# YoungSeng/QPGesture

Measured on AMD Instinct MI355X. Metric: matched gesture frames/sec (GestureKNN), higher is better.
Workload: dtype split-f16 products / f64 block sums + f64 re-evaluation; 1 GPU; 1 x 24 s clip (M=6 windows, Q=48 steps, 1440 frames each) per job vs speaker-10-class DB N_db=2048 windows (53248 candidates), shipped mode wavlm_feat(f32-bounded/f64-exact)+text(f32)+phase; n_db=2048, windows_per_clip=6, clips=1, clips_per_gpu=1, feature_dtype=f32, audio_precision=mixed, encode_batch=0, clips_in_flight=1, parallelism=single GPU, unsharded DB

## Files before the change

include/qpg.h:

```cpp
#ifndef QPG_H
#define QPG_H

#include <stddef.h>
#include <stdint.h>

#ifdef __cplusplus
extern "C" {
#endif

#define QPG_OK 0
#define QPG_EINVAL (-1)
#define QPG_EHIP (-2)
#define QPG_EUNSUP (-3)

typedef struct qpg_ctx qpg_ctx;

int qpg_version(void);
const char* qpg_build_id(void);
int qpg_ctx_create(int device, qpg_ctx** out);
int qpg_dev_kernarg(void);
int qpg_ctx_destroy(qpg_ctx* ctx);
#define QPG_OPT_GATE_DEDUP_FROM_CHAINS 0
#define QPG_OPT_TAKES_STAGES 1
#define QPG_OPT_COUNT 4
int qpg_ctx_set_option(qpg_ctx* ctx, int option, int value);
int qpg_ctx_get_option(qpg_ctx* ctx, int option, int* value);
int qpg_last_error(char* buf, size_t n);
int qpg_signal_i32(qpg_ctx*, void* stream, int32_t* dst, int32_t value);
int qpg_doorbell_wait(qpg_ctx*, void* stream, int32_t* counter, const int32_t* go, int32_t timeout_ms);


int qpg_wavlm_resample_f32(qpg_ctx*, void* stream, const float* x, int64_t N, int Tin, int F, int Tout, float* out);

int qpg_frame_norm2_f64(qpg_ctx*, void* stream, const float* x, int64_t rows, int F, double* out);

int qpg_audio_cand_norm2(qpg_ctx*, void* stream, const double* fn2, int N, int T, const int32_t* cand_t,
                         int G, int n_taps, int tap_stride, double* cn2);

int qpg_l2_normalize_rows_f32(qpg_ctx*, void* stream, const float* x, int64_t rows, int D, float* out);
int qpg_text_pack_queries_f32(qpg_ctx*, void* stream, const float* x, int M, int R, int D, const int32_t* q_win,
                              const int32_t* q_row, int Q, float* out);


int qpg_audio_pack_queries(qpg_ctx*, void* stream, const float* qbase, int M, int T, int F,
                           const int32_t* q_win, const int32_t* q_t, int Q, int n_taps, int tap_stride,
                           float* q32, double* qn2);

int qpg_audio_cosine_f64(qpg_ctx*, void* stream, const float* base, int N, int T, int F,
                         const int32_t* cand_t, int G, int n_taps, int tap_stride, const double* cn2,
                         const float* q32, const double* qn2, int Q, double* D, int64_t ldD);
int qpg_audio_cosine_f64_h(qpg_ctx*, void* stream, const void* base_f16, int N, int T, int F,
                           const int32_t* cand_t, int G, int n_taps, int tap_stride, const double* cn2,
                           const float* q32, const double* qn2, int Q, double* D, int64_t ldD);

#define QPG_AUDIO_MX_ERR 2.05e-6
int qpg_audio_cosine_mx(qpg_ctx*, void* stream, const float* base, int N, int T, int F, const int32_t* cand_t, int G,
                        int n_taps, int tap_stride, const double* cn2, const float* q32, const double* qn2, int Q,
                        void* D, int d_is_f32, int64_t ldD, int32_t* stats);

int qpg_audio_cosine_mx_h(qpg_ctx*, void* stream, const void* base_f16, int N, int T, int F, const int32_t* cand_t, int G,
                          int n_taps, int tap_stride, const double* cn2, const float* q32, const double* qn2, int Q,
                          void* D, int d_is_f32, int64_t ldD, int32_t* stats);

#define QPG_AUDIO_HL_ERR 1.3e-6
int qpg_audio_hl_supported(int T, int F, int G, int n_taps, int tap_stride, int cand_step);
int qpg_audio_pack_queries_hl(qpg_ctx*, void* stream, const float* qbase, int M, int T, int F, const int32_t* q_win,
                              const int32_t* q_t, int Q, int n_taps, int tap_stride, float* q32, double* qn2, void* image,
                              int64_t image_bytes);
int64_t qpg_audio_hl_db_bytes(int N, int F);
int64_t qpg_audio_hl_query_bytes(int Q, int F);
int qpg_audio_hl_pack_db(qpg_ctx*, void* stream, const float* base, int N, int T, int F, int G, int n_taps, int tap_stride,
                         int cand_step, void* image, int64_t image_bytes);
int qpg_audio_hl_pack_queries(qpg_ctx*, void* stream, const float* q32, int Q, int F, void* image, int64_t image_bytes);
int qpg_clip_pack_hl(qpg_ctx*, void* stream, const float* qbase, int M, int T, int F, const int32_t* q_win,
                     const int32_t* q_t, int Q, int n_taps, int tap_stride, float* q32, double* qn2, void* image,
                     int64_t image_bytes, const float* text_ctx, int Mt, int R, int Dt, const int32_t* tq_win,
                     const int32_t* tq_row, int Qt, float* qn_out, void* cols_image, int64_t cols_bytes);
int qpg_audio_cosine_hl(qpg_ctx*, void* stream, const void* db_image, int N, int F, int G, const double* cn2,
                        const void* q_image, const double* qn2, int Q, void* D, int d_is_f32, int64_t ldD, int32_t* stats);
int qpg_audio_hl1_supported(int T, int F, int G, int n_taps, int tap_stride, int cand_step);
int64_t qpg_audio_hl1_db_bytes(int N, int F);
int qpg_audio_hl1_pack_db(qpg_ctx*, void* stream, const void* base_f16, int N, int T, int F, int G, int n_taps,
                          int tap_stride, int cand_step, void* image, int64_t image_bytes);
int qpg_audio_cosine_hl1(qpg_ctx*, void* stream, const void* db_image, int N, int F, int G, const double* cn2,
                         const void* q_image, const double* qn2, int Q, void* D, int d_is_f32, int64_t ldD, int32_t* stats);
int qpg_probe_mfma_f16_tile(qpg_ctx*, void* stream, const void* a, const void* b, const float* c, int tiles, float* out);

int qpg_text_pack_candidates_f32(qpg_ctx*, void* stream, const float* x, int N, int R, int Dm,
                                 const int32_t* cand_r, int G, float* xt);

int qpg_text_cosine_f32(qpg_ctx*, void* stream, const float* xt, int64_t C, int Dm, const float* qn, int Q,
                        float* D, int64_t ldD);

int64_t qpg_text_percode_ws_bytes(int64_t C, int Q, int K, int tiles_per_chunk);
int qpg_text_percode_f32(qpg_ctx*, void* stream, const float* xt, int64_t C, int Dm, const int16_t* cand_code, int K,
                         const float* qn, int Q, int tiles_per_chunk, int32_t idx_base, float absent, void* ws,
                         int64_t ws_bytes, float* out_dist, int32_t* out_idx, int16_t* out_rank, int32_t* out_nn);
int qpg_text_pack_candidates_f16(qpg_ctx*, void* stream, const float* x, int N, int R, int Dm, const int32_t* cand_r,
                                 int G, void* xh, float* nrm);
int qpg_text_percode_f16(qpg_ctx*, void* stream, const void* xh, const float* nrm, int64_t C, int Dm,
                         const int16_t* cand_code, int K, const float* qn, int Q, int32_t idx_base, float absent,
                         void* ws, int64_t ws_bytes, float* out_dist, int32_t* out_idx, int16_t* out_rank,
                         int32_t* out_nn);

int64_t qpg_hl_rows_bytes(int64_t R, int D);
int64_t qpg_hl_cols_bytes(int Q, int D);
int qpg_hl_pack_rows(qpg_ctx*, void* stream, const float* xs, int64_t R, int D, void* image, int64_t image_bytes);
int qpg_hl_pack_cols(qpg_ctx*, void* stream, const float* qn, int Q, int D, void* image, int64_t image_bytes);
int qpg_hl_prepare_queries(qpg_ctx*, void* stream, const float* q, int Q, int D, float* qn_out, void* cols_image,
                           int64_t image_bytes, float* qperm_out);
int qpg_hl_gemm_distance(qpg_ctx*, void* stream, const void* rows_image, int64_t R, int D, const void* cols_image, int Q,
                         float* Dm, int64_t ldD, float* tile_min, int64_t ldT);
int qpg_hl_gemm_tilemin(qpg_ctx*, void* stream, const void* rows_image, int64_t R, int D, const void* cols_image, int Q,
                        float band, float* tile_min, uint16_t* tile_mask, int64_t ldT);
int qpg_hl_gemm_tilemin_h(qpg_ctx*, void* stream, const void* rows_image, int64_t R, int D, const void* cols_image, int Q,
                          float band, float* tile_min_t, uint16_t* tile_mask_t, int64_t ldQ);
int qpg_perm32_rows_f32(qpg_ctx*, void* stream, const float* x, int64_t R, int D, float* y);
int qpg_percode_select_bycode_f32(qpg_ctx*, void* stream, const float* tile_min_t, const uint16_t* tile_mask_t, int64_t ldQ,
                                  int Q, int64_t R, const int16_t* row_code, const int32_t* row_index,
                                  const int32_t* zero_row, const int32_t* code_tile, int K, float band,
                                  const float* qn_perm, const float* xs_perm, int D, float absent, float* out_dist,
                                  int32_t* out_idx, int16_t* out_rank, int32_t* out_nn, int32_t* stats, int32_t idx_base);
int qpg_percode_select_sorted_f32(qpg_ctx*, void* stream, const float* Dm, int64_t ldD, const float* tile_min,
                                  const uint16_t* tile_mask , int64_t ldT,
                                  int Q, int64_t R, const int16_t* row_code, const int32_t* row_index,
                                  const int32_t* zero_row, const int32_t* code_tile, int K, float band, const float* qn,
                                  const float* xs, int D, float absent, float* out_dist, int32_t* out_idx,
                                  int16_t* out_rank, int32_t* out_nn, int32_t* stats, int32_t idx_base, int q_block,
                                  int64_t block_stride);

int qpg_wavvq_lev_f32(qpg_ctx*, void* stream, const int32_t* sym_db, int N, int T, const int32_t* cand_t, int G,
                      const int32_t* tap_off, int n_taps, const int32_t* sym_q, int Mq, int Tq,
                      const int32_t* q_win, const int32_t* q_t, int Q, float* D, int64_t ldD);

int qpg_percode_select_f64(qpg_ctx*, void* stream, const double* D, int64_t ldD, int Q, const int16_t* cand_code,
                           int64_t C, int K, double absent, int32_t idx_base, double* out_dist, int32_t* out_idx,
                           int16_t* out_rank, int q_block, int64_t block_stride);
int qpg_percode_select_f32(qpg_ctx*, void* stream, const float* D, int64_t ldD, int Q, const int16_t* cand_code,
                           int64_t C, int K, float absent, int32_t idx_base, float* out_dist, int32_t* out_idx,
                           int16_t* out_rank, int q_block, int64_t block_stride);

int qpg_percode_select_guarded_f64(qpg_ctx*, void* stream, const double* D, int64_t ldD, int Q, const int16_t* cand_code,
                                   int64_t C, int K, double absent, int32_t idx_base, double* out_dist, int32_t* out_idx,
                                   int16_t* out_rank, int q_block, int64_t block_stride, const float* base, int T, int F,
                                   const int32_t* cand_t, int G, int n_taps, int tap_stride, const float* q32, double eps,
                                   int32_t* stats, int base_is_f16);

int64_t qpg_percode_select_exact_ws_bytes(int Q, int64_t C, int K);
int qpg_percode_select_exact_f64(qpg_ctx*, void* stream, const double* D, int64_t ldD, int Q, const int16_t* cand_code,
                                 int64_t C, int K, double absent, int32_t idx_base, double* out_dist, int32_t* out_idx,
                                 int16_t* out_rank, int q_block, int64_t block_stride, const float* base, int T, int F,
                                 const int32_t* cand_t, int G, int n_taps, int tap_stride, const float* q32, double eps,
                                 int32_t* stats, int base_is_f16, void* ws, int64_t ws_bytes);

int qpg_percode_select_mixed_f64(qpg_ctx*, void* stream, const void* D, int d_is_f32, int64_t ldD, int Q, const int16_t* cand_code,
                                 int64_t C, int K, double absent, int32_t idx_base, double* out_dist, int32_t* out_idx,
                                 int16_t* out_rank, int q_block, int64_t block_stride, const float* base, int T, int F,
                                 const int32_t* cand_t, int G, int n_taps, int tap_stride, const float* q32,
                                 const double* qn2, const double* cn2, double eps1, double eps2, int32_t* stats,
                                 void* ws, int64_t ws_bytes, int base_is_f16);
int64_t qpg_percode_select_mixed_ws_bytes(int Q, int K);
int64_t qpg_percode_select_mixed_ws_stride(int K);
int qpg_percode_select_mixed_f64_cut(qpg_ctx*, void* stream, const void* D, int d_is_f32, int64_t ldD, int Q,
                                     const int16_t* cand_code, int64_t C, int K, double absent, int32_t idx_base,
                                     double* out_dist, int32_t* out_idx, int16_t* out_rank, int q_block, int64_t block_stride,
                                     const float* base, int T, int F, const int32_t* cand_t, int G, int n_taps,
                                     int tap_stride, const float* q32, const double* qn2, const double* cn2, double eps1,
                                     double eps2, int32_t* stats, void* ws, int64_t ws_bytes, int base_is_f16,
                                     const int16_t* pos_rank_t, const int16_t* freq_rank, int top_n, int probe);

int64_t qpg_merge_mixed_ws_bytes(int Q, int K, int fl_cap);
int qpg_merge_mixed_phase1_f64(qpg_ctx*, void* stream, const void* recv, int W, int64_t src_stride, int64_t dist_off,
                               int64_t idx_off, int Q, int K, double absent, double eps1, int R, void* req,
                               int64_t req_stride, void* ws, int64_t ws_bytes, int32_t* stats, int fl_cap,
                               int64_t flag_off);
int qpg_shard_refine_f64(qpg_ctx*, void* stream, const void* req_recv, int W, int64_t req_stride, int R, int q_stride,
                         int64_t cand_base, const float* base, int base_is_f16, int T, int F, const int32_t* cand_t, int G,
                         int n_taps, int tap_stride, const float* q32, const double* qn2, const double* cn2, void* resp,
                         int64_t resp_stride, int reference_arithmetic, int32_t* stats, int Rq);
int qpg_flags_stamp(qpg_ctx*, void* stream, void* buf, int nblk, int64_t stride, int64_t off, const int32_t* stats);
int qpg_flags_gather(qpg_ctx*, void* stream, const void* buf, int nblk, int64_t stride, int64_t off, int32_t* stats);
int qpg_merge_mixed_phase2_f64(qpg_ctx*, void* stream, const void* recv, int W, int64_t src_stride, int64_t idx_off, int Q,
                               int K, double absent, const void* ws, int64_t ws_bytes, const void* resp_recv,
                               int64_t resp_stride, double* out_dist, int32_t* out_idx, int16_t* out_rank, int32_t* stats,
                               int fl_cap, double eps2);

int qpg_merge_select_f64(qpg_ctx*, void* stream, const void* recv, int W, int64_t src_stride, int64_t dist_off,
                         int64_t idx_off, int Q, int K, double absent, double* out_dist, int32_t* out_idx,
                         int16_t* out_rank, double eps2, int32_t* stats);
int qpg_merge_select_f32(qpg_ctx*, void* stream, const void* recv, int W, int64_t src_stride, int64_t dist_off,
                         int64_t idx_off, int Q, int K, float absent, float* out_dist, int32_t* out_idx,
                         int16_t* out_rank);

int qpg_rank_rows_f64(qpg_ctx*, void* stream, const double* d, int Q, int K, int16_t* out);
int qpg_rank_rows_f32(qpg_ctx*, void* stream, const float* d, int Q, int K, int16_t* out);


int qpg_l2_table_f32(qpg_ctx*, void* stream, const float* sig, int K, int Dm, float* out);

#define QPG_MODE_AUD_TXT 0
#define QPG_MODE_AUD 1
#define QPG_MODE_TXT 2
#define QPG_MODE_SERIAL_WALK 0x100
#define QPG_MODE_PREFUSED 0x200

int qpg_match_steps(qpg_ctx*, void* stream, const int16_t* aud_rank, const int32_t* aud_idx,
                    const int16_t* txt_rank, const int32_t* txt_idx, const int16_t* pos_rank,
                    const int16_t* freq_rank, const int32_t* code, int code_ld, const int32_t* aud_cidx,
                    const int32_t* aud_pslot, int Ga, const int32_t* txt_cidx, const int32_t* txt_pslot, int Gt,
                    const float* phase, int Tp, int mode, int M, int steps, int K, int seed_code,
                    const float* seed_phase, int32_t* gate_tables, int32_t* out_codes, float* out_phase,
                    int32_t* out_vote, int32_t* out_status, const int32_t* guard_flags);
int qpg_match_steps_batch(qpg_ctx*, void* stream, const int16_t* aud_rank, const int32_t* aud_idx, const int16_t* txt_rank,
                          const int32_t* txt_idx, const int16_t* pos_rank, const int16_t* freq_rank, const int32_t* code,
                          int code_ld, const int32_t* aud_cidx, const int32_t* aud_pslot, int Ga, const int32_t* txt_cidx,
                          const int32_t* txt_pslot, int Gt, const float* phase, int Tp, int mode, int M, int steps, int K,
                          int n_chains, const int32_t* seed_codes, const float* seed_phase, int32_t* gate_tables,
                          int32_t* out_codes, float* out_phase, int32_t* out_vote, int32_t* out_status,
                          int64_t status_stride, const int32_t* guard_flags);
#define QPG_TAKES_MAX 65536
size_t qpg_match_steps_takes_ws_bytes(int n_takes, int M, int steps);
int qpg_match_steps_takes(qpg_ctx*, void* stream, const int16_t* aud_rank, const int32_t* aud_idx, const int16_t* txt_rank,
                          const int32_t* txt_idx, const int16_t* pos_rank, const int16_t* freq_rank, const int32_t* code,
                          int code_ld, const int32_t* aud_cidx, const int32_t* aud_pslot, int Ga, const int32_t* txt_cidx,
                          const int32_t* txt_pslot, int Gt, const float* phase, int Tp, int mode, int M, int steps, int K,
                          int n_takes, const int32_t* seed_codes, const float* seed_phase, int32_t* gate_tables,
                          int32_t* out_codes, float* out_phase, int32_t* out_vote, int32_t* out_status,
                          int64_t status_stride, const int32_t* guard_flags, void* workspace, size_t workspace_bytes);
int qpg_fuse_best_ranked(qpg_ctx*, void* stream, const int16_t* rank, const int32_t* idx, const int16_t* pos_rank,
                         const int16_t* freq_rank, int Q, int K, int32_t* T);

typedef struct qpg_comm qpg_comm;
int qpg_comm_unique_id(void* id, int64_t id_bytes);
int qpg_comm_create(qpg_ctx*, const void* id, int64_t id_bytes, int rank, int world, qpg_comm** out);
int qpg_comm_destroy(qpg_comm*);
int qpg_comm_allgather(qpg_ctx*, void* stream, qpg_comm*, const void* send, void* recv, int64_t bytes);
int qpg_comm_alltoall(qpg_ctx*, void* stream, qpg_comm*, const void* send, void* recv, int64_t bytes);
int qpg_comm_allreduce_max_i32(qpg_ctx*, void* stream, qpg_comm*, int32_t* buf, int64_t count);
int qpg_allreduce_min_u64(qpg_ctx*, void* stream, qpg_comm*, uint64_t* buf, int64_t count);
int qpg_pack_min_u64(qpg_ctx*, void* stream, const float* dist, const int32_t* idx, int64_t n, uint64_t* packed);
int qpg_unpack_min_u64(qpg_ctx*, void* stream, const uint64_t* packed, int64_t n, float absent, float* dist, int32_t* idx);


int qpg_conv1d_f32(qpg_ctx*, void* stream, const float* x, int B, int T_in, int Cin, const float* w,
                   const float* bias, int taps, int Cin_pad, int Cout, int Cout_pad, int in_stride, int in_offset,
                   int dil, int T_out, int out_stride, int out_offset, int T_y, const float* residual, int relu_in,
                   int relu_out, float* y, float* ws, int64_t ws_floats);

int qpg_convt_f32(qpg_ctx*, void* stream, const float* x, int B, int T_in, int Cx, const float* wt, const float* bias,
                  int taps, int Cin_pad, int Cout, int Cout_pad, int in_stride, int in_offset, int dil, int T_out,
                  int out_stride, int out_offset, int T_y, const float* residual, int relu_in, int relu_out, float* y);
int qpg_convt_pair_f32(qpg_ctx*, void* stream, const float* x, int B, int T_in, int Cx, const float* wt0,
                       const float* bias0, int in_offset0, int out_offset0, const float* wt1, const float* bias1,
                       int in_offset1, int out_offset1, int taps, int Cin_pad, int Cout, int Cout_pad, int in_stride,
                       int dil, int T_out, int out_stride, int T_y, float* y);
int qpg_tpack_f32(qpg_ctx*, void* stream, const float* w, int taps, int Cin_pad, int Cout_pad, int nb, float* out);
int qpg_pad_channels_f32(qpg_ctx*, void* stream, const float* x, int64_t R, int C, int Cp, float* y);
int qpg_resblock_f32(qpg_ctx*, void* stream, const float* x, int B, int T, int dil, const float* wpack,
                     const float* b1, const float* b2, float* y, float* hidden);

int qpg_vq_argmin_f32(qpg_ctx*, void* stream, const float* z, const float* dot, const float* kk, int64_t R, int E,
                      int K, int64_t* ids, float* dmin, float* dsecond);

int qpg_vq_gather_f32(qpg_ctx*, void* stream, const float* k, const int64_t* ids, int64_t R, int E, int K, float* out,
                      int32_t* status);

#define QPG_CONV16_WEXP_FROM_IMAGE 0x7fff
int64_t qpg_conv16_image_bytes(int taps, int Cin, int Cout);
int qpg_conv16_pack_weights(qpg_ctx*, void* stream, const float* w, int taps, int Cin, int Cin_pad_w, int Cout, int Cout_pad_w,
                            void* image, int64_t image_bytes);
int qpg_conv16_f32(qpg_ctx*, void* stream, const float* x, int B, int T_in, int Cx, int Cin, const void* image, int w_exp,
                   const float* bias, int taps, int Cout, int in_stride, int in_offset, int dil, int T_out, int out_stride,
                   int out_offset, int T_y, const float* residual, int relu_in, int relu_out, float* y, int32_t* status);

#define QPG_VQ_MAX_DOWN 4
#define QPG_VQ_MAX_DEPTH 4
typedef struct {
  const float* w;
  const float* b;
  int32_t taps, cin, cin_pad, cout, cout_pad;
  const float* wt;
} qpg_conv_desc;
typedef struct {
  int32_t in_dim, width, emb, bins, down_t, depth, growth, reverse_dec;
  qpg_conv_desc enc_down[QPG_VQ_MAX_DOWN];
  qpg_conv_desc enc_res[QPG_VQ_MAX_DOWN][QPG_VQ_MAX_DEPTH][2];
  qpg_conv_desc enc_out;
  qpg_conv_desc dec_in;
  qpg_conv_desc dec_res[QPG_VQ_MAX_DOWN][QPG_VQ_MAX_DEPTH][2];
  qpg_conv_desc dec_up_even[QPG_VQ_MAX_DOWN];
  qpg_conv_desc dec_up_odd[QPG_VQ_MAX_DOWN];
  qpg_conv_desc dec_out;
  qpg_conv_desc kT;
  const float* k;
  const float* kk;
  const float* enc_res_pack[QPG_VQ_MAX_DOWN][QPG_VQ_MAX_DEPTH];
  const float* dec_res_pack[QPG_VQ_MAX_DOWN][QPG_VQ_MAX_DEPTH];
} qpg_vq_model;

int64_t qpg_vq_workspace_floats(const qpg_vq_model* m, int B, int T);
int qpg_vq_encode_f32(qpg_ctx*, void* stream, const qpg_vq_model* m, const float* x, int B, int T, float* ws,
                      int64_t ws_floats, int64_t* ids, float* latent, float* margin);
int qpg_vq_decode_f32(qpg_ctx*, void* stream, const qpg_vq_model* m, const int64_t* ids, int B, int L, float* ws,
                      int64_t ws_floats, float* out, int32_t* status);

int qpg_pose_to_euler_f64(qpg_ctx*, void* stream, const float* poses, int64_t T, int J, const double* mean,
                          const double* stdc, const double* sg_mid, const double* sg_head, const double* sg_tail, int W,
                          double* euler, int32_t* status);

#define QPG_PAE_CHANNELS 135
#define QPG_PAE_MID 15
#define QPG_PAE_EMBED 8
#define QPG_PAE_TIME 240
#define QPG_PAE_HALO 120
#define QPG_PAE_WS_STRIDE 136
#define QPG_PAE_MAX_CHUNK (1 << 22)
#define QPG_PAE_OFF_W1 0
#define QPG_PAE_OFF_BN1 522240
#define QPG_PAE_OFF_W2 522288
#define QPG_PAE_OFF_BN2 583728
#define QPG_PAE_OFF_FC 583776
#define QPG_PAE_OFF_FCBN 587616
#define QPG_PAE_OFF_FREQ 587664
#define QPG_PAE_OFF_TPI 587784
#define QPG_PAE_PARAM_FLOATS 587792
int qpg_pae_phase_f32(qpg_ctx*, void* stream, const float* params, const double* pose, const double* mean,
                      const double* stdc, const int64_t* clip_off, int n_clips, int64_t n_total, int64_t frame0,
                      int64_t n_frames, float* ws, int64_t ws_floats, float* out, float* v_out, float* latent_out);

#define QPG_PAET_OFF_TPI 0
#define QPG_PAET_OFF_ARGS 1
#define QPG_PAET_OFF_FREQS 241
#define QPG_PAET_TRAINABLE 361
#define QPG_PAET_OFF_CONV1_W 361
#define QPG_PAET_OFF_CONV1_B 486361
#define QPG_PAET_OFF_BN1 486376
#define QPG_PAET_OFF_CONV2_W 486406
#define QPG_PAET_OFF_CONV2_B 515206
#define QPG_PAET_OFF_BN2 515214
#define QPG_PAET_OFF_FC 515230
#define QPG_PAET_OFF_FCBN 519086
#define QPG_PAET_OFF_DECONV1_W 519118
#define QPG_PAET_OFF_DECONV1_B 547918
#define QPG_PAET_OFF_BN3 547933
#define QPG_PAET_OFF_DECONV2_W 547963
#define QPG_PAET_OFF_DECONV2_B 1033963
#define QPG_PAET_PARAM_FLOATS 1034098
#define QPG_PAET_ST_BN1 0
#define QPG_PAET_ST_BN2 30
#define QPG_PAET_ST_FCBN 46
#define QPG_PAET_ST_BN3 78
#define QPG_PAET_STATS_FLOATS 108
#define QPG_PAET_MAX_BATCH 65536
#define QPG_PAET_SLABS 16
int qpg_pae_train_ws_floats(qpg_ctx*, void* stream, int batch, int64_t* floats);
int qpg_pae_train_forward_f32(qpg_ctx*, void* stream, const float* params, float* stats, const float* poses,
                              int64_t n_frames, const int64_t* starts, int batch, int train, float* ws,
                              int64_t ws_floats, double* loss);
int qpg_pae_train_backward_f32(qpg_ctx*, void* stream, const float* params, int batch, float* ws, int64_t ws_floats,
                               float* grads);
int qpg_pae_adamw_f32(qpg_ctx*, void* stream, float* p, const float* g, float* m, float* v, int64_t n, double lr,
                      double weight_decay, double beta1, double beta2, double eps, int64_t step);

int64_t qpg_vq_reduce_ws_bytes(void);

int qpg_vq_loss_f32(qpg_ctx*, void* stream, const float* x_out, const float* x_target, int B, int T, int C,
                    const float* commit_loss, float w_commit, float w_reg, float w_vel, float w_acc, void* ws,
                    int64_t ws_bytes, float* out6);
int qpg_vq_loss_grad_f32(qpg_ctx*, void* stream, const float* x_out, const float* x_target, int B, int T, int C,
                         float w_reg, float w_vel, float w_acc, float upstream, float* d_x_out);

int qpg_vq_latent_stats_f32(qpg_ctx*, void* stream, const float* z, const float* zq, const float* dmin, int64_t R,
                            int E, void* ws, int64_t ws_bytes, float* out3);
int qpg_vq_commit_grad_f32(qpg_ctx*, void* stream, const float* z, const float* zq, int64_t R, int E, float scale,
                           const float* d_zq, float* d_z);

int64_t qpg_vq_code_sums_ws_bytes(int64_t R, int E, int K);
int qpg_vq_code_sums_f32(qpg_ctx*, void* stream, const float* z, const int64_t* ids, int64_t R, int E, int K,
                         float* batch_sum, float* batch_elem, void* ws, int64_t ws_bytes);
int qpg_vq_ema_update_f32(qpg_ctx*, void* stream, float* k, float* k_sum, float* k_elem, const float* batch_sum,
                          const float* batch_elem, const float* k_rand, float mu, float threshold, int K, int E,
                          float* kT, int ldkT, float* kk, void* ws, int64_t ws_bytes, float* out4);
int qpg_vq_code_norms_f32(qpg_ctx*, void* stream, const float* k, int K, int E, float* kk);
// ... 26 lines not shown
```

qpgesture_amd/code_knn.py:

```python
import ctypes
from collections import namedtuple
from typing import NamedTuple, Optional

import numpy as np
import torch

from . import _lib
from .parallel import allreduce_max_, allreduce_min_index, exchange_bytes, shard_rows
from .sorted_rows import SortedRows

from .constant import (ABSENT_DIST, NUM_AUDIO_FEAT_FRAMES, STEP_SZ, WAVVQ_GROUP_SIZE, codebook_size, num_frames,
                       num_frames_code)

MODE_AUD_TXT, MODE_AUD, MODE_TXT = _lib.QPG_MODE_AUD_TXT, _lib.QPG_MODE_AUD, _lib.QPG_MODE_TXT
AUDIO_MX_ERR = _lib.QPG_AUDIO_MX_ERR
AUDIO_MX_BAND = 2.1 * AUDIO_MX_ERR
AUDIO_HL_ERR = _lib.QPG_AUDIO_HL_ERR
AUDIO_HL_BAND = 2.1 * AUDIO_HL_ERR

FLAG_LIST_OVERFLOW, FLAG_SMALL_NORMS, FLAG_REQUEST_OVERFLOW, FLAG_CROSS_SHARD_TIE = 1, 2, 4, 8
FLAG_TEXT_OVERFLOW = 16


_PIN_SENTINEL = -1234567
# ... 599 lines not shown
        D = torch.empty((Q, max(C, 1)), dtype=torch.float32, device=dev)
        taps = (ctypes.c_int32 * len(db.vq_taps))(*db.vq_taps)
        _lib.call("qpg_wavvq_lev_f32", dev, db.vq_sym, db.n_local, db.Tv, db.vq_t, db.Gv, taps, len(db.vq_taps),
                  sym_q, sym_q.shape[0], sym_q.shape[1], _i32(q_win, dev), _i32(q_t, dev), Q, D, D.stride(0))
        dist, idx, rank = self._select_plain(D, db.vq_cand_code, C, db.Gv, out, want_rank and db.world == 1)
        self._last_D_aud = D
        return self._finish(dist, idx, rank, want_rank, reduce)

    def _reduce_min(self, dist, idx):
        if self.db.world == 1:
            return dist, idx
        return allreduce_min_index(dist, idx)

    def guard_stats(self):
        v = self._guard_stats.cpu().numpy()
        return int(v[0]), bool(v[1])

    def mixed_stats(self):
        v = self._guard_stats.cpu().numpy()
        return {"tier1_pairs": int(v[2]), "tier2_pairs": int(v[0]), "flags": int(v[1])}

    def tier1_list_lengths(self):
        ws, Q = self._mix_ws, self._last_mix_Q
        if ws is None or not Q:
            return np.zeros((0,), np.int64)
        K = self.db.K
        stride = int(_lib.load().qpg_percode_select_mixed_ws_stride(K))
        w = ws[:Q * stride].view(Q, stride)[:, 24 * K:24 * K + 4].contiguous().view(torch.int32)
        return w.cpu().numpy().reshape(-1).astype(np.int64)

    def clear_flags(self):
        self._guard_stats[1:2].zero_()

    @staticmethod
    def numpy_ranks(dist, idx=None, integer=False):
        d = dist.detach().cpu().numpy()
        present = None if idx is None else (idx.detach().cpu().numpy() >= 0)
        out = np.empty(d.shape, np.int16)
        for r_, row in enumerate(d):
            full = present is not None and bool(present[r_].all())
            if full and integer:
                arr = np.array([int(x) for x in row])
            elif full:
                arr = np.array(list(row))
            else:
                arr = np.array(list(row.astype(np.float64)))
            out[r_] = arr.argsort().argsort()
        return torch.from_numpy(out).to(dist.device)

    def rank_rows(self, dist):
        out = torch.empty(dist.shape, dtype=torch.int16, device=dist.device)
        name = "qpg_rank_rows_f64" if dist.dtype == torch.float64 else "qpg_rank_rows_f32"
        _lib.call(name, self.db.device, dist.contiguous(), dist.shape[0], dist.shape[1], out)
        return out

    def _unpack(self, dist, idx, G, ks, cidx):
        d = dist[0].cpu().numpy()
        ix = idx[0].cpu().numpy()
        code = self.db.code_host
        dists, pays, aux = [], [], []
        for c in range(self.db.K):
            if ix[c] < 0:
                dists.append(ABSENT_DIST)
                pays.append([])
                aux.append([])
            else:
                j, g = divmod(int(ix[c]), G)
                dists.append(d[c])
                pays.append(code[j, cidx[g]:cidx[g] + STEP_SZ])
                aux.append([j, ks[g]])
        return dists, pays, aux

    def search_audio_cands(self, clip_input, mode="wavlm_feat"):
        db = self.db
        if mode == "wavvq_feat":
            v = np.asarray(clip_input).reshape(11, 2).astype(np.int64)
            track = np.zeros((1, db.Tv, 2), np.int64)
            t0 = -min(db.vq_taps)
            for i, off in enumerate(db.vq_taps):
                track[0, t0 + off] = v[i]
            dist, idx = self.sweep_audio_wavvq(track, [0], [t0])
            return self._unpack(dist, idx, db.Gv, db.vq_k, db.vq_cidx_host)
        if mode != "wavlm_feat":
            raise NotImplementedError(mode)
        q = torch.as_tensor(np.asarray(clip_input, np.float32).reshape(1, NUM_AUDIO_FEAT_FRAMES, db.F),
                            device=db.device).contiguous()
        dist, idx = self.sweep_audio(q, [0], [0], tap_stride=1)
        return self._unpack(dist, idx, db.Ga, db.aud_k, db.aud_cidx_host)

    def search_text_cands(self, clip_input, mode="wavvq_feat"):
        db = self.db
        q = torch.as_tensor(np.asarray(clip_input, np.float32).reshape(1, db.Dt), device=db.device).contiguous()
        dist, idx = self.sweep_text(q)
        return self._unpack(dist, idx, db.Gt, db.txt_k, db.txt_rows_host)

    def n_steps(self):
        return len(self.query_positions())

    def _query_index(self, M):
        if M not in self._qcache:
            pos, dev = self.query_positions(), self.db.device
            qw = np.repeat(np.arange(M), len(pos))
            qt = np.tile(np.array([int(i) for i in pos]), M)
            rows_ = [int(i / self.n_db_frm * 30) for i in pos] * M
            self._qcache[M] = (_i32(qw, dev), _i32(qt, dev), _i32(np.asarray(rows_), dev))
        return self._qcache[M]

    def _fork_side(self):
        dev = self.db.device
        if self._side_stream is None:
            self._side_stream = torch.cuda.Stream(dev)
            self._side_gate, self._side_done = torch.cuda.Event(), torch.cuda.Event()
            self._sweep_event = torch.cuda.Event()
        if dev.index is None or dev.index == torch.cuda.current_device():
            self._side_gate.record()
        else:
            self._side_gate.record(torch.cuda.current_stream(dev))
        self._side_stream.wait_event(self._side_gate)
        return self._side_stream

    def _clip_pack(self, test_interp, test_context, q_win, q_t, q_row, Q):
        db, dev = self.db, self.db.device
        q32 = torch.empty((Q, NUM_AUDIO_FEAT_FRAMES * db.F), dtype=torch.float32, device=dev)
        qn2 = torch.empty((Q,), dtype=torch.float64, device=dev)
        qi = self._hl_qimage = _grown(self._hl_qimage, int(_lib.load().qpg_audio_hl_query_bytes(Q, db.F)), dev)
        qn = torch.empty((Q, db.Dt), dtype=torch.float32, device=dev)
        cols = db.txt_sorted.cols_buffer(Q, self._txt_scratch)
        tc, ti = test_context.contiguous(), test_interp.contiguous()
        _lib.call("qpg_clip_pack_hl", dev, ti, ti.shape[0], db.T, db.F, q_win, q_t, Q, NUM_AUDIO_FEAT_FRAMES,
                  db.tap_stride, q32, qn2, qi, qi.numel(), tc, tc.shape[0], tc.shape[1], db.Dt, q_win, q_row, Q, qn, cols,
                  cols.numel())
        return q32, qn2, qn

    def sweep_tables(self, test_interp, test_context, n_windows, mode=MODE_AUD_TXT, owner_blocks=False, for_walk=False,
                     after_sweep=None):
        db, dev = self.db, self.db.device
        M, steps = n_windows, self.n_steps()
        if test_interp.shape[0] < M or (mode != MODE_AUD and test_context.shape[0] < M):
            raise IndexError("n_windows=%d but the test arrays hold %d audio / %d context windows"
                             % (M, test_interp.shape[0], test_context.shape[0]))
        want = (db.Tv, 2) if self.use_wavvq else (db.T, db.F)
        if tuple(test_interp.shape[1:]) != want:
            raise ValueError("test audio windows have shape %s, database expects %s"
                             % (tuple(test_interp.shape[1:]), want))
        q_win, q_t, q_row = self._query_index(M)
        Q = M * steps
        key = (self._knobs(), self._facts(), M, steps, mode, for_walk, owner_blocks)
        plan = self._plans.get(key)
        if plan is None:
            plan = self._plans[key] = plan_step(*key)
        sharded = plan.sharded
        T = dict(aud_d=None, aud_idx=None, aud_rank=None, txt_d=None, txt_idx=None, txt_rank=None)
        gtab = torch.empty((3, max(M, 1) * steps, db.K), dtype=torch.int32, device=dev) if plan.split_fuse else None
        lay = self._layout(Q, owner_blocks, mode) if sharded else None
        side = self._fork_side() if plan.overlap else None
        packed = None
        if plan.clip_pack:
            packed = self._clip_pack(test_interp, test_context, q_win, q_t, q_row, Q)
            self._side_gate.record(torch.cuda.current_stream(dev))
            side.wait_event(self._side_gate)

        def keep(p_, g, r):
            T[p_ + "_d"], T[p_ + "_idx"], T[p_ + "_rank"] = r[0], r[1], (None if sharded else r[2])
            if gtab is not None:
                _lib.call("qpg_fuse_best_ranked", dev, r[2], r[1], db.pos_rank, db.freq_rank, Q, db.K, gtab[g])

        def text_pack():
            tc = test_context.contiguous()
            qn = torch.empty((Q, db.Dt), dtype=torch.float32, device=dev)
            _lib.call("qpg_text_pack_queries_f32", dev, tc, tc.shape[0], tc.shape[1], db.Dt, q_win, q_row, Q, qn)
            return qn

        def text_side(qn=None):
            if packed is not None:
                qn = packed[2]
            elif qn is None:
                qn = text_pack()
            keep("txt", 1, self.sweep_text(qn, want_rank=not sharded, reduce=not sharded, normalised=True,
                                           out=lay.views("txt") if sharded else None, cols_packed=packed is not None,
                                           kind=plan.text))

        if plan.order == "text_first":
            with torch.cuda.stream(side):
                text_side()
        aud = None
        if mode != MODE_TXT:
            out = lay.views("aud") if sharded else None
            if self.use_wavvq:
                r = self.sweep_audio_wavvq(test_interp, q_win, q_t, want_rank=not sharded, reduce=not sharded, out=out)
            else:
                aud = self._sweep_audio(plan.audio, test_interp, q_win, q_t, out=out, prepacked=packed,
                                        sweep_event=self._sweep_event if plan.order == "text_after_sweep" else None,
                                        after_sweep=after_sweep)
                r = self._finish(aud.dist, aud.idx, aud.rank, not sharded, not sharded)
            keep("aud", 0, r)
        if plan.order == "text_after_sweep":
            with torch.cuda.stream(side):
                qn_early = None if packed is not None else text_pack()
                side.wait_event(self._sweep_event)
                text_side(qn_early)
        elif plan.order == "audio_first":
            with torch.cuda.stream(side):
                text_side()
        if plan.overlap:
            self._side_done.record(side)
            torch.cuda.current_stream(dev).wait_event(self._side_done)
        elif mode != MODE_AUD:
            text_side()
        if sharded:
            self._merge_shards(lay, owner_blocks, T, aud)
        if self.host_ranks:
            for p_ in ("aud", "txt"):
                if T[p_ + "_d"] is not None:
                    T[p_ + "_rank"] = self.numpy_ranks(T[p_ + "_d"], T[p_ + "_idx"],
                                                       integer=(p_ == "aud" and self.use_wavvq))
        if gtab is not None:
            T["gate_tables"] = gtab
        return T

    def _layout(self, Q, owner_blocks, mode):
        parts = tuple(p_ for p_, off in (("aud", MODE_TXT), ("txt", MODE_AUD)) if mode != off)
        key = (Q, self.db.world if owner_blocks else 1, parts, not self.use_wavvq)
        if key not in self._layouts:
            self._layouts[key] = ExchangeLayout(key[0], self.db.K, key[1], parts, key[3], self.db.device)
        return self._layouts[key]

    def _merge_shards(self, lay, owner_blocks, T, aud):
        db, dev = self.db, self.db.device
        _lib.call("qpg_flags_stamp", dev, lay.send, lay.nblk, lay.block_bytes, lay.off["flags"], self._guard_stats)
        recv = exchange_bytes(lay.send, db.world, owner_blocks)
        src_stride = lay.block_bytes if owner_blocks else lay.send.numel()
        gathered = False
        for p_ in lay.parts:
            d = torch.empty((lay.Qb, db.K), dtype=lay.dtype[p_], device=dev)
            ix = torch.empty((lay.Qb, db.K), dtype=torch.int32, device=dev)
            rk = torch.empty((lay.Qb, db.K), dtype=torch.int16, device=dev)
            wavlm_aud = p_ == "aud" and aud is not None
            if wavlm_aud and aud.plan.path in ("mixed", "exact"):
                self._merge_mixed(recv, src_stride, lay, owner_blocks, d, ix, rk, aud.q32, aud.qn2, aud.plan)
                gathered = True
            elif lay.dtype[p_] == torch.float64:
                guard = wavlm_aud and self.tie_eps > 0
                _lib.call("qpg_merge_select_f64", dev, recv, db.world, src_stride, lay.off[p_ + "_d"],
                          lay.off[p_ + "_i"], lay.Qb, db.K, float(ABSENT_DIST), d, ix, rk,
                          float(self.tie_eps) if guard else 0.0, self._guard_stats if guard else None)
            else:
                _lib.call("qpg_merge_select_f32", dev, recv, db.world, src_stride,
                          lay.off[p_ + "_d"], lay.off[p_ + "_i"], lay.Qb, db.K, float(ABSENT_DIST), d, ix, rk)
            T[p_ + "_d"], T[p_ + "_idx"], T[p_ + "_rank"] = d, ix, rk
        if not gathered:
            _lib.call("qpg_flags_gather", dev, recv, db.world, src_stride, lay.off["flags"], self._guard_stats)
        if owner_blocks:
            allreduce_max_(self._guard_stats[1:2], force=self.force_sharded)

    def _merge_mixed(self, recv, src_stride, lay, owner_blocks, d, ix, rk, q32, qn2, plan):
        db, dev = self.db, self.db.device
        W, Qb, K = db.world, lay.Qb, db.K
        exact = plan.path == "exact"
        if exact:
            Rq, fl_cap, band = K, K * W, float(self.tie_eps)
        else:
            Rq = int(self.mixed_requests) if self.mixed_requests else max(64, 512 // W)
            fl_cap, band = 1024, plan.band
        R = Qb * Rq
        req_stride = resp_stride = 8 + 8 * R
        key = (exact, W, R)
        bufs = self._mm_cache.get(key)
        need_ws = int(_lib.load().qpg_merge_mixed_ws_bytes(Qb, K, fl_cap))
        if bufs is None or bufs[2].numel() < need_ws:
            bufs = self._mm_cache[key] = (torch.empty((W * req_stride,), dtype=torch.uint8, device=dev),
                                          torch.empty((W * resp_stride,), dtype=torch.uint8, device=dev),
                                          torch.empty((need_ws,), dtype=torch.uint8, device=dev))
        req, resp, ws = bufs
        _lib.call("qpg_merge_mixed_phase1_f64", dev, recv, W, src_stride, lay.off["aud_d"], lay.off["aud_i"], Qb, K,
                  float(ABSENT_DIST), band, R, req, req_stride, ws, ws.numel(), self._guard_stats, fl_cap,
                  lay.off["flags"])
        half = int(db.feature_dtype == "f16")
        refine = (db.idx_base * db.Ga, db.base, half, db.T, db.F, db.aud_t, db.Ga, NUM_AUDIO_FEAT_FRAMES, db.tap_stride,
                  q32, qn2, db.cn2, resp, resp_stride, int(exact), self._guard_stats, Rq)
        if owner_blocks:
            req_recv = exchange_bytes(req, W, True)
            _lib.call("qpg_shard_refine_f64", dev, req_recv, W, req_stride, R, Qb, *refine)
            resp_recv = exchange_bytes(resp, W, True)
        else:
            mine = req[db.rank * req_stride:(db.rank + 1) * req_stride]
            _lib.call("qpg_shard_refine_f64", dev, mine, 1, req_stride, R, 0, *refine)
            resp_recv = exchange_bytes(resp[:resp_stride], W, False)
        _lib.call("qpg_merge_mixed_phase2_f64", dev, recv, W, src_stride, lay.off["aud_i"], Qb, K, float(ABSENT_DIST), ws,
                  ws.numel(), resp_recv, resp_stride, d, ix, rk, self._guard_stats, fl_cap,
                  0.0 if exact else float(self.tie_eps))

    def _seed_phase_tensor(self, seed_phase):
        if isinstance(seed_phase, torch.Tensor):
            return seed_phase.to(self.db.device, torch.float32).contiguous()
        return torch.as_tensor(np.asarray(seed_phase, np.float32), device=self.db.device).contiguous()

    def _launch_walk(self, T, q0, Qt, rows, mode, prefusable, M, steps, seed, sp, outs, chains=None):
        db, dev = self.db, self.db.device
        gate = T.get("gate_tables")
        prefused = prefusable and gate is not None and mode == MODE_AUD_TXT and gate.shape[1] == Qt
        if not prefused:
            gate = torch.empty((3, rows, db.K), dtype=torch.int32, device=dev)
        mode_w = mode | (_lib.QPG_MODE_PREFUSED if prefused else 0)
        if chains is None and self.serial_walk:
            mode_w |= _lib.QPG_MODE_SERIAL_WALK
        a_cidx, a_pslot, a_G = self._audio_grid()
        tabs = [None if T[k] is None else T[k][q0:q0 + Qt] for k in ("aud_rank", "aud_idx", "txt_rank", "txt_idx")]
        head = (*tabs, db.pos_rank, db.freq_rank, db.code, db.code.shape[1], a_cidx, a_pslot, a_G, db.txt_cidx,
                db.txt_pslot, db.Gt, db.phase, db.Tp, mode_w, M, steps, db.K)
        guard = self._guard_stats[1:2]
        if chains is None:
            _lib.call("qpg_match_steps", dev, *head, seed, sp, gate, *outs, guard)
        else:
            _lib.call("qpg_match_steps_batch", dev, *head, chains, seed, sp, gate, *outs, 2, guard)
        return gate

    def walk(self, T, n_windows, window_offset=0, mode=MODE_AUD_TXT, seed_code=None, seed_phase=None, sync=True,
             seed_ptrs=None, out_pin=None, n_chains=1):
# ... 165 lines not shown
```

qpgesture_amd/csrc/qpg_common.h:

```cpp
#pragma once
#include <hip/hip_runtime.h>
#include <stdint.h>
#include <stdio.h>
#include <string.h>

#include "../../include/qpg.h"

struct qpg_ctx {
  int device;
  int n_cu;
  float* zeros;
  bool select_lds_raised;
  int opt[QPG_OPT_COUNT];
};

#ifdef QPG_DEBUG_HOOKS
#define QPG_HOOK_VAR(type, name, value) static type name = value
#else
#define QPG_HOOK_VAR(type, name, value) static constexpr type name = value
#endif

void qpg_set_error(const char* fmt, ...);

#define QPG_REQUIRE(cond, ...)      \
  do {                              \
    if (!(cond)) {                  \
      qpg_set_error(__VA_ARGS__);   \
      return QPG_EINVAL;            \
    }                               \
  } while (0)

#define QPG_LAUNCH_CHECK(name)                                                \
  do {                                                                        \
    hipError_t e_ = hipGetLastError();                                        \
    if (e_ != hipSuccess) {                                                   \
      qpg_set_error("%s: launch failed: %s", name, hipGetErrorString(e_));    \
      return QPG_EHIP;                                                        \
    }                                                                         \
  } while (0)

static inline hipStream_t qpg_stream(void* s) { return reinterpret_cast<hipStream_t>(s); }

typedef double f64x4 __attribute__((ext_vector_type(4)));
typedef float f32x4 __attribute__((ext_vector_type(4)));
typedef float f32x16 __attribute__((ext_vector_type(16)));

#pragma clang fp contract(off)
__device__ __forceinline__ float f_mul(float a, float b) { return a * b; }
__device__ __forceinline__ float f_add(float a, float b) { return a + b; }
__device__ __forceinline__ float f_sub(float a, float b) { return a - b; }
__device__ __forceinline__ float f_div(float a, float b) { return a / b; }
__device__ __forceinline__ float f_sqrt(float a) { return __builtin_sqrtf(a); }
__device__ __forceinline__ double f_mul(double a, double b) { return a * b; }
__device__ __forceinline__ double f_add(double a, double b) { return a + b; }
__device__ __forceinline__ double f_sub(double a, double b) { return a - b; }
__device__ __forceinline__ double f_div(double a, double b) { return a / b; }

__device__ __forceinline__ double cosine_from_dot(double dot, double qn2, double cn2) {
  const double tiny = 10.0 * 2.220446049250313e-16;
  double nq = sqrt(qn2), nc = sqrt(cn2);
  bool zq = nq < tiny, zc = nc < tiny;
  if (zq || zc) {
    double a = zq ? qn2 : 1.0, b = zc ? cn2 : 1.0;
    double cross = dot / ((zq ? 1.0 : nq) * (zc ? 1.0 : nc));
    return 0.5 * (a + b - 2.0 * cross);
  }
  return 1.0 - dot / (nq * nc);
}


__host__ __device__ __forceinline__ int rank_sort_pow2(int K) {
  int p = 2;
  while (p < K) p <<= 1;
  return p;
}
__device__ __forceinline__ unsigned long long rank_sort_key(double d) {
  const long long b = __double_as_longlong(d + 0.0);
  return b < 0 ? ~(unsigned long long)b : ((unsigned long long)b | 0x8000000000000000ull);
}
__device__ __forceinline__ unsigned long long rank_sort_key(float d) {
  const unsigned int b = __float_as_uint(d + 0.0f);
  return (unsigned long long)((b >> 31) ? ~b : (b | 0x80000000u));
}
template <int PJ>
__device__ __forceinline__ int lane_xor(int x) {
  if (PJ == 1) return __builtin_amdgcn_update_dpp(x, x, 0xB1, 0xf, 0xf, false);
  if (PJ == 2) return __builtin_amdgcn_update_dpp(x, x, 0x4E, 0xf, 0xf, false);
  if (PJ == 4) {
    const int t = __builtin_amdgcn_update_dpp(x, x, 0x104, 0xf, 0x5, false);
    return __builtin_amdgcn_update_dpp(t, x, 0x114, 0xf, 0xa, false);
  }
  if (PJ == 8) return __builtin_amdgcn_update_dpp(x, x, 0x128, 0xf, 0xf, false);
  if (PJ == 16) {
    const auto r = __builtin_amdgcn_permlane16_swap(x, x, false, false);
    return (threadIdx.x & 16) ? r[0] : r[1];
  }
  const auto r = __builtin_amdgcn_permlane32_swap(x, x, false, false);
  return (threadIdx.x & 32) ? r[0] : r[1];
}
template <int PJ>
__device__ __forceinline__ void lane_xor_pair(unsigned long long k0, unsigned long long k1, int c0, int c1,
                                              unsigned long long& p0, unsigned long long& p1, int& q0, int& q1) {
  const unsigned int a0 = (unsigned int)lane_xor<PJ>((int)(unsigned int)k0);
  const unsigned int a1 = (unsigned int)lane_xor<PJ>((int)(unsigned int)(k0 >> 32));
  const unsigned int a2 = (unsigned int)lane_xor<PJ>((int)(unsigned int)k1);
  const unsigned int a3 = (unsigned int)lane_xor<PJ>((int)(unsigned int)(k1 >> 32));
  q0 = lane_xor<PJ>(c0);
  q1 = lane_xor<PJ>(c1);
  p0 = ((unsigned long long)a1 << 32) | a0;
  p1 = ((unsigned long long)a3 << 32) | a2;
}

struct RankPair {
  unsigned long long k0, k1;
  int c0, c1;
};
__device__ __forceinline__ bool rank_gt(unsigned long long ka, int ca, unsigned long long kb, int cb) {
  return ka > kb || (ka == kb && ca > cb);
}
template <int J>
__device__ __forceinline__ void bitonic_chain(RankPair& e, int i0, int k, unsigned long long* skey, int* scode) {
  if constexpr (J == 0) {
    return;
  } else {
    if (J < k) {
      const bool up = (i0 & k) == 0;
      if constexpr (J == 1) {
        if (rank_gt(e.k0, e.c0, e.k1, e.c1) == up) {
          const unsigned long long tk = e.k0; e.k0 = e.k1; e.k1 = tk;
          const int tc = e.c0; e.c0 = e.c1; e.c1 = tc;
        }
      } else {
        unsigned long long p0, p1;
        int q0, q1;
        if constexpr (J / 2 < 64) {
          lane_xor_pair<J / 2>(e.k0, e.k1, e.c0, e.c1, p0, p1, q0, q1);
        } else {
          __syncthreads();
          skey[i0] = e.k0; skey[i0 + 1] = e.k1; scode[i0] = e.c0; scode[i0 + 1] = e.c1;
          __syncthreads();
          const int o0 = i0 ^ J;
          p0 = skey[o0]; p1 = skey[o0 + 1]; q0 = scode[o0]; q1 = scode[o0 + 1];
        }
        const bool keep_min = ((i0 & J) == 0) == up;
        if (rank_gt(e.k0, e.c0, p0, q0) == keep_min) { e.k0 = p0; e.c0 = q0; }
        if (rank_gt(e.k1, e.c1, p1, q1) == keep_min) { e.k1 = p1; e.c1 = q1; }
      }
    }
    bitonic_chain<J / 2>(e, i0, k, skey, scode);
  }
}
template <int KP, typename T, typename F>
__device__ __forceinline__ void block_sorted_ranks_unrolled(const T* v, int K, unsigned long long* skey, int* scode,
                                                            F&& emit) {
  const int tid = threadIdx.x;
  if ((tid & ~63) * 2 >= KP) {
    for (int k = 256; k <= KP; k <<= 1)
      for (int j = k >> 1; j >= 128; j >>= 1) {
        __syncthreads();
        __syncthreads();
      }
    return;
  }
  const int i0 = 2 * tid;
  RankPair e;
  e.k0 = i0 < K ? rank_sort_key(v[i0]) : ~0ull;
  e.k1 = i0 + 1 < K ? rank_sort_key(v[i0 + 1]) : ~0ull;
// ... 44 lines not shown
```

qpgesture_amd/csrc/qpg_core.hip:

```cpp
#include <stdarg.h>

#include "qpg_common.h"
#include <stdlib.h>

static thread_local char g_err[512] = "";

void qpg_set_error(const char* fmt, ...) {
  va_list ap;
  va_start(ap, fmt);
  vsnprintf(g_err, sizeof(g_err), fmt, ap);
  va_end(ap);
}

extern "C" int qpg_version(void) { return 109; }

#ifndef QPG_BUILD_ID
#define QPG_BUILD_ID "unstamped"
#endif
static const char g_build_id[] = "QPG_BUILD_ID=" QPG_BUILD_ID;
extern "C" const char* qpg_build_id(void) { return g_build_id + 13; }

extern "C" int qpg_dev_kernarg(void) {
  const char* e = getenv("HIP_FORCE_DEV_KERNARG");
  return (e && e[0] == '1') ? 1 : 0;
}

extern "C" int qpg_last_error(char* buf, size_t n) {
  if (!buf || n == 0) return QPG_EINVAL;
  strncpy(buf, g_err, n - 1);
  buf[n - 1] = 0;
  return QPG_OK;
}

extern "C" int qpg_ctx_create(int device, qpg_ctx** out) {
  QPG_REQUIRE(out != nullptr, "qpg_ctx_create: out is null");
  int n = 0;
  if (hipGetDeviceCount(&n) != hipSuccess || device < 0 || device >= n) {
    qpg_set_error("qpg_ctx_create: no HIP device %d (count %d)", device, n);
    return QPG_EHIP;
  }
  hipDeviceProp_t p;
  if (hipGetDeviceProperties(&p, device) != hipSuccess) {
    qpg_set_error("qpg_ctx_create: hipGetDeviceProperties failed");
    return QPG_EHIP;
  }
  qpg_ctx* c = new qpg_ctx;
  c->device = device;
  c->n_cu = p.multiProcessorCount;
  c->zeros = nullptr;
  c->select_lds_raised = false;
  for (int i = 0; i < QPG_OPT_COUNT; ++i) c->opt[i] = 0;
  c->opt[QPG_OPT_GATE_DEDUP_FROM_CHAINS] = 1;
  c->opt[QPG_OPT_TAKES_STAGES] = 7;
  int prev = 0;
  (void)hipGetDevice(&prev);
  const bool ok = hipSetDevice(device) == hipSuccess && hipMalloc(reinterpret_cast<void**>(&c->zeros), 4096) == hipSuccess &&
                  hipMemset(c->zeros, 0, 4096) == hipSuccess;
  (void)hipSetDevice(prev);
  if (!ok) {
    qpg_set_error("qpg_ctx_create: could not allocate the context's zero page on device %d", device);
    delete c;
    return QPG_EHIP;
  }
  *out = c;
  return QPG_OK;
}

extern "C" int qpg_ctx_set_option(qpg_ctx* ctx, int option, int value) {
  QPG_REQUIRE(ctx != nullptr, "qpg_ctx_set_option: null context");
  QPG_REQUIRE(option >= 0 && option < QPG_OPT_COUNT, "qpg_ctx_set_option: unknown option %d", option);
  if (option == QPG_OPT_GATE_DEDUP_FROM_CHAINS) QPG_REQUIRE(value >= 0, "qpg_ctx_set_option: gate_dedup_from_chains >= 0");
  ctx->opt[option] = value;
  return QPG_OK;
}

extern "C" int qpg_ctx_get_option(qpg_ctx* ctx, int option, int* value) {
  QPG_REQUIRE(ctx != nullptr && value != nullptr, "qpg_ctx_get_option: null pointer");
  QPG_REQUIRE(option >= 0 && option < QPG_OPT_COUNT, "qpg_ctx_get_option: unknown option %d", option);
  *value = ctx->opt[option];
  return QPG_OK;
}

extern "C" int qpg_ctx_destroy(qpg_ctx* ctx) {
  if (ctx && ctx->zeros) (void)hipFree(ctx->zeros);
  delete ctx;
  return QPG_OK;
}

__global__ void signal_i32_kernel(int32_t* dst, int32_t value) {
  __hip_atomic_store(dst, value, __ATOMIC_RELEASE, __HIP_MEMORY_SCOPE_SYSTEM);
}

extern "C" int qpg_signal_i32(qpg_ctx* ctx, void* stream, int32_t* dst, int32_t value) {
  QPG_REQUIRE(ctx && dst && (reinterpret_cast<uintptr_t>(dst) % 4) == 0, "qpg_signal_i32: null or misaligned destination");
  hipLaunchKernelGGL(signal_i32_kernel, dim3(1), dim3(1), 0, qpg_stream(stream), dst, value);
  QPG_LAUNCH_CHECK("signal_i32_kernel");
  return QPG_OK;
}

__global__ void doorbell_wait_kernel(int32_t* __restrict__ counter, const int32_t* __restrict__ go, int32_t timeout_ms) {
  const int32_t seq = atomicAdd(counter, 1) + 1;
  const long long t0 = wall_clock64();
  const long long limit = (long long)timeout_ms * 100000ll;
  while (__hip_atomic_load(go, __ATOMIC_RELAXED, __HIP_MEMORY_SCOPE_SYSTEM) - seq < 0) {
    if (wall_clock64() - t0 > limit) break;
    __builtin_amdgcn_s_sleep(16);
  }
  __atomic_thread_fence(__ATOMIC_ACQUIRE);
}

extern "C" int qpg_doorbell_wait(qpg_ctx* ctx, void* stream, int32_t* counter, const int32_t* go, int32_t timeout_ms) {
  QPG_REQUIRE(ctx && counter && go && timeout_ms > 0 && timeout_ms <= 60000, "qpg_doorbell_wait: bad argument (timeout 1..60000 ms)");
  hipLaunchKernelGGL(doorbell_wait_kernel, dim3(1), dim3(1), 0, qpg_stream(stream), counter, go, timeout_ms);
  QPG_LAUNCH_CHECK("doorbell_wait_kernel");
  return QPG_OK;
}

__global__ __launch_bounds__(256) void frame_norm2_kernel(const float* __restrict__ x, int64_t rows, int F,
                                                          double* __restrict__ out) {
  const int lane = threadIdx.x & 63;
  const int64_t row = (int64_t)blockIdx.x * 4 + (threadIdx.x >> 6);
  if (row >= rows) return;
  const float* p = x + row * F;
  double s = 0.0;
  if ((F & 3) == 0) {
    for (int e = lane * 4; e < F; e += 256) {
      f32x4 v = *reinterpret_cast<const f32x4*>(p + e);
      s += (double)v.x * v.x + (double)v.y * v.y + (double)v.z * v.z + (double)v.w * v.w;
    }
  } else {
    for (int e = lane; e < F; e += 64) s += (double)p[e] * p[e];
  }
  for (int o = 32; o > 0; o >>= 1) s += __shfl_down(s, o, 64);
  if (lane == 0) out[row] = s;
}

extern "C" int qpg_frame_norm2_f64(qpg_ctx* ctx, void* stream, const float* x, int64_t rows, int F, double* out) {
  QPG_REQUIRE(ctx && x && out && rows >= 0 && F > 0, "qpg_frame_norm2_f64: bad argument");
  if (rows == 0) return QPG_OK;
  hipLaunchKernelGGL(frame_norm2_kernel, dim3((unsigned)((rows + 3) / 4)), dim3(256), 0, qpg_stream(stream), x, rows,
                     F, out);
  QPG_LAUNCH_CHECK("frame_norm2_kernel");
  return QPG_OK;
}

__global__ void audio_cand_norm2_kernel(const double* __restrict__ fn2, int N, int T, const int32_t* __restrict__ cand_t,
                                        int G, int n_taps, int tap_stride, double* __restrict__ cn2) {
  int64_t i = (int64_t)blockIdx.x * blockDim.x + threadIdx.x;
  if (i >= (int64_t)N * G) return;
  int j = (int)(i / G), g = (int)(i % G);
  int t0 = cand_t[g];
  double s = 0.0;
  for (int k = 0; k < n_taps; ++k) {
    int t = t0 + k * tap_stride;
    if (t < T) s += fn2[(int64_t)j * T + t];
  }
  cn2[i] = s;
}

extern "C" int qpg_audio_cand_norm2(qpg_ctx* ctx, void* stream, const double* fn2, int N, int T,
                                    const int32_t* cand_t, int G, int n_taps, int tap_stride, double* cn2) {
  QPG_REQUIRE(ctx && fn2 && cand_t && cn2 && N >= 0 && T > 0 && G > 0 && n_taps > 0 && tap_stride > 0,
              "qpg_audio_cand_norm2: bad argument");
  int64_t n = (int64_t)N * G;
  if (n == 0) return QPG_OK;
  hipLaunchKernelGGL(audio_cand_norm2_kernel, dim3((unsigned)((n + 255) / 256)), dim3(256), 0, qpg_stream(stream),
                     fn2, N, T, cand_t, G, n_taps, tap_stride, cn2);
  QPG_LAUNCH_CHECK("audio_cand_norm2_kernel");
  return QPG_OK;
}

template <bool GATHER>
__global__ __launch_bounds__(256) void l2_normalize_rows_kernel(const float* __restrict__ x, int64_t rows, int D,
                                                                float* __restrict__ out,
                                                                const int32_t* __restrict__ win,
                                                                const int32_t* __restrict__ row, int R) {
  const int64_t t = (int64_t)blockIdx.x * blockDim.x + threadIdx.x;
  int64_t r = t >> 2;
  const int l = (int)(t & 3);
  const bool live = r < rows;
  if (!live) r = rows - 1;
  const float* p = GATHER ? x + ((int64_t)win[r] * R + row[r]) * D : x + r * D;
  float a = 0.f;
  const int nfull = D >> 4;
  int g = 0;
  for (; g + 8 <= nfull; g += 8) {
    float v[32];
#pragma unroll
    for (int j = 0; j < 32; ++j) v[j] = p[(g + (j >> 2)) * 16 + (j & 3) * 4 + l];
#pragma unroll
    for (int j = 0; j < 8; ++j) {
#pragma unroll
      for (int u = 3; u >= 0; --u) a = f_add(f_mul(v[j * 4 + u], v[j * 4 + u]), a);
    }
  }
  for (; g < nfull; ++g) {
#pragma unroll
    for (int u = 3; u >= 0; --u) {
      const float v = p[g * 16 + u * 4 + l];
      a = f_add(f_mul(v, v), a);
    }
  }
  for (int i = nfull * 16; i < D; i += 4) {
    const float v = (i + l < D) ? p[i + l] : 0.f;
    a = f_add(f_mul(v, v), a);
  }
  const float o1 = __shfl_xor(a, 1, 64);
  const float pair = f_add(a, o1);
  const float o2 = __shfl_xor(pair, 2, 64);
  float n = f_sqrt(f_add(pair, o2));
  if (n < 10.f * 1.1920928955078125e-07f) n = 1.f;
  if (live) {
    float* o = out + r * D;
    int e = l;
    for (; e + 28 < D; e += 32) {
      float v[8];
#pragma unroll
      for (int j = 0; j < 8; ++j) v[j] = p[e + 4 * j];
#pragma unroll
      for (int j = 0; j < 8; ++j) o[e + 4 * j] = f_div(v[j], n);
    }
    for (; e < D; e += 4) o[e] = f_div(p[e], n);
  }
}

extern "C" int qpg_l2_normalize_rows_f32(qpg_ctx* ctx, void* stream, const float* x, int64_t rows, int D, float* out) {
// ... 47 lines not shown
```

qpgesture_amd/csrc/qpg_select.hip:

```cpp
#include "qpg_common.h"

__device__ __forceinline__ unsigned long long order_key(double d) {
  unsigned long long b = (unsigned long long)__double_as_longlong(d);
  return (b >> 63) ? ~b : (b | 0x8000000000000000ull);
}
__device__ __forceinline__ double key_value(unsigned long long k, double) {
  unsigned long long b = (k >> 63) ? (k & 0x7fffffffffffffffull) : ~k;
  return __longlong_as_double((long long)b);
}
__device__ __forceinline__ unsigned int order_key(float d) {
  unsigned int b = __float_as_uint(d);
  return (b >> 31) ? ~b : (b | 0x80000000u);
}
__device__ __forceinline__ float key_value(unsigned int k, float) {
  unsigned int b = (k >> 31) ? (k & 0x7fffffffu) : ~k;
  return __uint_as_float(b);
}

template <typename T, typename KeyT, bool PACKED>
__global__ __launch_bounds__(1024) void percode_select_kernel(const T* __restrict__ D, int64_t ldD,
                                                              const int16_t* __restrict__ cand_code, int64_t C, int K,
                                                              T absent, int32_t idx_base, T* __restrict__ out_dist,
                                                              int32_t* __restrict__ out_idx,
                                                              int16_t* __restrict__ out_rank, int q_block,
                                                              int64_t block_stride) {
  extern __shared__ __attribute__((aligned(16))) unsigned char smem[];
  unsigned long long* best = reinterpret_cast<unsigned long long*>(smem);
  unsigned int* besti = reinterpret_cast<unsigned int*>(smem + 8 * (size_t)K);
  T* v = reinterpret_cast<T*>(smem + 12 * (size_t)rank_sort_pow2(K));
  constexpr int VEC = 16 / sizeof(T);
  typedef T vecT __attribute__((ext_vector_type(VEC)));
  typedef int16_t vecC __attribute__((ext_vector_type(VEC)));
  const int q = blockIdx.x;
  if (q_block > 0) {
    const int64_t shift = (int64_t)(q / q_block) * block_stride;
    const int64_t rowoff = (int64_t)(q % q_block) * K - (int64_t)q * K;
    out_dist = reinterpret_cast<T*>(reinterpret_cast<unsigned char*>(out_dist) + shift) + rowoff;
    out_idx = reinterpret_cast<int32_t*>(reinterpret_cast<unsigned char*>(out_idx) + shift) + rowoff;
  }
  const T* row = D + (int64_t)q * ldD;
  for (int k = threadIdx.x; k < K; k += blockDim.x) {
    best[k] = ~0ull;
    besti[k] = 0xffffffffu;
  }
  __syncthreads();
  const bool vec_ok = (ldD % VEC) == 0 && (reinterpret_cast<uintptr_t>(D) % 16) == 0 &&
                      (reinterpret_cast<uintptr_t>(cand_code) % (2 * VEC)) == 0;
  const int64_t Cv = vec_ok ? (C / VEC) * VEC : 0;
  for (int64_t c = (int64_t)threadIdx.x * VEC; c < Cv; c += (int64_t)blockDim.x * VEC) {
    const vecT d = *reinterpret_cast<const vecT*>(row + c);
    const vecC cd = *reinterpret_cast<const vecC*>(cand_code + c);
#pragma unroll
    for (int e = 0; e < VEC; ++e) {
      if ((unsigned)cd[e] >= (unsigned)K) continue;
      const unsigned long long key = PACKED ? (((unsigned long long)order_key(d[e]) << 32) | (unsigned int)(c + e + idx_base))
                                            : (unsigned long long)order_key(d[e]);
      atomicMin(&best[cd[e]], key);
    }
  }
  for (int64_t c = Cv + threadIdx.x; c < C; c += blockDim.x) {
    const int cd = cand_code[c];
    if ((unsigned)cd >= (unsigned)K) continue;
    const unsigned long long key = PACKED ? (((unsigned long long)order_key(row[c]) << 32) | (unsigned int)(c + idx_base))
                                          : (unsigned long long)order_key(row[c]);
    atomicMin(&best[cd], key);
  }
  __syncthreads();
  if (!PACKED) {
    for (int64_t c = (int64_t)threadIdx.x * VEC; c < Cv; c += (int64_t)blockDim.x * VEC) {
      const vecT d = *reinterpret_cast<const vecT*>(row + c);
      const vecC cd = *reinterpret_cast<const vecC*>(cand_code + c);
#pragma unroll
      for (int e = 0; e < VEC; ++e)
        if ((unsigned)cd[e] < (unsigned)K && (unsigned long long)order_key(d[e]) == best[cd[e]])
          atomicMin(&besti[cd[e]], (unsigned int)(c + e + idx_base));
    }
    for (int64_t c = Cv + threadIdx.x; c < C; c += blockDim.x) {
      const int cd = cand_code[c];
      if ((unsigned)cd < (unsigned)K && (unsigned long long)order_key(row[c]) == best[cd])
        atomicMin(&besti[cd], (unsigned int)(c + idx_base));
    }
    __syncthreads();
  }
  for (int k = threadIdx.x; k < K; k += blockDim.x) {
    const unsigned long long kv = best[k];
    const bool have = kv != ~0ull;
    T d;
    int32_t ix;
    if (PACKED) {
      d = have ? key_value((KeyT)(kv >> 32), T(0)) : absent;
      ix = have ? (int32_t)(kv & 0xffffffffu) : -1;
    } else {
      d = have ? key_value((KeyT)kv, T(0)) : absent;
      ix = have ? (int32_t)besti[k] : -1;
    }
    v[k] = d;
    out_dist[(int64_t)q * K + k] = d;
    out_idx[(int64_t)q * K + k] = ix;
  }
  if (!out_rank) return;
  __syncthreads();
  const int Kp = rank_sort_pow2(K);
  block_sorted_ranks(v, K, best, reinterpret_cast<int*>(best + Kp),
                     [&](int k, int r) { out_rank[(int64_t)q * K + k] = (int16_t)r; });
}

template <typename T, typename F>
__device__ __forceinline__ void block_stable_ranks(const T* v, int K, int* cnt, F&& emit) {
  const int tid = threadIdx.x;
  if (K <= 512 && K >= 64 && (int)blockDim.x >= 256) {
    __shared__ unsigned long long rank_skey[512];
    __shared__ int rank_scode[512];
    block_sorted_ranks(v, K, rank_skey, rank_scode, emit);
    return;
  }
  const int P = (int)blockDim.x >= 2 * K ? (int)blockDim.x / K : 1;
  if (P == 1) {
    for (int k = tid; k < K; k += blockDim.x) {
      const T x = v[k];
      int r = 0;
#pragma unroll 8
      for (int o = 0; o < K; ++o) {
        const T y = v[o];
        r += (y < x) || (y == x && o < k);
      }
      emit(k, r);
    }
    return;
  }
  for (int k = tid; k < K; k += blockDim.x) cnt[k] = 0;
  __syncthreads();
  if (tid < P * K) {
    const int k = tid % K, part = tid / K;
    const int o0 = (int)((int64_t)part * K / P), o1 = (int)((int64_t)(part + 1) * K / P);
    const T x = v[k];
    int r = 0;
#pragma unroll 8
    for (int o = o0; o < o1; ++o) {
      const T y = v[o];
      r += (y < x) || (y == x && o < k);
    }
    atomicAdd(&cnt[k], r);
  }
  __syncthreads();
  for (int k = tid; k < K; k += blockDim.x) emit(k, cnt[k]);
}

struct GuardArgs {
  const float* base;
  int half;
  const float* q32;
  const int32_t* cand_t;
  int T, F, G, n_taps, tap_stride;
// ... 349 lines not shown
#define SEL_STAMP(i)                                                                          \
  do {                                                                                        \
    __syncthreads();                                                                          \
    if (blockIdx.x == 0 && blockIdx.y == 0 && threadIdx.x == 0) {                             \
      qpg_select_prof_buf[phase][i] = wall_clock64();                                         \
      qpg_select_prof_buf[3 + phase][i] = clock64();                                          \
    }                                                                                         \
  } while (0)
extern "C" int qpg_debug_select_prof(long long* out) {
  return hipMemcpyFromSymbol(out, HIP_SYMBOL(qpg_select_prof_buf), sizeof(long long) * 96) == hipSuccess ? 0 : -1;
}
#else
#define SEL_STAMP(i)
#endif

template <int NPER>
__global__ __launch_bounds__(256) void select_refine_kernel(GuardArgs A, int K, const double* __restrict__ cn2,
                                                            const double* __restrict__ qn2, unsigned char* __restrict__ ws,
                                                            int fast) {
  const int q = blockIdx.x, lane = threadIdx.x & 63;
  const int g = blockIdx.y * 4 + (threadIdx.x >> 6), ng = gridDim.y * 4;
  unsigned char* wq = mix_query_base(ws, q, K);
  const int* w_n = reinterpret_cast<const int*>(wq + 24 * (size_t)K);
  const int* w_lc = w_n + 4;
  double* w_ld = reinterpret_cast<double*>(const_cast<int*>(w_lc) + 2 * MIX_LIST);
  const int n = w_n[0];
  if (g >= n) return;
  const double qq = qn2[q];
  const float* qrow = A.q32 + (int64_t)q * A.n_taps * A.F;
  for (int e = g; e < n; e += ng) {
    const int c = w_lc[e];
    const double dot = fast ? pair_dot_fast_f64<NPER>(A, qrow, c, lane) : pair_dot_wave_f64(A, q, c, lane);
    if (lane == 0) w_ld[e] = cosine_from_dot(dot, qq, cn2[c]);
  }
}

__global__ __launch_bounds__(1024) void mixed_stream_kernel(const float* __restrict__ D, int64_t ldD,
                                                           const int16_t* __restrict__ cand_code, int64_t C, int K,
                                                           double eps1, unsigned char* __restrict__ ws) {
  extern __shared__ __attribute__((aligned(16))) unsigned char smem[];
  unsigned int* best32 = reinterpret_cast<unsigned int*>(smem);
  int* pc = reinterpret_cast<int*>(best32 + K);
  float* pd = reinterpret_cast<float*>(pc + MIX_SPOT);
  int16_t* pk = reinterpret_cast<int16_t*>(pd + MIX_SPOT);
  __shared__ int n_pot, n_keep;
  const int q = blockIdx.x, sl = blockIdx.y, tid = threadIdx.x;
#ifdef QPG_SELECT_PROF
  const int phase = 0;
#endif
  const float* row = D + (int64_t)q * ldD;
  const int64_t chunk = (((C + MIX_SPLIT - 1) / MIX_SPLIT) + 63) & ~(int64_t)63;
  const int64_t c0 = (int64_t)sl * chunk, c1 = c0 + chunk < C ? c0 + chunk : C;
  for (int k = tid; k < K; k += blockDim.x) best32[k] = 0xffffffffu;
  if (tid == 0) {
    n_pot = 0;
    n_keep = 0;
  }
  __syncthreads();
  SEL_STAMP(0);
  auto visit = [&](int64_t c, float dv, int cd) {
    if ((unsigned)cd >= (unsigned)K) return;
    const unsigned int key = order_key(dv);
    unsigned int old = *reinterpret_cast<volatile unsigned int*>(&best32[cd]);
    if (key < old) old = atomicMin(&best32[cd], key);
    if ((double)dv <= (double)key_value(old < key ? old : key, 0.f) + eps1) {
      const int pp = atomicAdd(&n_pot, 1);
      if (pp < MIX_SPOT) {
        pc[pp] = (int)c;
        pd[pp] = dv;
        pk[pp] = (int16_t)cd;
      }
    }
  };
  typedef int16_t c16x4 __attribute__((ext_vector_type(4)));
  const bool vec_ok = (ldD % 4) == 0 && (reinterpret_cast<uintptr_t>(D) % 16) == 0 &&
                      (reinterpret_cast<uintptr_t>(cand_code) % 8) == 0;
  const int64_t cv = vec_ok ? c0 + ((c1 - c0) / 4) * 4 : c0;
  constexpr int UN = 2;
  for (int64_t b = c0 + (int64_t)tid * 4; b < cv; b += (int64_t)blockDim.x * 4 * UN) {
    f32x4 d[UN];
    c16x4 cd[UN];
#pragma unroll
    for (int u = 0; u < UN; ++u) {
      const int64_t c = b + (int64_t)u * blockDim.x * 4;
      d[u] = (f32x4){0.f, 0.f, 0.f, 0.f};
      cd[u] = (c16x4){-1, -1, -1, -1};
      if (c < cv) {
        d[u] = *reinterpret_cast<const f32x4*>(row + c);
        cd[u] = *reinterpret_cast<const c16x4*>(cand_code + c);
      }
    }
    unsigned int key[UN][4], old[UN][4];
#pragma unroll
    for (int u = 0; u < UN; ++u)
#pragma unroll
      for (int e = 0; e < 4; ++e) {
        const int code = cd[u][e];
        key[u][e] = order_key(d[u][e]);
        old[u][e] = (unsigned)code < (unsigned)K ? *reinterpret_cast<volatile unsigned int*>(&best32[code]) : 0u;
      }
#pragma unroll
    for (int u = 0; u < UN; ++u)
#pragma unroll
      for (int e = 0; e < 4; ++e) {
        const int code = cd[u][e];
        if ((unsigned)code >= (unsigned)K) continue;
        unsigned int o = old[u][e];
        if (key[u][e] < o) o = atomicMin(&best32[code], key[u][e]);
        const unsigned int lo = o < key[u][e] ? o : key[u][e];
        if ((double)d[u][e] <= (double)key_value(lo, 0.f) + eps1) {
          const int pp = atomicAdd(&n_pot, 1);
          if (pp < MIX_SPOT) {
            pc[pp] = (int)(b + (int64_t)u * blockDim.x * 4 + e);
            pd[pp] = d[u][e];
            pk[pp] = (int16_t)code;
          }
        }
      }
  }
  for (int64_t c = cv + tid; c < c1; c += blockDim.x) visit(c, row[c], cand_code[c]);
  __syncthreads();
  SEL_STAMP(1);
  MixStream m = mix_stream_of(ws, q, K);
  if (MIX_INV_ATOMIC) {
    for (int k = tid; k < K; k += blockDim.x)
      if (best32[k] != 0xffffffffu) atomicMax(&m.inv[k], ~best32[k]);
  } else {
    for (int k = tid; k < K; k += blockDim.x) m.inv[(size_t)sl * K + k] = ~best32[k];
  }
  SEL_STAMP(2);
  const int np = n_pot;
  if (np > MIX_SPOT) {
    if (tid == 0) m.cnt[sl] = -1;
    return;
  }
  const int seg = sl * MIX_SPOT;
  for (int e = tid; e < np; e += blockDim.x) {
    if (!((double)pd[e] <= (double)key_value(best32[pk[e]], 0.f) + eps1)) continue;
    const int pos = seg + atomicAdd(&n_keep, 1);
    m.pot_c[pos] = pc[e];
    m.pot_d[pos] = pd[e];
    m.pot_k[pos] = pk[e];
  }
  __syncthreads();
  if (tid == 0) m.cnt[sl] = n_keep;
  SEL_STAMP(3);
}

template <typename DT>
__global__ __launch_bounds__(1024) void percode_select_mixed_f64_kernel(
    const DT* __restrict__ D, int64_t ldD, const int16_t* __restrict__ cand_code, int64_t C, int K, double absent,
    int32_t idx_base, double* __restrict__ out_dist, int32_t* __restrict__ out_idx, int16_t* __restrict__ out_rank,
    int q_block, int64_t block_stride, GuardArgs A, double eps1, const double* __restrict__ cn2,
    const double* __restrict__ qn2, int use_qlds, int phase, unsigned char* __restrict__ ws, int pre, RankCut RC) {
  extern __shared__ __attribute__((aligned(16))) unsigned char smem[];
  unsigned long long* best = reinterpret_cast<unsigned long long*>(smem);
  double* v = reinterpret_cast<double*>(smem + 8 * (size_t)K);
  unsigned int* besti = reinterpret_cast<unsigned int*>(smem + 16 * (size_t)K);
  unsigned int* near_ = besti + K;
  int* s_code = reinterpret_cast<int*>(near_ + K);
  unsigned char* refd = reinterpret_cast<unsigned char*>(s_code + K);
  unsigned char* tail = smem + 32 * (size_t)K;
  double* l_d = reinterpret_cast<double*>(tail);
  int* l_c = reinterpret_cast<int*>(tail + 8 * MIX_LIST);
  int* l_k = l_c + MIX_LIST;
  int* l2 = l_k + MIX_LIST;
  int* ctl = l2 + MIX_LIST2;
  int* p_c = ctl + 8;
  int16_t* p_k = reinterpret_cast<int16_t*>(p_c + MIX_LIST);
  int* rk = reinterpret_cast<int*>(p_k + MIX_LIST);
  int* pot_c = rk + K;
  int16_t* pot_k = reinterpret_cast<int16_t*>(pot_c + MIX_POT);
  float* qlds = reinterpret_cast<float*>(pot_k + MIX_POT);
  const int q = blockIdx.x, tid = threadIdx.x, lane = tid & 63, wv = tid >> 6, nwv = blockDim.x >> 6;
  const DT* row = D + (int64_t)q * ldD;
  if (q_block > 0) {
    const int64_t shift = (int64_t)(q / q_block) * block_stride;
    const int64_t rowoff = (int64_t)(q % q_block) * K - (int64_t)q * K;
    out_dist = reinterpret_cast<double*>(reinterpret_cast<unsigned char*>(out_dist) + shift) + rowoff;
    out_idx = reinterpret_cast<int32_t*>(reinterpret_cast<unsigned char*>(out_idx) + shift) + rowoff;
  }
  unsigned char* wq = ws ? mix_query_base(ws, q, K) : nullptr;
  for (int k = tid; k < K; k += blockDim.x) {
    best[k] = ~0ull;
    besti[k] = 0xffffffffu;
    near_[k] = 0;
    refd[k] = 0;
  }
  if (tid < 8) ctl[tid] = 0;
  __syncthreads();
  SEL_STAMP(0);
  unsigned long long* skey = reinterpret_cast<unsigned long long*>(p_c);
  int* scode = reinterpret_cast<int*>(skey + 512);
  auto rank_pass = [&](bool store) {
    block_sorted_ranks(v, K, skey, scode, [&](int k, int r) {
      if (store && out_rank) out_rank[(int64_t)q * K + k] = (int16_t)r;
      s_code[r] = k;
    });
  };
  int n = 0;
  bool order_parked = false;
  if (phase != 2) {
  constexpr int VE = 16 / (int)sizeof(DT);
  typedef DT vecD __attribute__((ext_vector_type(VE)));
  typedef int16_t vecC __attribute__((ext_vector_type(VE)));
  const bool vec_ok = (ldD % VE) == 0 && (reinterpret_cast<uintptr_t>(D) % 16) == 0 &&
                      (reinterpret_cast<uintptr_t>(cand_code) % (2 * VE)) == 0;
  const int64_t Cv = vec_ok ? (C / VE) * VE : 0;
  constexpr bool K32 = sizeof(DT) == 4;
  unsigned int* best32 = reinterpret_cast<unsigned int*>(s_code);
  const bool streamed = K32 && pre;
  MixStream ms = {};
  if (streamed) ms = mix_stream_of(ws, q, K);
  if (K32 && !streamed) {
    for (int k = tid; k < K; k += blockDim.x) best32[k] = 0xffffffffu;
    __syncthreads();
  }
  auto pass1 = [&](int64_t c, DT dv, int cd) {
    if ((unsigned)cd >= (unsigned)K) return;
    const double d = (double)dv;
    double lo;
    if constexpr (K32) {
      const unsigned int key = order_key((float)dv);
      unsigned int old = *reinterpret_cast<volatile unsigned int*>(&best32[cd]);
      if (key < old) old = atomicMin(&best32[cd], key);
      lo = (double)key_value(old < key ? old : key, 0.f);
    } else {
      const unsigned long long key = (unsigned long long)order_key(d);
      unsigned long long old = *reinterpret_cast<volatile unsigned long long*>(&best[cd]);
      if (key < old) old = atomicMin(&best[cd], key);
      lo = key_value(old < key ? old : key, 0.0);
    }
    if (d <= lo + eps1) {
      const int pp = atomicAdd(&ctl[4], 1);
      if (pp < MIX_POT) {
        pot_c[pp] = (int)c;
        pot_k[pp] = (int16_t)cd;
      }
    }
  };
  if (!streamed) {
#pragma unroll 4
    for (int64_t c = (int64_t)tid * VE; c < Cv; c += (int64_t)blockDim.x * VE) {
      const vecD d = *reinterpret_cast<const vecD*>(row + c);
      const vecC cd = *reinterpret_cast<const vecC*>(cand_code + c);
#pragma unroll
      for (int e = 0; e < VE; ++e) pass1(c + e, d[e], cd[e]);
    }
    for (int64_t c = Cv + tid; c < C; c += blockDim.x) pass1(c, row[c], cand_code[c]);
    __syncthreads();
  }
  int g_pot = 0;
  if (K32) {
    for (int k = tid; k < K; k += blockDim.x) {
      unsigned int b;
      if (streamed && MIX_INV_ATOMIC) {
        b = ~ms.inv[k];
        ms.inv[k] = 0;
      } else if (streamed) {
        unsigned int iv[MIX_SPLIT], mx = 0u;
#pragma unroll
        for (int sl = 0; sl < MIX_SPLIT; ++sl) iv[sl] = ms.inv[(size_t)sl * K + k];
#pragma unroll
        for (int sl = 0; sl < MIX_SPLIT; ++sl) mx = iv[sl] > mx ? iv[sl] : mx;
        b = ~mx;
      } else {
        b = best32[k];
      }
      best[k] = b == 0xffffffffu ? ~0ull : (unsigned long long)order_key((double)key_value(b, 0.f));
    }
    if (streamed) {
#pragma unroll
      for (int sl = 0; sl < MIX_SPLIT; ++sl) {
        const int ns = ms.cnt[sl];
        g_pot = (ns < 0 || g_pot < 0) ? -1 : g_pot + ns;
      }
    }
    __syncthreads();
  }
  SEL_STAMP(1);
  auto pass2 = [&](int64_t c, double d, int cd) {
    if ((unsigned)cd >= (unsigned)K) return;
    const unsigned long long bk = best[cd];
    if ((unsigned long long)order_key(d) == bk) atomicMin(&besti[cd], (unsigned int)(c + idx_base));
    else if (d > key_value(bk, 0.0) + eps1) return;
    if (atomicAdd(&near_[cd], 1u) == 1u) ctl[1] = 1;
    const int pp = atomicAdd(&ctl[3], 1);
    if (pp < MIX_LIST) {
      p_c[pp] = (int)c;
      p_k[pp] = (int16_t)cd;
    }
  };
  if (streamed && g_pot >= 0) {
    int seg_end[MIX_SPLIT];
    {
      int acc = 0;
#pragma unroll
      for (int sl = 0; sl < MIX_SPLIT; ++sl) {
        acc += ms.cnt[sl];
        seg_end[sl] = acc;
      }
    }
    constexpr int UE = 4;
    for (int e0 = tid; e0 < g_pot; e0 += (int)blockDim.x * UE) {
      int pc_[UE], pk_[UE];
      float pd_[UE];
#pragma unroll
      for (int u = 0; u < UE; ++u) {
        const int e = e0 + u * (int)blockDim.x;
        pk_[u] = -1;
        if (e < g_pot) {
          int sl = 0, first = 0;
#pragma unroll
          for (int i = 0; i < MIX_SPLIT - 1; ++i)
            if (e >= seg_end[i]) {
              sl = i + 1;
              first = seg_end[i];
            }
          const int pos = sl * MIX_SPOT + e - first;
          pc_[u] = ms.pot_c[pos];
          pd_[u] = ms.pot_d[pos];
          pk_[u] = ms.pot_k[pos];
        }
      }
#pragma unroll
      for (int u = 0; u < UE; ++u)
        if (pk_[u] >= 0) pass2(pc_[u], (double)pd_[u], pk_[u]);
    }
  } else if (!streamed && ctl[4] <= MIX_POT) {
    const int npot = ctl[4];
    for (int e = tid; e < npot; e += blockDim.x) pass2(pot_c[e], (double)row[pot_c[e]], pot_k[e]);
  } else {
#pragma unroll 4
    for (int64_t c = (int64_t)tid * VE; c < Cv; c += (int64_t)blockDim.x * VE) {
      const vecD d = *reinterpret_cast<const vecD*>(row + c);
      const vecC cd = *reinterpret_cast<const vecC*>(cand_code + c);
#pragma unroll
      for (int e = 0; e < VE; ++e) pass2(c + e, (double)d[e], cd[e]);
    }
    for (int64_t c = Cv + tid; c < C; c += blockDim.x) pass2(c, (double)row[c], cand_code[c]);
  }
  __syncthreads();
  if (streamed && tid < MIX_SPLIT) ms.cnt[tid] = 0;
  SEL_STAMP(2);
  for (int k = tid; k < K; k += blockDim.x) v[k] = besti[k] != 0xffffffffu ? key_value(best[k], 0.0) : absent;
  __syncthreads();
  const bool cut = RC.pos_t != nullptr && streamed && out_rank != nullptr && phase == 1;
  unsigned char* need2 = nullptr;
  if (cut) {
    unsigned char* cs = reinterpret_cast<unsigned char*>(pot_c);
    const int Kp = rank_sort_pow2(K);
    unsigned long long* skey2 = reinterpret_cast<unsigned long long*>(cs);
// ... 204 lines not shown
      w_v[k] = v[k];
      w_bi[k] = besti[k];
      w_nr[k] = near_[k];
    }
    for (int e = tid; e < n; e += blockDim.x) {
      w_lc[e] = l_c[e];
      w_lk[e] = l_k[e];
    }
    if (tid == 0) {
      w_n[0] = n;
      w_n[1] = order_parked ? 1 : 0;
    }
    SEL_STAMP(6);
    return;
  }
  if (phase == 2) {
    const unsigned long long* w_best = reinterpret_cast<const unsigned long long*>(wq);
    const double* w_v = reinterpret_cast<const double*>(wq + 8 * (size_t)K);
    const unsigned int* w_bi = reinterpret_cast<const unsigned int*>(wq + 16 * (size_t)K);
    const unsigned int* w_nr = w_bi + K;
    const int* w_n = reinterpret_cast<const int*>(wq + 24 * (size_t)K);
    const int* w_lc = w_n + 4;
    const int* w_lk = w_lc + MIX_LIST;
    const double* w_ld = reinterpret_cast<const double*>(w_lk + MIX_LIST);
    n = w_n[0];
    for (int k = tid; k < K; k += blockDim.x) {
      best[k] = w_best[k];
      v[k] = w_v[k];
      besti[k] = w_bi[k];
      near_[k] = w_nr[k];
    }
    for (int e = tid; e < n; e += blockDim.x) {
      l_c[e] = w_lc[e];
      l_k[e] = w_lk[e];
      l_d[e] = w_ld[e];
    }
    if (RC.pos_t) {
      unsigned char* isref = reinterpret_cast<unsigned char*>(pot_c);
      for (int k = tid; k < K; k += blockDim.x) isref[k] = 0;
      __syncthreads();
      for (int e = tid; e < n; e += blockDim.x) isref[w_lk[e]] = 1;
    }
    __syncthreads();
  }
  SEL_STAMP(7);
  if (n > 0) {
    const double qq = qn2[q];
    const bool fast = use_qlds != 0;
    if (phase == 0 && fast) {
      const int D4 = (A.n_taps * A.F) >> 2;
      const f32x4* src = reinterpret_cast<const f32x4*>(A.q32 + (int64_t)q * A.n_taps * A.F);
      for (int i = tid; i < D4; i += blockDim.x) reinterpret_cast<f32x4*>(qlds)[i] = src[i];
      __syncthreads();
    }
    for (int e = wv; e < n && phase == 0; e += nwv) {
      const int c = l_c[e];
      const double dot = fast ? pair_dot_fast_f64<4>(A, qlds, c, lane) : pair_dot_wave_f64(A, q, c, lane);
      if (lane == 0) l_d[e] = cosine_from_dot(dot, qq, cn2[c]);
    }
    for (int k = tid; k < K; k += blockDim.x)
      if (near_[k] >= 2) {
        rk[k] = (int)besti[k];
        best[k] = ~0ull;
        besti[k] = 0xffffffffu;
        s_code[k] = 0;
      }
    __syncthreads();
    for (int e = tid; e < n; e += blockDim.x) atomicMin(&best[l_k[e]], (unsigned long long)order_key(l_d[e]));
    __syncthreads();
    if (A.eps > 0.0) {
      for (int e = tid; e < n; e += blockDim.x)
        if (l_d[e] <= key_value(best[l_k[e]], 0.0) + A.eps) atomicAdd(&s_code[l_k[e]], 1);
      __syncthreads();
      for (int e = tid; e < n; e += blockDim.x)
        if (s_code[l_k[e]] >= 2 && l_d[e] <= key_value(best[l_k[e]], 0.0) + A.eps) {
          const int pos = atomicAdd(&ctl[2], 1);
          if (pos < MIX_LIST2) l2[pos] = e;
        }
      __syncthreads();
      int n2 = ctl[2];
      if (n2 > MIX_LIST2) {
        n2 = MIX_LIST2;
        if (tid == 0) atomicOr(&A.stats[1], 1);
      }
      if (n2 > 0) {
        for (int i0 = 0; i0 < n2; i0 += blockDim.x / 4) {
          const int i = i0 + (tid >> 2);
          const int e = l2[i < n2 ? i : 0];
          const double dr = refine_pair_f64(A, q, l_c[e], tid & 3);
          if (i < n2 && (tid & 3) == 0) {
            l_d[e] = dr;
            refd[l_k[e]] = 1;
          }
        }
        __syncthreads();
        for (int k = tid; k < K; k += blockDim.x)
          if (refd[k]) best[k] = ~0ull;
        __syncthreads();
        for (int i = tid; i < n2; i += blockDim.x)
          atomicMin(&best[l_k[l2[i]]], (unsigned long long)order_key(l_d[l2[i]]));
        __syncthreads();
        if (tid == 0) atomicAdd(&A.stats[0], n2);
      }
    }
    for (int e = tid; e < n; e += blockDim.x)
      if ((unsigned long long)order_key(l_d[e]) == best[l_k[e]])
        atomicMin(&besti[l_k[e]], (unsigned int)(l_c[e] + idx_base));
    __syncthreads();
    for (int k = tid; k < K; k += blockDim.x)
      if (near_[k] >= 2) {
        if (best[k] != ~0ull) v[k] = key_value(best[k], 0.0);
        else besti[k] = (unsigned int)rk[k];
      }
    if (tid == 0) atomicAdd(&A.stats[2], n);
    __syncthreads();
  }
  for (int k = tid; k < K; k += blockDim.x) {
    const bool have = besti[k] != 0xffffffffu;
    out_dist[(int64_t)q * K + k] = v[k];
    out_idx[(int64_t)q * K + k] = have ? (int32_t)besti[k] : -1;
  }
  SEL_STAMP(8);
  if (!out_rank) return;
  if (tid == 0) ctl[2] = 0;
  __syncthreads();
  bool repaired = false;
  if (phase == 2 && RC.pos_t && reinterpret_cast<const int*>(wq + 24 * (size_t)K)[1] == 1) {
    const int16_t* w_order = reinterpret_cast<const int16_t*>(wq + mix_park_order_off(K));
    for (int r = tid; r < K; r += blockDim.x) s_code[r] = w_order[r];
    __syncthreads();
    for (int round = 0; round < 24 && !repaired; ++round) {
      if (tid == 0) ctl[5] = 0;
      __syncthreads();
#pragma unroll
      for (int parity = 0; parity < 2; ++parity) {
        for (int r = 2 * tid + parity; r + 1 < K; r += 2 * blockDim.x) {
          const int ka = s_code[r], kb = s_code[r + 1];
          if (rank_gt(rank_sort_key(v[ka]), ka, rank_sort_key(v[kb]), kb)) {
            s_code[r] = kb;
            s_code[r + 1] = ka;
            ctl[5] = 1;
          }
        }
        __syncthreads();
      }
      repaired = ctl[5] == 0;
      __syncthreads();
    }
    if (repaired)
      for (int r = tid; r < K; r += blockDim.x) out_rank[(int64_t)q * K + s_code[r]] = (int16_t)r;
  }
  if (!repaired) rank_pass(true);
  SEL_STAMP(9);
  if (A.eps <= 0.0) return;
  __syncthreads();
  for (int r = tid; r + 1 < K; r += blockDim.x) {
    const int ka = s_code[r], kb = s_code[r + 1];
    if (besti[ka] == 0xffffffffu || besti[kb] == 0xffffffffu) continue;
    if (phase == 2 && RC.pos_t &&
        !(reinterpret_cast<const unsigned char*>(pot_c)[ka] && reinterpret_cast<const unsigned char*>(pot_c)[kb]))
      continue;
    if (v[kb] - v[ka] < A.eps) {
#pragma unroll
      for (int h = 0; h < 2; ++h) {
        const int k = h ? kb : ka;
        if (atomicExch(&near_[k], 0xffffffffu) == 0xffffffffu || refd[k]) continue;
        const int pos = atomicAdd(&ctl[2], 1);
        if (pos < MIX_LIST2) {
          l2[pos] = k;
        }
      }
    }
  }
  __syncthreads();
  int n3 = ctl[2];
  SEL_STAMP(10);
  if (n3 == 0) return;
  if (n3 > MIX_LIST2) {
    n3 = MIX_LIST2;
    if (tid == 0) atomicOr(&A.stats[1], 1);
  }
  for (int i0 = 0; i0 < n3; i0 += blockDim.x / 4) {
    const int i = i0 + (tid >> 2);
    const int k = l2[i < n3 ? i : 0];
    const double dr = refine_pair_f64(A, q, (int64_t)(besti[k] - (unsigned int)idx_base), tid & 3);
    if (i < n3 && (tid & 3) == 0) {
      v[k] = dr;
      out_dist[(int64_t)q * K + k] = dr;
    }
  }
  if (tid == 0) atomicAdd(&A.stats[0], n3);
  __syncthreads();
  SEL_STAMP(11);
  rank_pass(true);
  SEL_STAMP(12);
}

extern "C" int64_t qpg_percode_select_mixed_ws_bytes(int Q, int K) {
  return (Q <= 0 || K <= 0) ? 0 : (int64_t)((size_t)Q * mix_ws_stride(K));
}
extern "C" int64_t qpg_percode_select_mixed_ws_stride(int K) {
  return K <= 0 ? 0 : (int64_t)mix_ws_stride(K);
}

static int select_mixed_impl(const char* name, qpg_ctx* ctx, void* stream, const void* D, int d_is_f32, int64_t ldD, int Q,
                             const int16_t* cand_code, int64_t C, int K, double absent,
                             int32_t idx_base, double* out_dist, int32_t* out_idx, int16_t* out_rank,
                             int q_block, int64_t block_stride, const float* base, int T, int F,
                             const int32_t* cand_t, int G, int n_taps, int tap_stride,
                             const float* q32, const double* qn2, const double* cn2, double eps1,
                             double eps2, int32_t* stats, void* ws, int64_t ws_bytes, int base_is_f16,
                             const RankCut* cut = nullptr) {
  QPG_REQUIRE(ctx && D && (cand_code || C == 0) && out_dist && out_idx && base && cand_t && q32 && qn2 && cn2 && stats,
              "%s: null pointer", name);
  QPG_REQUIRE(Q >= 0 && C >= 0 && K > 0 && K <= 512 && ldD >= C && C + (int64_t)idx_base < 0x7fffffffll,
              "%s: bad size (K <= 512)", name);
  QPG_REQUIRE(T > 0 && F > 0 && (F % 4) == 0 && G > 0 && n_taps > 0 && tap_stride > 0 && C % G == 0 &&
                  eps1 >= 2.0 * QPG_AUDIO_HL_ERR && eps2 >= 0.0 && eps2 < eps1,
              "%s: bad geometry (F %% 4 == 0) or eps (eps1 >= 2 x the sweep's error bound - at least %g -, 0 <= eps2 < eps1)",
              name, 2.0 * (double)QPG_AUDIO_HL_ERR);
  QPG_REQUIRE(q_block >= 0 && (q_block == 0 || (!out_rank && Q % q_block == 0 && block_stride % 8 == 0)),
              "%s: block layout needs Q %% q_block == 0, an 8-byte multiple stride and no rank output", name);
  if (Q == 0) return QPG_OK;
  GuardArgs A;
  A.base = base; A.half = base_is_f16; A.q32 = q32; A.cand_t = cand_t; A.T = T; A.F = F; A.G = G; A.n_taps = n_taps;
  A.tap_stride = tap_stride; A.eps = eps2; A.stats = stats;
  const int use_qlds = (n_taps == 6 && F == 1024) ? 1 : 0;
  const size_t sh2 = 32 * (size_t)K + 16 * MIX_LIST + 4 * MIX_LIST2 + 32 + 6 * MIX_LIST + 4 * (size_t)K;
  size_t sh2c = sh2;
  const RankCut RCnone = {nullptr, nullptr, 1, 0};
  const size_t sh1 = sh2 + 6 * MIX_POT;
  const size_t sh = sh1 + (use_qlds ? (size_t)n_taps * F * 4 : 0);
  if (!ctx->select_lds_raised) {
    if (hipFuncSetAttribute(reinterpret_cast<const void*>(percode_select_mixed_f64_kernel<double>),
                            hipFuncAttributeMaxDynamicSharedMemorySize, 128 * 1024) != hipSuccess ||
        hipFuncSetAttribute(reinterpret_cast<const void*>(percode_select_mixed_f64_kernel<float>),
                            hipFuncAttributeMaxDynamicSharedMemorySize, 128 * 1024) != hipSuccess) {
      qpg_set_error("%s: cannot raise the dynamic LDS limit", name);
      return QPG_EHIP;
    }
    ctx->select_lds_raised = true;
  }
  unsigned char* w = static_cast<unsigned char*>(ws);
  if (ws)
    QPG_REQUIRE(ws_bytes >= qpg_percode_select_mixed_ws_bytes(Q, K) && (reinterpret_cast<uintptr_t>(ws) % 16) == 0,
                "%s: workspace too small or misaligned (qpg_percode_select_mixed_ws_bytes)", name);
#define SEL_MIX_LAUNCH(DT, SH, PHASE, PRE)                                                                                  \
  hipLaunchKernelGGL((percode_select_mixed_f64_kernel<DT>), dim3(Q), dim3(1024), SH, qpg_stream(stream),               \
                     static_cast<const DT*>(D), ldD, cand_code, C, K, absent, idx_base, out_dist, out_idx, out_rank,   \
                     q_block, block_stride, A, eps1, cn2, qn2, use_qlds, PHASE, w, PRE, RCv)
  RankCut RCv = RCnone;
  if (!ws) {
    if (d_is_f32) SEL_MIX_LAUNCH(float, sh, 0, 0); else SEL_MIX_LAUNCH(double, sh, 0, 0);
    QPG_LAUNCH_CHECK("percode_select_mixed_f64_kernel");
    return QPG_OK;
  }
  if (d_is_f32) {
    const size_t shs = 4 * (size_t)K + 10 * (size_t)MIX_SPOT;
    hipLaunchKernelGGL(mixed_stream_kernel, dim3(Q, MIX_SPLIT), dim3(1024), shs, qpg_stream(stream),
                       static_cast<const float*>(D), ldD, cand_code, C, K, eps1, w);
    QPG_LAUNCH_CHECK("mixed_stream_kernel");
    if (cut && cut->pos_t && out_rank) {
      RCv = *cut;
      sh2c = sh2 + 12 * (size_t)rank_sort_pow2(K) + 8 * (size_t)((K + 7) / 8 * 8) + 17 * 8 + 64 * (8 + 8 + 4) +
             16 * (size_t)K;
    }
    SEL_MIX_LAUNCH(float, sh2c, 1, 1);
  } else {
    SEL_MIX_LAUNCH(double, sh1, 1, 0);
  }
  QPG_LAUNCH_CHECK("percode_select_mixed_f64_kernel (lists)");
  const int rb = Q >= 512 ? 8 : (Q >= 128 ? 16 : 64);
  hipLaunchKernelGGL((select_refine_kernel<4>), dim3(Q, rb), dim3(256), 0, qpg_stream(stream), A, K, cn2, qn2, w, use_qlds);
  QPG_LAUNCH_CHECK("select_refine_kernel");
  if (d_is_f32) SEL_MIX_LAUNCH(float, sh2c, 2, 0); else SEL_MIX_LAUNCH(double, sh2, 2, 0);
  QPG_LAUNCH_CHECK("percode_select_mixed_f64_kernel (merge)");
#undef SEL_MIX_LAUNCH
  return QPG_OK;
}

extern "C" int qpg_percode_select_mixed_f64(qpg_ctx* ctx, void* stream, const void* D, int d_is_f32, int64_t ldD, int Q,
                                            const int16_t* cand_code, int64_t C, int K, double absent,
                                            int32_t idx_base, double* out_dist, int32_t* out_idx, int16_t* out_rank,
                                            int q_block, int64_t block_stride, const float* base, int T, int F,
                                            const int32_t* cand_t, int G, int n_taps, int tap_stride,
                                            const float* q32, const double* qn2, const double* cn2, double eps1,
                                            double eps2, int32_t* stats, void* ws, int64_t ws_bytes, int base_is_f16) {
  return select_mixed_impl("qpg_percode_select_mixed_f64", ctx, stream, D, d_is_f32, ldD, Q, cand_code, C, K, absent, idx_base,
                           out_dist, out_idx, out_rank, q_block, block_stride, base, T, F, cand_t, G, n_taps, tap_stride, q32,
                           qn2, cn2, eps1, eps2, stats, ws, ws_bytes, base_is_f16);
}

extern "C" int qpg_percode_select_mixed_f64_cut(qpg_ctx* ctx, void* stream, const void* D, int d_is_f32, int64_t ldD, int Q,
                                                const int16_t* cand_code, int64_t C, int K, double absent,
                                                int32_t idx_base, double* out_dist, int32_t* out_idx, int16_t* out_rank,
                                                int q_block, int64_t block_stride, const float* base, int T, int F,
                                                const int32_t* cand_t, int G, int n_taps, int tap_stride,
                                                const float* q32, const double* qn2, const double* cn2, double eps1,
                                                double eps2, int32_t* stats, void* ws, int64_t ws_bytes, int base_is_f16,
                                                const int16_t* pos_rank_t, const int16_t* freq_rank, int top_n, int probe) {
  const char* name = "qpg_percode_select_mixed_f64_cut";
  QPG_REQUIRE(pos_rank_t && freq_rank && out_rank && ws && d_is_f32 && q_block == 0 && (top_n == 1 || top_n == 2) &&
                  probe >= 0,
              "%s: needs the rank tables, out_rank, an f32 matrix, a workspace, no block layout, top_n 1 or 2", name);
  RankCut rc = {pos_rank_t, freq_rank, top_n, probe > 0 ? probe : 64};
  return select_mixed_impl(name, ctx, stream, D, d_is_f32, ldD, Q, cand_code, C, K, absent, idx_base, out_dist, out_idx,
                           out_rank, q_block, block_stride, base, T, F, cand_t, G, n_taps, tap_stride, q32, qn2, cn2, eps1, eps2,
                           stats, ws, ws_bytes, base_is_f16, &rc);
}

template <typename T, typename KeyT, bool PACKED>
static int percode_select(const char* name, qpg_ctx* ctx, void* stream, const T* D, int64_t ldD, int Q,
                          const int16_t* cand_code, int64_t C, int K, T absent, int32_t idx_base, T* out_dist,
                          int32_t* out_idx, int16_t* out_rank, int q_block, int64_t block_stride) {
  QPG_REQUIRE(ctx && D && (cand_code || C == 0) && out_dist && out_idx, "%s: null pointer", name);
  QPG_REQUIRE(Q >= 0 && C >= 0 && K > 0 && K <= 2048 && ldD >= C && C + (int64_t)idx_base < 0x7fffffffll,
              "%s: bad size (K <= 2048, candidate indices must stay below 2^31)", name);
  QPG_REQUIRE(q_block >= 0 && (q_block == 0 || (!out_rank && Q % q_block == 0 && block_stride % 8 == 0)),
              "%s: block layout needs Q %% q_block == 0, an 8-byte multiple stride and no rank output", name);
  if (Q == 0) return QPG_OK;
  const size_t sh = 12 * (size_t)rank_sort_pow2(K) + (size_t)K * sizeof(T);
  hipLaunchKernelGGL((percode_select_kernel<T, KeyT, PACKED>), dim3(Q), dim3(1024), sh, qpg_stream(stream), D, ldD,
                     cand_code, C, K, absent, idx_base, out_dist, out_idx, out_rank, q_block, block_stride);
  QPG_LAUNCH_CHECK(name);
  return QPG_OK;
}

extern "C" int qpg_percode_select_f64(qpg_ctx* ctx, void* stream, const double* D, int64_t ldD, int Q,
                                      const int16_t* cand_code, int64_t C, int K, double absent, int32_t idx_base,
                                      double* out_dist, int32_t* out_idx, int16_t* out_rank, int q_block,
                                      int64_t block_stride) {
  return percode_select<double, unsigned long long, false>("qpg_percode_select_f64", ctx, stream, D, ldD, Q, cand_code,
                                                           C, K, absent, idx_base, out_dist, out_idx, out_rank, q_block,
                                                           block_stride);
}
extern "C" int qpg_percode_select_f32(qpg_ctx* ctx, void* stream, const float* D, int64_t ldD, int Q,
                                      const int16_t* cand_code, int64_t C, int K, float absent, int32_t idx_base,
                                      float* out_dist, int32_t* out_idx, int16_t* out_rank, int q_block,
                                      int64_t block_stride) {
  return percode_select<float, unsigned int, true>("qpg_percode_select_f32", ctx, stream, D, ldD, Q, cand_code, C, K,
                                                   absent, idx_base, out_dist, out_idx, out_rank, q_block, block_stride);
}

struct ExactWs {
  double* wmin;
  double* list_d;
  int32_t* widx;
  unsigned int* near_;
  int* list_c;
  int* cnt;
};
__host__ static size_t exact_ws_layout(int Q, int64_t C, int K, unsigned char* b, ExactWs* w) {
  size_t o = 0;
  const size_t QK = (size_t)Q * K, QC = (size_t)Q * (size_t)C;
  if (w) w->wmin = reinterpret_cast<double*>(b + o);
  o += QK * 8;
  if (w) w->list_d = reinterpret_cast<double*>(b + o);
  o += QC * 8;
  if (w) w->widx = reinterpret_cast<int32_t*>(b + o);
  o += QK * 4;
  if (w) w->near_ = reinterpret_cast<unsigned int*>(b + o);
  o += QK * 4;
  if (w) w->list_c = reinterpret_cast<int*>(b + o);
  o += QC * 4;
  if (w) w->cnt = reinterpret_cast<int*>(b + o);
  o += ((size_t)Q * 4 + 15) / 16 * 16;
  return o;
}

__global__ void exact_zero_kernel(unsigned int* __restrict__ near_, int64_t n, int* __restrict__ cnt, int Q) {
  const int64_t i = (int64_t)blockIdx.x * blockDim.x + threadIdx.x;
  if (i < n) near_[i] = 0;
  if (i < Q) cnt[i] = 0;
}

__global__ __launch_bounds__(256) void exact_band_kernel(const double* __restrict__ D, int64_t ldD,
                                                         const int16_t* __restrict__ cand_code, int64_t C, int K,
                                                         double eps, ExactWs W) {
  const int q = blockIdx.x;
  const double* row = D + (int64_t)q * ldD;
  for (int64_t c = (int64_t)blockIdx.y * blockDim.x + threadIdx.x; c < C; c += (int64_t)gridDim.y * blockDim.x) {
    const int cd = cand_code[c];
    if ((unsigned)cd >= (unsigned)K) continue;
    if (row[c] <= W.wmin[(int64_t)q * K + cd] + eps) {
      atomicAdd(&W.near_[(int64_t)q * K + cd], 1u);
      const int pos = atomicAdd(&W.cnt[q], 1);
      W.list_c[(int64_t)q * C + pos] = (int)c;
    }
  }
}

__global__ __launch_bounds__(256) void exact_refine_kernel(GuardArgs A, const int16_t* __restrict__ cand_code, int64_t C,
                                                           int K, ExactWs W) {
  const int q = blockIdx.x, tid = threadIdx.x;
  const int n = W.cnt[q];
  for (int e0 = blockIdx.y * 64; e0 < n; e0 += gridDim.y * 64) {
    const int e = e0 + (tid >> 2);
    int c = 0;
    bool need = false;
    if (e < n) {
      c = W.list_c[(int64_t)q * C + e];
      need = W.near_[(int64_t)q * K + cand_code[c]] >= 2;
    }
    if (__ballot(need) == 0ull) continue;
    const double dr = refine_pair_f64(A, q, need ? c : 0, tid & 3);
    if (need && (tid & 3) == 0) W.list_d[(int64_t)q * C + e] = dr;
  }
}

__global__ __launch_bounds__(1024) void exact_merge_kernel(const int16_t* __restrict__ cand_code, int64_t C, int K,
                                                           double absent, int32_t idx_base, double* __restrict__ out_dist,
                                                           int32_t* __restrict__ out_idx, int16_t* __restrict__ out_rank,
                                                           int q_block, int64_t block_stride, GuardArgs A, ExactWs W) {
  extern __shared__ __attribute__((aligned(16))) unsigned char smem[];
  unsigned long long* best = reinterpret_cast<unsigned long long*>(smem);
  double* v = reinterpret_cast<double*>(smem + 8 * (size_t)K);
  unsigned int* besti = reinterpret_cast<unsigned int*>(smem + 16 * (size_t)K);
  unsigned int* nearl = besti + K;
  int* s_code = reinterpret_cast<int*>(nearl + K);
  int* rkc = s_code + K;
  int* l2 = rkc + K;
  int* ctl = l2 + K;
  const int q = blockIdx.x, tid = threadIdx.x;
  if (q_block > 0) {
    const int64_t shift = (int64_t)(q / q_block) * block_stride;
    const int64_t rowoff = (int64_t)(q % q_block) * K - (int64_t)q * K;
    out_dist = reinterpret_cast<double*>(reinterpret_cast<unsigned char*>(out_dist) + shift) + rowoff;
// ... 671 lines not shown
```

qpgesture_amd/csrc/qpg_sorted.hip:

```cpp
#include "qpg_common.h"

__device__ __forceinline__ unsigned int okey32(float d) {
  const unsigned int b = __float_as_uint(d);
  return (b >> 31) ? ~b : (b | 0x80000000u);
}
__device__ __forceinline__ float okey32_value(unsigned int k) {
  return __uint_as_float((k >> 31) ? (k & 0x7fffffffu) : ~k);
}

#define SORT_SPLIT 8
#define SORT_LIST 2048
#define SORT_TILES 1024
#define SORT_THREADS 256

__global__ __launch_bounds__(SORT_THREADS) void percode_select_sorted_kernel(
    const float* __restrict__ Dm, int64_t ldD, const float* __restrict__ tmin, const uint16_t* __restrict__ tmask,
    int64_t ldT, int64_t R, const int16_t* __restrict__ row_code, const int32_t* __restrict__ row_index, const int32_t* __restrict__ zero_row,
    const int32_t* __restrict__ code_tile, int K, float band, const float* __restrict__ qn, const float* __restrict__ xs,
    int Dd, float absent, float* __restrict__ out_dist, int32_t* __restrict__ out_idx, int32_t* __restrict__ stats,
    int32_t idx_base, int q_block, int64_t block_stride) {
  extern __shared__ __attribute__((aligned(16))) unsigned char smem[];
  const int S = gridDim.y, s = blockIdx.y;
  const int k0 = (int)((int64_t)s * K / S), k1 = (int)((int64_t)(s + 1) * K / S), KL = k1 - k0;
  const int KLmax = ((K + S - 1) / S + 4) & ~3;
  unsigned long long* ebest = reinterpret_cast<unsigned long long*>(smem);
  unsigned int* best = reinterpret_cast<unsigned int*>(ebest + KLmax);
  int* list = reinterpret_cast<int*>(best + KLmax);
  int* tl = list + SORT_LIST;
  float* qrow = reinterpret_cast<float*>(tl + SORT_TILES);
  __shared__ int n_list, n_tiles;
  const int q = blockIdx.x, tid = threadIdx.x;
  const float* row = Dm ? Dm + (int64_t)q * ldD : nullptr;
  const float* trow = tmin + (int64_t)q * ldT;
  const uint16_t* mrow = tmask ? tmask + (int64_t)q * ldT : nullptr;
  const int t0 = code_tile[k0], t1 = code_tile[k1];
  for (int k = tid; k < KL; k += blockDim.x) {
    ebest[k] = ~0ull;
    best[k] = (zero_row && zero_row[k0 + k] >= 0) ? okey32(0.5f) : 0xffffffffu;
  }
  for (int i = tid; i < Dd / 4; i += blockDim.x)
    reinterpret_cast<f32x4*>(qrow)[i] = reinterpret_cast<const f32x4*>(qn + (int64_t)q * Dd)[i];
  if (tid == 0) {
    n_list = 0;
    n_tiles = 0;
  }
  __syncthreads();
  for (int t = t0 + tid; t < t1; t += blockDim.x) {
    const int code = (row_code[(int64_t)t * 16] & 0x1fff) - k0;
    if ((unsigned)code < (unsigned)KL) atomicMin(&best[code], okey32(trow[t]));
  }
  __syncthreads();
  if (band >= 0.f) {
    for (int t = t0 + tid; t < t1; t += blockDim.x) {
      const int code = (row_code[(int64_t)t * 16] & 0x1fff) - k0;
      if ((unsigned)code >= (unsigned)KL) continue;
      if (trow[t] <= okey32_value(best[code]) + band) {
        const int pos = atomicAdd(&n_tiles, 1);
        if (pos < SORT_TILES) tl[pos] = t;
      }
    }
    for (int k = tid; k < KL; k += blockDim.x)
      if (zero_row && zero_row[k0 + k] >= 0 && 0.5f <= okey32_value(best[k]) + band) {
        const int pos = atomicAdd(&n_list, 1);
        if (pos < SORT_LIST) list[pos] = (int)R + k0 + k;
      }
    __syncthreads();
    int nt = n_tiles;
    if (nt > SORT_TILES) {
      nt = SORT_TILES;
      if (tid == 0 && stats) atomicOr(&stats[1], 16);
    }
    for (int i = tid >> 4; i < nt; i += blockDim.x >> 4) {
      const int64_t r = (int64_t)tl[i] * 16 + (tid & 15);
      const int cd = row_code[r];
      if (cd & 0x4000) continue;
      const bool in = mrow ? ((mrow[tl[i]] >> (tid & 15)) & 1) != 0
                           : row[r] <= okey32_value(best[(cd & 0x1fff) - k0]) + band;
      if (in) {
        const int pos = atomicAdd(&n_list, 1);
        if (pos < SORT_LIST) list[pos] = (int)r;
      }
    }
  }
  __syncthreads();
  int n = n_list;
  if (n > SORT_LIST) {
    n = SORT_LIST;
    if (tid == 0 && stats) atomicOr(&stats[1], 16);
  }
  for (int e = tid; e < n; e += blockDim.x) {
    const int r = list[e];
    const bool z = r >= (int)R;
    const f32x4* xp = reinterpret_cast<const f32x4*>(xs + (int64_t)(z ? (int)R : r) * Dd);
    const f32x4* qp = reinterpret_cast<const f32x4*>(qrow);
    float a0 = 0.f, a1 = 0.f, a2 = 0.f, a3 = 0.f;
    for (int g0 = 0; g0 < Dd / 16; g0 += 4) {
      f32x4 xv[16];
#pragma unroll
      for (int i = 0; i < 16; ++i) xv[i] = (g0 * 4 + i) < Dd / 4 ? xp[g0 * 4 + i] : (f32x4){0.f, 0.f, 0.f, 0.f};
#pragma unroll
      for (int gg = 0; gg < 4; ++gg) {
        if (g0 + gg >= Dd / 16) break;
#pragma unroll
        for (int u = 3; u >= 0; --u) {
          const f32x4 x = xv[gg * 4 + u], qq = qp[(g0 + gg) * 4 + u];
          const float d0 = f_sub(qq.x, x.x), d1 = f_sub(qq.y, x.y), d2 = f_sub(qq.z, x.z), d3 = f_sub(qq.w, x.w);
          a0 = f_add(f_mul(d0, d0), a0);
          a1 = f_add(f_mul(d1, d1), a1);
          a2 = f_add(f_mul(d2, d2), a2);
          a3 = f_add(f_mul(d3, d3), a3);
        }
      }
    }
    const float dist = f_mul(0.5f, f_add(f_add(a0, a1), f_add(a2, a3)));
    const int cd = z ? r - (int)R : (row_code[r] & 0x1fff);
    const int oi = z ? zero_row[cd] : row_index[r];
    atomicMin(&ebest[cd - k0], ((unsigned long long)okey32(dist) << 32) | (unsigned int)oi);
  }
  __syncthreads();
  if (q_block > 0) {
    const int64_t shift = (int64_t)(q / q_block) * block_stride;
    const int64_t rowoff = (int64_t)(q % q_block) * K - (int64_t)q * K;
    out_dist = reinterpret_cast<float*>(reinterpret_cast<unsigned char*>(out_dist) + shift) + rowoff;
    out_idx = reinterpret_cast<int32_t*>(reinterpret_cast<unsigned char*>(out_idx) + shift) + rowoff;
  }
  for (int k = tid; k < KL; k += blockDim.x) {
    const unsigned long long kv = ebest[k];
    const bool have = kv != ~0ull;
    out_dist[(int64_t)q * K + k0 + k] = have ? okey32_value((unsigned int)(kv >> 32)) : absent;
    out_idx[(int64_t)q * K + k0 + k] = have ? (int32_t)(kv & 0xffffffffu) + idx_base : -1;
  }
}

__global__ __launch_bounds__(256) void sorted_finish_kernel(const float* __restrict__ dist, const int32_t* __restrict__ idx,
                                                             int K, int16_t* __restrict__ out_rank,
                                                             int32_t* __restrict__ out_nn) {
  extern __shared__ __attribute__((aligned(16))) unsigned char smem[];
  unsigned long long* skey = reinterpret_cast<unsigned long long*>(smem);
  int* scode = reinterpret_cast<int*>(skey + rank_sort_pow2(K));
  float* v = reinterpret_cast<float*>(scode + rank_sort_pow2(K));
  __shared__ unsigned long long nn_key;
  const int q = blockIdx.x, tid = threadIdx.x, lane = tid & 63;
  if (tid == 0) nn_key = ~0ull;
  unsigned long long mine = ~0ull;
  for (int k = tid; k < K; k += blockDim.x) {
    const float dv = dist[(int64_t)q * K + k];
    const int iv = idx[(int64_t)q * K + k];
    v[k] = dv;
    if (iv >= 0) {
      const unsigned long long kv = ((unsigned long long)okey32(dv) << 32) | (unsigned int)iv;
      if (kv < mine) mine = kv;
    }
  }
  __syncthreads();
  if (out_nn) {
    for (int o = 32; o > 0; o >>= 1) {
      const unsigned long long other = __shfl_xor(mine, o, 64);
      mine = other < mine ? other : mine;
    }
    if (lane == 0 && mine != ~0ull) atomicMin(&nn_key, mine);
    __syncthreads();
    if (tid == 0) out_nn[q] = nn_key != ~0ull ? (int32_t)(nn_key & 0xffffffffu) : -1;
  }
  if (!out_rank) return;
  block_sorted_ranks(v, K, skey, scode, [&](int k, int r) { out_rank[(int64_t)q * K + k] = (int16_t)r; });
}

extern "C" int qpg_percode_select_sorted_f32(qpg_ctx* ctx, void* stream, const float* Dm, int64_t ldD, const float* tile_min,
                                             const uint16_t* tile_mask, int64_t ldT, int Q, int64_t R,
                                             const int16_t* row_code,
                                             const int32_t* row_index, const int32_t* zero_row, const int32_t* code_tile,
                                             int K, float band, const float* qn, const float* xs, int Dd, float absent,
                                             float* out_dist, int32_t* out_idx, int16_t* out_rank, int32_t* out_nn,
                                             int32_t* stats, int32_t idx_base, int q_block, int64_t block_stride) {
  const char* name = "qpg_percode_select_sorted_f32";
  QPG_REQUIRE(ctx && (Dm || tile_mask) && tile_min && row_code && row_index && code_tile && qn && xs && out_dist && out_idx,
              "%s: null pointer", name);
  QPG_REQUIRE(Q >= 0 && R > 0 && (R % 16) == 0 && R < 0x7fffffffll - 0x2000 && (!Dm || ldD >= R) && ldT >= R / 16 && K > 0 &&
                  K <= 2048 && K <= 0x1fff && Dd > 0 && (Dd % 16) == 0 && (reinterpret_cast<uintptr_t>(xs) % 16) == 0 &&
                  (reinterpret_cast<uintptr_t>(qn) % 16) == 0,
              "%s: bad size / alignment (R %% 16 == 0, D %% 16 == 0, K <= 2048)", name);
  QPG_REQUIRE(q_block >= 0 && idx_base >= 0 &&
                  (q_block == 0 || (!out_rank && !out_nn && Q % q_block == 0 && block_stride % 8 == 0)),
              "%s: block layout needs Q %% q_block == 0, an 8-byte multiple stride and no rank / nn output", name);
  if (Q == 0) return QPG_OK;
  const int S = K >= 32 * SORT_SPLIT ? SORT_SPLIT : (K >= 32 ? K / 32 : 1);
  const int KLmax = ((K + S - 1) / S + 4) & ~3;
  const size_t sh = 12 * (size_t)KLmax + 4 * (size_t)SORT_LIST + 4 * (size_t)SORT_TILES + 4 * (size_t)Dd;
  QPG_REQUIRE(sh <= 64 * 1024, "%s: K / D too large for the LDS tables", name);
  hipLaunchKernelGGL(percode_select_sorted_kernel, dim3(Q, S), dim3(SORT_THREADS), sh, qpg_stream(stream), Dm, ldD, tile_min,
                     tile_mask, ldT, R, row_code, row_index, zero_row, code_tile, K, band, qn, xs, Dd, absent, out_dist, out_idx, stats,
                     idx_base, q_block, block_stride);
  QPG_LAUNCH_CHECK("percode_select_sorted_kernel");
  if (out_rank || out_nn) {
    hipLaunchKernelGGL(sorted_finish_kernel, dim3(Q), dim3(256), 12 * (size_t)rank_sort_pow2(K) + 4 * (size_t)K, qpg_stream(stream),
                       (const float*)out_dist, (const int32_t*)out_idx, K, out_rank, out_nn);
    QPG_LAUNCH_CHECK("sorted_finish_kernel");
  }
  return QPG_OK;
}

__global__ __launch_bounds__(256) void perm32_kernel(const float* __restrict__ x, int64_t n32, float* __restrict__ y) {
  for (int64_t i = (int64_t)blockIdx.x * blockDim.x + threadIdx.x; i < n32; i += (int64_t)gridDim.x * blockDim.x) {
    const f32x4* p = reinterpret_cast<const f32x4*>(x) + i * 8;
    f32x4 u[8];
#pragma unroll
    for (int v = 0; v < 8; ++v) u[v] = p[v];
    f32x4* o = reinterpret_cast<f32x4*>(y) + i * 8;
#pragma unroll
    for (int k = 0; k < 4; ++k) {
      o[2 * k] = (f32x4){u[3][k], u[2][k], u[1][k], u[0][k]};
      o[2 * k + 1] = (f32x4){u[7][k], u[6][k], u[5][k], u[4][k]};
    }
  }
}

extern "C" int qpg_perm32_rows_f32(qpg_ctx* ctx, void* stream, const float* x, int64_t R, int D, float* y) {
  QPG_REQUIRE(ctx && x && y && x != y && R >= 0 && D > 0 && (D % 32) == 0 && (reinterpret_cast<uintptr_t>(x) % 16) == 0 &&
                  (reinterpret_cast<uintptr_t>(y) % 16) == 0,
              "qpg_perm32_rows_f32: bad argument (D %% 32 == 0, 16-byte aligned, out of place)");
  const int64_t n32 = R * (D / 32);
  if (n32 == 0) return QPG_OK;
  const int64_t nb = (n32 + 255) / 256;
  hipLaunchKernelGGL(perm32_kernel, dim3((unsigned)(nb < 16384 ? nb : 16384)), dim3(256), 0, qpg_stream(stream), x, n32, y);
  QPG_LAUNCH_CHECK("perm32_kernel");
  return QPG_OK;
}

#define BYC_THREADS 512
#define BYC_QMAX 2048
#define BYC_LIST 1024

template <int PT>
__global__ __launch_bounds__(BYC_THREADS) void percode_select_bycode_kernel(
    const float* __restrict__ tmin_t, const uint16_t* __restrict__ tmask_t, int64_t ldQ, int Q, int64_t R,
    const int16_t* __restrict__ row_code, const int32_t* __restrict__ row_index, const int32_t* __restrict__ zero_row,
    const int32_t* __restrict__ code_tile, int K, float band, const float* __restrict__ qp, const float* __restrict__ xsp,
    int Dd, float absent, float* __restrict__ out_dist, int32_t* __restrict__ out_idx, int32_t* __restrict__ stats,
    int32_t idx_base) {
  extern __shared__ __attribute__((aligned(16))) unsigned char smem[];
  const int rowb = Dd * 4;
  float* rows0 = reinterpret_cast<float*>(smem);
  unsigned long long* ebest = reinterpret_cast<unsigned long long*>(smem + (size_t)17 * rowb);
  float* cmin = reinterpret_cast<float*>(ebest + Q);
  int* list_q = reinterpret_cast<int*>(cmin + Q);
  int* list_r = list_q + BYC_LIST;
  __shared__ int n_list[2];
  const int code = blockIdx.x, tid = threadIdx.x;
  const int t0 = code_tile[code], t1 = code_tile[code + 1], nt = t1 - t0;
  const int zr = zero_row ? zero_row[code] : -1;
  const int nv = Dd / 4;
  for (int q = tid; q < Q; q += BYC_THREADS) {
    const float* tp = tmin_t + (int64_t)t0 * ldQ + q;
    float m = zr >= 0 ? 0.5f : __builtin_inff();
    for (int t = 0; t < nt; t += 8) {
      float v[8];
#pragma unroll
      for (int i = 0; i < 8; ++i) v[i] = t + i < nt ? tp[(int64_t)(t + i) * ldQ] : __builtin_inff();
#pragma unroll
      for (int i = 0; i < 8; ++i) m = fminf(m, v[i]);
    }
    cmin[q] = m;
    ebest[q] = ~0ull;
  }
  for (int i = tid; i < nv; i += BYC_THREADS)
    reinterpret_cast<f32x4*>(rows0 + 16 * Dd)[i] = (f32x4){0.f, 0.f, 0.f, 0.f};
  if (tid == 0) n_list[0] = n_list[1] = 0;
  f32x4 stage[PT];
  float nmin[BYC_QMAX / BYC_THREADS];
  unsigned int nmask[BYC_QMAX / BYC_THREADS];
  auto fetch = [&](int t) {
    const f32x4* src = reinterpret_cast<const f32x4*>(xsp + (int64_t)(t0 + t) * 16 * Dd);
#pragma unroll
    for (int u = 0; u < PT; ++u) {
      const int i = u * BYC_THREADS + tid;
      stage[u] = i < 16 * nv ? src[i] : (f32x4){0.f, 0.f, 0.f, 0.f};
    }
    const int64_t to = (int64_t)(t0 + t) * ldQ;
#pragma unroll
    for (int u = 0; u < BYC_QMAX / BYC_THREADS; ++u) {
      const int q = u * BYC_THREADS + tid;
      nmin[u] = q < Q ? tmin_t[to + q] : __builtin_inff();
      nmask[u] = q < Q ? tmask_t[to + q] : 0u;
    }
  };
  auto commit = [&]() {
    f32x4* dst = reinterpret_cast<f32x4*>(rows0);
#pragma unroll
    for (int u = 0; u < PT; ++u) {
      const int i = u * BYC_THREADS + tid;
      if (i < 16 * nv) dst[i] = stage[u];
    }
  };
  if (nt > 0 && band >= 0.f) {
    fetch(0);
    commit();
  }
  __syncthreads();
  const int k4 = tid & 3;
  const int G32 = Dd / 32;
  for (int t = 0; t < nt && band >= 0.f; ++t) {
    float vmin[BYC_QMAX / BYC_THREADS];
    unsigned int vmask[BYC_QMAX / BYC_THREADS];
#pragma unroll
    for (int u = 0; u < BYC_QMAX / BYC_THREADS; ++u) {
      vmin[u] = nmin[u];
      vmask[u] = nmask[u];
    }
    if (t + 1 < nt) fetch(t + 1);
#pragma unroll
    for (int u = 0; u < BYC_QMAX / BYC_THREADS; ++u) {
      const int q = u * BYC_THREADS + tid;
      if (q >= Q) break;
      const float lim = cmin[q] + band;
      if (vmin[u] <= lim) {
        unsigned int bits = vmask[u];
        while (bits) {
          const int r = __builtin_ctz(bits);
          bits &= bits - 1;
          if (row_code[(int64_t)(t0 + t) * 16 + r] & 0x4000) continue;
          const int pos = atomicAdd(&n_list[t & 1], 1);
          if (pos < BYC_LIST) {
            list_q[pos] = q;
            list_r[pos] = r;
          }
        }
      }
      if (t == 0 && zr >= 0 && 0.5f <= lim) {
        const int pos = atomicAdd(&n_list[t & 1], 1);
        if (pos < BYC_LIST) {
          list_q[pos] = q;
          list_r[pos] = 16;
        }
      }
    }
    __syncthreads();
    int n = n_list[t & 1];
    if (tid == 0) n_list[(t + 1) & 1] = 0;
    if (n > BYC_LIST) {
      n = BYC_LIST;
      if (tid == 0 && stats) atomicOr(&stats[1], 16);
    }
    const float* rb = rows0;
    for (int e0 = 0; e0 < n; e0 += BYC_THREADS / 4) {
      const int e = e0 + (tid >> 2);
      const bool on = e < n;
      const int q = on ? list_q[e] : 0, r = on ? list_r[e] : 16;
      const f32x4* xp = reinterpret_cast<const f32x4*>(rb + (size_t)r * Dd) + 2 * k4;
      const f32x4* qv = reinterpret_cast<const f32x4*>(qp + (int64_t)q * Dd) + 2 * k4;
      float a = 0.f;
      for (int g0 = 0; g0 < G32; g0 += 8) {
        f32x4 qq[16];
#pragma unroll
        for (int i = 0; i < 8; ++i) {
          const bool in = g0 + i < G32;
          qq[2 * i] = in ? qv[(g0 + i) * 8] : (f32x4){0.f, 0.f, 0.f, 0.f};
          qq[2 * i + 1] = in ? qv[(g0 + i) * 8 + 1] : (f32x4){0.f, 0.f, 0.f, 0.f};
        }
#pragma unroll
        for (int i = 0; i < 16; ++i) {
          if (g0 + (i >> 1) >= G32) break;
          const f32x4 xv = xp[(g0 + (i >> 1)) * 8 + (i & 1)];
#pragma unroll
          for (int j = 0; j < 4; ++j) {
            const float d = f_sub(qq[i][j], xv[j]);
            a = f_add(f_mul(d, d), a);
          }
        }
      }
      const float s01 = f_add(a, __shfl_xor(a, 1, 64));
      const float s = f_add(s01, __shfl_xor(s01, 2, 64));
      if (on && k4 == 0) {
        const float dist = f_mul(0.5f, s);
        const int oi = r == 16 ? zr : row_index[(int64_t)(t0 + t) * 16 + r];
        atomicMin(&ebest[q], ((unsigned long long)okey32(dist) << 32) | (unsigned int)oi);
      }
    }
    __syncthreads();
    if (t + 1 < nt) commit();
  }
  if (nt == 0 && zr >= 0 && band >= 0.f) {
    for (int q = tid; q < Q; q += BYC_THREADS) {
      const float* qr = qp + (int64_t)q * Dd;
      float a0 = 0.f, a1 = 0.f, a2 = 0.f, a3 = 0.f;
      for (int G = 0; G < G32; ++G)
        for (int j = 0; j < 8; ++j) {
          const float d0 = qr[G * 32 + j], d1 = qr[G * 32 + 8 + j], d2 = qr[G * 32 + 16 + j], d3 = qr[G * 32 + 24 + j];
          a0 = f_add(f_mul(d0, d0), a0);
          a1 = f_add(f_mul(d1, d1), a1);
          a2 = f_add(f_mul(d2, d2), a2);
          a3 = f_add(f_mul(d3, d3), a3);
        }
      const float dist = f_mul(0.5f, f_add(f_add(a0, a1), f_add(a2, a3)));
      ebest[q] = ((unsigned long long)okey32(dist) << 32) | (unsigned int)zr;
    }
    __syncthreads();
  }
  for (int q = tid; q < Q; q += BYC_THREADS) {
    const unsigned long long kv = ebest[q];
    const bool have = kv != ~0ull;
    out_dist[(int64_t)q * K + code] = have ? okey32_value((unsigned int)(kv >> 32)) : absent;
    out_idx[(int64_t)q * K + code] = have ? (int32_t)(kv & 0xffffffffu) + idx_base : -1;
  }
}

extern "C" int qpg_percode_select_bycode_f32(qpg_ctx* ctx, void* stream, const float* tile_min_t, const uint16_t* tile_mask_t,
                                             int64_t ldQ, int Q, int64_t R, const int16_t* row_code,
                                             const int32_t* row_index, const int32_t* zero_row, const int32_t* code_tile,
                                             int K, float band, const float* qn_perm, const float* xs_perm, int Dd,
                                             float absent, float* out_dist, int32_t* out_idx, int16_t* out_rank,
                                             int32_t* out_nn, int32_t* stats, int32_t idx_base) {
  const char* name = "qpg_percode_select_bycode_f32";
  QPG_REQUIRE(ctx && tile_min_t && tile_mask_t && row_code && row_index && code_tile && qn_perm && xs_perm && out_dist && out_idx,
              "%s: null pointer", name);
  QPG_REQUIRE(Q >= 0 && ldQ >= Q && R > 0 && (R % 16) == 0 && R < 0x7fffffffll - 0x2000 && K > 0 && K <= 0x1fff && Dd > 0 &&
                  (Dd % 128) == 0 && Dd <= 1024 && (reinterpret_cast<uintptr_t>(xs_perm) % 16) == 0 &&
                  (reinterpret_cast<uintptr_t>(qn_perm) % 16) == 0 && idx_base >= 0,
              "%s: bad size / alignment (R %% 16 == 0, D %% 128 == 0, D <= 1024)", name);
  if (Q == 0) return QPG_OK;
  static bool raised = false;
  if (!raised) {
    bool ok = true;
#define BYC_RAISE(PT_) ok = ok && hipFuncSetAttribute(reinterpret_cast<const void*>(percode_select_bycode_kernel<PT_>), \
                                                      hipFuncAttributeMaxDynamicSharedMemorySize, 96 * 1024) == hipSuccess
    BYC_RAISE(1); BYC_RAISE(2); BYC_RAISE(3); BYC_RAISE(4); BYC_RAISE(5); BYC_RAISE(6); BYC_RAISE(7); BYC_RAISE(8);
#undef BYC_RAISE
    if (!ok) {
      qpg_set_error("%s: cannot raise the dynamic LDS limit", name);
      return QPG_EHIP;
    }
    raised = true;
  }
  for (int qa = 0; qa < Q; qa += BYC_QMAX) {
    const int qn = Q - qa < BYC_QMAX ? Q - qa : BYC_QMAX;
    const size_t sh = (size_t)17 * Dd * 4 + 12 * (size_t)qn + 8 * (size_t)BYC_LIST;
    QPG_REQUIRE(sh <= 96 * 1024, "%s: LDS tables too large", name);
#define BYC_GO(PT_) hipLaunchKernelGGL(percode_select_bycode_kernel<PT_>, dim3(K), dim3(BYC_THREADS), sh, qpg_stream(stream), \
                                       tile_min_t + qa, tile_mask_t + qa, ldQ, qn, R, row_code, row_index, zero_row, code_tile, K, \
                                       band, qn_perm + (int64_t)qa * Dd, xs_perm, Dd, absent, out_dist + (int64_t)qa * K,           \
                                       out_idx + (int64_t)qa * K, stats, idx_base)
    switch (Dd / 128) {
      case 1: BYC_GO(1); break;
      case 2: BYC_GO(2); break;
      case 3: BYC_GO(3); break;
      case 4: BYC_GO(4); break;
      case 5: BYC_GO(5); break;
      case 6: BYC_GO(6); break;
      case 7: BYC_GO(7); break;
      default: BYC_GO(8); break;
    }
#undef BYC_GO
    QPG_LAUNCH_CHECK("percode_select_bycode_kernel");
  }
  if (out_rank || out_nn) {
    hipLaunchKernelGGL(sorted_finish_kernel, dim3(Q), dim3(256), 12 * (size_t)rank_sort_pow2(K) + 4 * (size_t)K, qpg_stream(stream),
                       (const float*)out_dist, (const int32_t*)out_idx, K, out_rank, out_nn);
    QPG_LAUNCH_CHECK("sorted_finish_kernel");
  }
  return QPG_OK;
}
```

qpgesture_amd/csrc/qpg_tail.hip:

```cpp
#include "qpg_common.h"
#include <type_traits>

__global__ __launch_bounds__(256) void l2_table_kernel(const float* __restrict__ sig, int K, int Dm,
                                                       float* __restrict__ out) {
  const int p = blockIdx.x;
  for (int c = threadIdx.x; c < K; c += blockDim.x) {
    double s = 0.0;
    for (int e = 0; e < Dm; ++e) {
      const float d = f_sub(sig[(int64_t)p * Dm + e], sig[(int64_t)c * Dm + e]);
      s += (double)d * (double)d;
    }
    out[(int64_t)p * K + c] = (c == p) ? __builtin_inff() : (float)sqrt(s);
  }
}

extern "C" int qpg_l2_table_f32(qpg_ctx* ctx, void* stream, const float* sig, int K, int Dm, float* out) {
  QPG_REQUIRE(ctx && sig && out && K > 0 && Dm > 0, "qpg_l2_table_f32: bad argument");
  hipLaunchKernelGGL(l2_table_kernel, dim3(K), dim3(256), 0, qpg_stream(stream), sig, K, Dm, out);
  QPG_LAUNCH_CHECK("l2_table_kernel");
  return QPG_OK;
}

__device__ __forceinline__ float lane4_sum(float v, int l) {
  const float o1 = __shfl_xor(v, 1, 64);
  const float pair = (l & 1) ? f_add(o1, v) : f_add(v, o1);
  const float o2 = __shfl_xor(pair, 2, 64);
  return (l & 2) ? f_add(o2, pair) : f_add(pair, o2);
}

__device__ __forceinline__ float einsum_sq_128(const float* v, int l) {
  float a = 0.f;
#pragma unroll
  for (int g = 0; g < 8; ++g) {
#pragma unroll
    for (int u = 3; u >= 0; --u) {
      const float x = v[g * 16 + u * 4 + l];
      a = f_add(f_mul(x, x), a);
    }
  }
  return lane4_sum(a, l);
}

struct ArgMin {
  double v;
  int i;
};
__device__ __forceinline__ ArgMin amin(ArgMin a, ArgMin b) {
  return (b.v < a.v || (b.v == a.v && b.i < a.i)) ? b : a;
}
__device__ __forceinline__ ArgMin wave_argmin(ArgMin m) {
#pragma unroll
  for (int o = 32; o > 0; o >>= 1) {
    ArgMin t{__shfl_xor(m.v, o, 64), __shfl_xor(m.i, o, 64)};
    m = amin(m, t);
  }
  return m;
}

#define QPG_KMAX_PER_LANE 16

__global__ __launch_bounds__(256) void fuse_best_kernel(const int16_t* __restrict__ rank0,
                                                        const int32_t* __restrict__ idx0,
                                                        const int16_t* __restrict__ rank1,
                                                        const int32_t* __restrict__ idx1,
                                                        const int16_t* __restrict__ pos_rank,
                                                        const int16_t* __restrict__ freq_rank, int Q, int K, int mode,
                                                        int32_t* __restrict__ T0, int32_t* __restrict__ T1) {
  const int lane = threadIdx.x & 63;
  const int64_t task = (int64_t)blockIdx.x * 4 + (threadIdx.x >> 6);
  if (task >= (int64_t)Q * K) return;
  const int q = (int)(task / K), p = (int)(task - (int64_t)q * K);
  if (mode == 0) {
    const int16_t* ra = rank0 + (int64_t)q * K;
    const int16_t* rt = rank1 + (int64_t)q * K;
    ArgMin ma{__builtin_inf(), 0x7fffffff}, mt{__builtin_inf(), 0x7fffffff};
#pragma unroll
    for (int i = 0; i < QPG_KMAX_PER_LANE; ++i) {
      const int c = lane + 64 * i;
      if (c < K) {
        const double pos_score = (double)pos_rank[(int64_t)p * K + c] + (double)freq_rank[c] * 0.05;
        ma = amin(ma, ArgMin{pos_score + (double)ra[c], c});
        mt = amin(mt, ArgMin{pos_score + (double)rt[c], c});
      }
    }
    ma = wave_argmin(ma);
    mt = wave_argmin(mt);
    if (lane == 0) {
      T0[task] = idx0[(int64_t)q * K + ma.i];
      T1[task] = idx1[(int64_t)q * K + mt.i];
    }
    return;
  }
  const int16_t* rk = (mode == 1 ? rank0 : rank1) + (int64_t)q * K;
  const int32_t* ix = (mode == 1 ? idx0 : idx1) + (int64_t)q * K;
  ArgMin m{__builtin_inf(), 0x7fffffff};
  double vals[QPG_KMAX_PER_LANE];
#pragma unroll
  for (int i = 0; i < QPG_KMAX_PER_LANE; ++i) {
    const int c = lane + 64 * i;
    vals[i] = __builtin_inf();
    if (c < K) {
      const double pos_score = (double)pos_rank[(int64_t)p * K + c] + (double)freq_rank[c] * 0.05;
      vals[i] = pos_score + (double)rk[c];
      m = amin(m, ArgMin{vals[i], c});
    }
  }
  m = wave_argmin(m);
  ArgMin m2{__builtin_inf(), 0x7fffffff};
#pragma unroll
  for (int i = 0; i < QPG_KMAX_PER_LANE; ++i) {
    const int c = lane + 64 * i;
    if (c < K && c != m.i) m2 = amin(m2, ArgMin{vals[i], c});
  }
  m2 = wave_argmin(m2);
  if (lane == 0) {
    T0[task] = ix[m.i];
    T1[task] = ix[m2.i];
  }
}

__global__ __launch_bounds__(256) void fuse_best_ranked_kernel(const int16_t* __restrict__ rank0,
                                                               const int32_t* __restrict__ idx0,
                                                               const int16_t* __restrict__ rank1,
                                                               const int32_t* __restrict__ idx1,
                                                               const int16_t* __restrict__ pos_rank,
                                                               const int16_t* __restrict__ freq_rank, int Q, int K,
                                                               int32_t* __restrict__ T0, int32_t* __restrict__ T1) {
  extern __shared__ __attribute__((aligned(16))) int16_t inv[];
  __shared__ int bad;
  const int tid = threadIdx.x, l16 = tid & 15;
  const int64_t task = (int64_t)blockIdx.x * 16 + (tid >> 4);
  const int q = (int)(((int64_t)blockIdx.x * 16) / K);
  const int p = (int)(task - (int64_t)q * K);
  if (tid == 0) bad = 0;
  for (int c = tid; c < 2 * K; c += blockDim.x) inv[c] = -1;
  __syncthreads();
  for (int c = tid; c < K; c += blockDim.x) {
    const int ra = rank0[(int64_t)q * K + c], rt = rank1[(int64_t)q * K + c];
    if ((unsigned)ra < (unsigned)K) inv[ra] = (int16_t)c; else bad = 1;
    if ((unsigned)rt < (unsigned)K) inv[K + rt] = (int16_t)c; else bad = 1;
  }
  __syncthreads();
  for (int c = tid; c < 2 * K; c += blockDim.x)
    if (inv[c] < 0) bad = 1;
  __syncthreads();
  const bool full = bad != 0;
  const int16_t* pr = pos_rank + (int64_t)p * K;
  auto xchg = [](ArgMin m, auto tag) {
    constexpr int PJ = decltype(tag)::value;
    const unsigned long long b = (unsigned long long)__double_as_longlong(m.v);
    const unsigned int lo = (unsigned int)lane_xor<PJ>((int)(unsigned int)b);
    const unsigned int hi = (unsigned int)lane_xor<PJ>((int)(unsigned int)(b >> 32));
    return ArgMin{__longlong_as_double((long long)(((unsigned long long)hi << 32) | lo)), lane_xor<PJ>(m.i)};
// ... 214 lines not shown
          vb[k][tpos(e0 + 49)] = cur[k].head.y;
        }
      }
      CandRegs nxt[2][2];
      const bool spec = s + 1 < A.steps;
      if (spec) {
#pragma unroll
        for (int k = 0; k < 2; ++k) {
          const int pn = __shfl(cur[k].pay, 3, 64);
          nxt[k][0] = load_cand(A, 0, tab[(s + 1) * K + pn], s_cidx, s_pslot, lane);
          nxt[k][1] = load_cand(A, 1, tab[A.steps * K + (s + 1) * K + pn], s_cidx, s_pslot, lane);
        }
      }
      __syncthreads();
      if (lane < 16) {
        const int l = lane & 3, grp = lane >> 2;
        const float* v = (grp & 1) ? vb[grp >> 1] : va[grp >> 1];
        float n = f_sqrt(einsum_sq_128_t(v, l));
        if (n < eps10) n = 1.f;
        if (l == 0) nrm[grp] = n;
      }
      __syncthreads();
#pragma unroll
      for (int k = 0; k < 2; ++k) {
        const float na = nrm[2 * k], nb = nrm[2 * k + 1];
        const float2 xa = reinterpret_cast<const float2*>(va[k])[lane], xb = reinterpret_cast<const float2*>(vb[k])[lane];
        float2 d;
        d.x = f_sub(f_div(xa.x, na), f_div(xb.x, nb));
        d.y = f_sub(f_div(xa.y, na), f_div(xb.y, nb));
        reinterpret_cast<float2*>(va[k])[lane] = d;
      }
      __syncthreads();
      if (lane < 8) {
        const int l = lane & 3, k = lane >> 2;
        const float sc = f_mul(0.5f, einsum_sq_128_t(va[k], l));
        if (l == 0) score[k] = sc;
      }
      __syncthreads();
      const int fi = (score[1] < score[0]) ? 1 : 0;
      prev = fi ? cur[1].tail : cur[0].tail;
      reinterpret_cast<float2*>(A.out_phase + ((int64_t)w * A.steps + s) * 128)[lane] = prev;
      const int wpay = fi ? cur[1].pay : cur[0].pay;
      if (lane < A.step_codes) wincodes[s * A.step_codes + lane] = wpay;
      if (lane == 0) A.out_vote[w * A.steps + s] = fi;
      prev_code = __shfl(wpay, A.step_codes - 1, 64);
      if (spec) {
        cur[0] = fi ? nxt[1][0] : nxt[0][0];
        cur[1] = fi ? nxt[1][1] : nxt[0][1];
      }
    }
    __syncthreads();
    if (lane < A.codes_per_window) A.out_codes[(int64_t)w * A.codes_per_window + lane] = wincodes[lane];
    prev_code = wincodes[last_idx];
  }
  __threadfence_system();
  __syncthreads();
  if (lane == 0) {
    A.out_status[0] = bad;
    __threadfence_system();
    A.out_status[1] = A.guard_flags ? A.guard_flags[0] : 0;
  }
}


struct GateGeom {
  int s_last, off_last;
};

__device__ __forceinline__ const float* cand_block(const TailArgs& A, int which, int ci, int* pay_base) {
  const int G = which ? A.G1 : A.G0;
  const int cc = ci < 0 ? 0 : ci;
  const int j = cc / G, g = cc - j * G;
  const int ps = (which ? A.pslot1 : A.pslot0)[g];
  *pay_base = j * A.code_ld + (which ? A.cidx1 : A.cidx0)[g];
  return A.phase + ((int64_t)j * A.Tp + ps) * 16;
}

__device__ __forceinline__ unsigned int gate_eval(const TailArgs& A, int q, int p, const float* prev, int lane) {
  const int K = A.K;
  const int k = (lane >> 2) & 1, l = lane & 3;
  const int ck = (k ? A.T1 : A.T0)[(int64_t)q * K + p];
  int pb_unused;
  const float* head = cand_block(A, k, ck, &pb_unused);
  float xa[32], xb[32];
  float sa = 0.f, sb = 0.f;
#pragma unroll
  for (int g = 0; g < 8; ++g) {
#pragma unroll
    for (int u = 3; u >= 0; --u) {
      const int e = g * 16 + u * 4 + l;
      const float va = e < 80 ? prev[48 + e] : head[e - 80];
      const float vb = e < 48 ? prev[80 + e] : head[e - 48];
      xa[g * 4 + u] = va;
      xb[g * 4 + u] = vb;
      sa = f_add(f_mul(va, va), sa);
      sb = f_add(f_mul(vb, vb), sb);
    }
  }
  const float eps10 = 10.f * 1.1920928955078125e-07f;
  float na = f_sqrt(lane4_sum(sa, l)), nb = f_sqrt(lane4_sum(sb, l));
  if (na < eps10) na = 1.f;
  if (nb < eps10) nb = 1.f;
  float sd = 0.f;
#pragma unroll
  for (int g = 0; g < 8; ++g) {
#pragma unroll
    for (int u = 3; u >= 0; --u) {
      const float d = f_sub(f_div(xa[g * 4 + u], na), f_div(xb[g * 4 + u], nb));
      sd = f_add(f_mul(d, d), sd);
    }
  }
  const float score = f_mul(0.5f, lane4_sum(sd, l));
  const float other = __shfl_xor(score, 4, 64);
  const float s0 = k ? other : score, s1 = k ? score : other;
  const int fi = (s1 < s0) ? 1 : 0;
  return (unsigned int)((p << 1) | fi);
}

__device__ __forceinline__ const float* gate_prev(const TailArgs& A, const GateGeom& geo, int s, int kp, int ci, int* p) {
  int pb;
  const float* prev = cand_block(A, kp, ci, &pb) + 384;
  *p = A.code[pb + (s == 0 ? geo.off_last : A.step_codes - 1)];
  return prev;
}

__global__ __launch_bounds__(256) void gate_table_kernel(TailArgs A, GateGeom geo, uint16_t* __restrict__ Gt) {
  const int K = A.K, Qc = A.M * A.steps, Q = Qc * A.n_chains;
  const int lane = threadIdx.x & 63;
  const int64_t task = ((int64_t)blockIdx.x * 256 + threadIdx.x) >> 3;
  const int64_t n_task = (int64_t)Q * 2 * K;
  const bool live = task < n_task;
  const int q = live ? (int)(task / (2 * K)) : 0;
  const int sigma = live ? (int)(task - (int64_t)q * 2 * K) : 0;
  const int chain = q / Qc;
  const bool first = q == chain * Qc;
  if (first && sigma != 0) return;
  const int s = q % A.steps;
  int p;
  const float* prev;
  if (first) {
    p = A.seed_codes ? A.seed_codes[chain] : A.seed_code;
    prev = A.seed_phase + (int64_t)chain * 128;
  } else {
    const int pp = sigma >> 1, kp = sigma & 1;
    const int ci = (kp ? A.T1 : A.T0)[(int64_t)(q - 1) * K + pp];
    prev = gate_prev(A, geo, s, kp, ci, &p);
  }
  const unsigned int g = gate_eval(A, q, p, prev, lane);
  if (live && (lane & 7) == 0) Gt[task] = (uint16_t)g;
}

#define GD_SLOTS 2048
#define GD_THREADS 1024
__global__ __launch_bounds__(GD_THREADS) void gate_table_dedup_kernel(TailArgs A, GateGeom geo, uint16_t* __restrict__ Gt) {
  __shared__ int key[GD_SLOTS];
  __shared__ unsigned short val[GD_SLOTS];
  __shared__ unsigned short ulist[GD_SLOTS];
  __shared__ int n_u;
  const int K = A.K, Qc = A.M * A.steps, tid = threadIdx.x, lane = tid & 63;
  const int q = blockIdx.x, chain = q / Qc, s = q % A.steps;
  uint16_t* out = Gt + (int64_t)q * 2 * K;
  if (q == chain * Qc) {
    if (tid < 8) {
      const int p = A.seed_codes ? A.seed_codes[chain] : A.seed_code;
      const unsigned int g = gate_eval(A, q, p, A.seed_phase + (int64_t)chain * 128, lane);
      if (tid == 0) out[0] = (uint16_t)g;
    }
    return;
  }
  for (int i = tid; i < GD_SLOTS; i += GD_THREADS) key[i] = 0;
  if (tid == 0) n_u = 0;
  __syncthreads();
  constexpr int PER = 2 * 512 / GD_THREADS;
  int slot[PER];
#pragma unroll
  for (int u = 0; u < PER; ++u) {
    const int sigma = u * GD_THREADS + tid;
    slot[u] = -1;
    if (sigma < 2 * K) {
      const int pp = sigma >> 1, kp = sigma & 1;
      const int ci = (kp ? A.T1 : A.T0)[(int64_t)(q - 1) * K + pp];
      const int kv = (((ci < 0 ? 0 : ci) << 1) | kp) + 1;
      unsigned int h = ((unsigned int)kv * 2654435761u) >> 21;
      for (;;) {
        const int old = atomicCAS(&key[h], 0, kv);
        if (old == 0) {
          ulist[atomicAdd(&n_u, 1)] = (unsigned short)h;
          break;
        }
        if (old == kv) break;
        h = (h + 1) & (GD_SLOTS - 1);
      }
      slot[u] = (int)h;
    }
  }
  __syncthreads();
  const int nu = n_u;
  for (int u = tid >> 3; u < nu; u += GD_THREADS >> 3) {
    const int h = ulist[u], kv = key[h] - 1;
    int p;
    const float* prev = gate_prev(A, geo, s, kv & 1, kv >> 1, &p);
    const unsigned int g = gate_eval(A, q, p, prev, lane);
    if ((lane & 7) == 0) val[h] = (unsigned short)g;
  }
  __syncthreads();
#pragma unroll
  for (int u = 0; u < PER; ++u)
    if (slot[u] >= 0) out[u * GD_THREADS + tid] = val[slot[u]];
}

#define QPG_CHASE_QMAX 2048
__global__ __launch_bounds__(1024) void gate_chase_kernel(TailArgs A, const uint16_t* __restrict__ Gt) {
  extern __shared__ __attribute__((aligned(16))) uint16_t gl[];
  __shared__ uint16_t sig[QPG_CHASE_QMAX];
  __shared__ int bad_s;
  const int K = A.K, Q = A.M * A.steps, tid = threadIdx.x, nt = blockDim.x;
  const int per_w = A.steps * 2 * K;
  const int chain = blockIdx.x;
  const int64_t q0 = (int64_t)chain * Q;
  Gt += q0 * 2 * K;
  A.T0 += q0 * K;
  A.T1 += q0 * K;
  A.out_phase += q0 * 128;
  A.out_vote += q0;
  A.out_codes += (int64_t)chain * A.M * A.codes_per_window;
  A.out_status += (int64_t)chain * A.status_stride;
  if (tid == 0) bad_s = 0;
  int sigma = 0;
  auto stage = [&](int w, int first, int step) {
    const int4* src = reinterpret_cast<const int4*>(Gt + (int64_t)w * per_w);
    int4* dst = reinterpret_cast<int4*>(gl + (size_t)(w & 1) * per_w);
    for (int v = first; v < per_w / 8; v += step) dst[v] = src[v];
  };
  stage(0, tid, nt);
  __syncthreads();
  for (int w = 0; w < A.M; ++w) {
    if (tid >= 64 && w + 1 < A.M) stage(w + 1, tid - 64, nt - 64);
    if (tid == 0) {
      const uint16_t* g = gl + (size_t)(w & 1) * per_w;
      for (int s = 0; s < A.steps; ++s) {
        sigma = (w == 0 && s == 0) ? g[0] : g[s * 2 * K + sigma];
        sig[w * A.steps + s] = (uint16_t)sigma;
      }
    }
    __syncthreads();
  }
  for (int i = tid; i < Q * 32; i += nt) {
    const int q = i >> 5, v = i & 31;
    const int sg = sig[q], p = sg >> 1, fi = sg & 1;
    const int ci = (fi ? A.T1 : A.T0)[(int64_t)q * K + p];
    int pb;
    const float* blk = cand_block(A, fi, ci, &pb) + 384;
    reinterpret_cast<f32x4*>(A.out_phase + (int64_t)q * 128)[v] = reinterpret_cast<const f32x4*>(blk)[v];
    if (v == 0) {
      A.out_vote[q] = fi;
      if (A.T0[(int64_t)q * K + p] < 0 || A.T1[(int64_t)q * K + p] < 0) bad_s = 1;
    }
  }
  for (int i = tid; i < A.M * A.codes_per_window; i += nt) {
    const int w = i / A.codes_per_window, c = i - w * A.codes_per_window;
    const int q = w * A.steps + c / A.step_codes;
    const int sg = sig[q], p = sg >> 1, fi = sg & 1;
    const int ci = (fi ? A.T1 : A.T0)[(int64_t)q * K + p];
    int pb;
    cand_block(A, fi, ci, &pb);
    A.out_codes[i] = A.code[pb + c % A.step_codes];
  }
  __threadfence_system();
  __syncthreads();
  if (tid == 0) {
    A.out_status[0] = bad_s;
    __threadfence_system();
    A.out_status[1] = A.guard_flags ? A.guard_flags[0] : 0;
  }
}

#define QPG_TAKES_PER_BLOCK 64
__host__ __device__ __forceinline__ int64_t takes_trail_off(int n_takes) { return ((int64_t)n_takes + 7) & ~(int64_t)7; }

__global__ __launch_bounds__(256) void takes_step0_kernel(TailArgs A, int n_takes, uint16_t* __restrict__ step0) {
  const int lane = threadIdx.x & 63;
  const int task = (int)(((int64_t)blockIdx.x * 256 + threadIdx.x) >> 3);
  const bool live = task < n_takes;
  const int take = live ? task : n_takes - 1;
  int p = A.seed_codes[take];
  p = p < 0 ? 0 : (p >= A.K ? A.K - 1 : p);
  const unsigned int g = gate_eval(A, 0, p, A.seed_phase + (int64_t)take * 128, lane);
  if (live && (lane & 7) == 0) step0[take] = (uint16_t)g;
}

__global__ __launch_bounds__(1024) void gate_chase_takes_kernel(int M, int steps, int K, int n_takes,
                                                                const uint16_t* __restrict__ Gt,
                                                                const uint16_t* __restrict__ step0,
                                                                uint16_t* __restrict__ trail) {
  extern __shared__ __attribute__((aligned(16))) uint16_t gl[];
  const int tid = threadIdx.x, nt = blockDim.x;
  const int per_w = steps * 2 * K;
  const int take = blockIdx.x * QPG_TAKES_PER_BLOCK + tid;
  const bool chaser = tid < QPG_TAKES_PER_BLOCK && take < n_takes;
  auto stage = [&](int w, int first, int step) {
    const int4* src = reinterpret_cast<const int4*>(Gt + (int64_t)w * per_w);
    int4* dst = reinterpret_cast<int4*>(gl + (size_t)(w & 1) * per_w);
    for (int v = first; v < per_w / 8; v += step) dst[v] = src[v];
  };
  stage(0, tid, nt);
  __syncthreads();
  int sigma = chaser ? step0[take] : 0;
  for (int w = 0; w < M; ++w) {
    if (tid >= 64 && w + 1 < M) stage(w + 1, tid - 64, nt - 64);
    if (chaser) {
      const uint16_t* g = gl + (size_t)(w & 1) * per_w;
      for (int s = 0; s < steps; ++s) {
        if (w | s) sigma = g[s * 2 * K + sigma];
        trail[(int64_t)(w * steps + s) * n_takes + take] = (uint16_t)sigma;
      }
    }
    __syncthreads();
  }
}

__global__ __launch_bounds__(256) void takes_epilogue_kernel(TailArgs A, int n_takes, const uint16_t* __restrict__ trail) {
  __shared__ uint16_t sig[QPG_CHASE_QMAX];
  __shared__ int bad_s;
  const int K = A.K, Q = A.M * A.steps, tid = threadIdx.x, nt = blockDim.x;
  const int take = blockIdx.x;
  A.out_phase += (int64_t)take * Q * 128;
  A.out_vote += (int64_t)take * Q;
  A.out_codes += (int64_t)take * A.M * A.codes_per_window;
  A.out_status += (int64_t)take * A.status_stride;
  if (tid == 0) bad_s = 0;
  for (int q = tid; q < Q; q += nt) sig[q] = trail[(int64_t)q * n_takes + take];
  __syncthreads();
  for (int i = tid; i < Q * 32; i += nt) {
    const int q = i >> 5, v = i & 31;
    const int sg = sig[q], p = sg >> 1, fi = sg & 1;
    const int ci = (fi ? A.T1 : A.T0)[(int64_t)q * K + p];
    int pb;
    const float* blk = cand_block(A, fi, ci, &pb) + 384;
    reinterpret_cast<f32x4*>(A.out_phase + (int64_t)q * 128)[v] = reinterpret_cast<const f32x4*>(blk)[v];
    if (v == 0) {
      A.out_vote[q] = fi;
      if (A.T0[(int64_t)q * K + p] < 0 || A.T1[(int64_t)q * K + p] < 0) bad_s = 1;
    }
  }
  for (int i = tid; i < A.M * A.codes_per_window; i += nt) {
    const int w = i / A.codes_per_window, c = i - w * A.codes_per_window;
    const int q = w * A.steps + c / A.step_codes;
    const int sg = sig[q], p = sg >> 1, fi = sg & 1;
    const int ci = (fi ? A.T1 : A.T0)[(int64_t)q * K + p];
    int pb;
    cand_block(A, fi, ci, &pb);
    A.out_codes[i] = A.code[pb + c % A.step_codes];
  }
  __threadfence_system();
  __syncthreads();
  if (tid == 0) {
    A.out_status[0] = bad_s;
    __threadfence_system();
    A.out_status[1] = A.guard_flags ? A.guard_flags[0] : 0;
  }
}

__global__ void status_only_kernel(int32_t* out_status, const int32_t* guard_flags) {
  out_status[0] = 0;
  out_status[1] = guard_flags ? guard_flags[0] : 0;
}

extern "C" int qpg_fuse_best_ranked(qpg_ctx* ctx, void* stream, const int16_t* rank, const int32_t* idx,
                                    const int16_t* pos_rank, const int16_t* freq_rank, int Q, int K, int32_t* T) {
  QPG_REQUIRE(ctx && rank && idx && pos_rank && freq_rank && T, "qpg_fuse_best_ranked: null pointer");
  QPG_REQUIRE(Q > 0 && K > 0 && (K % 16) == 0 && K <= 4096 && ((int64_t)Q * K) / 16 < 0x7fffffffll,
              "qpg_fuse_best_ranked: K %% 16 == 0, K <= 4096");
  hipLaunchKernelGGL(fuse_best_ranked_one_kernel, dim3((unsigned)(((int64_t)Q * K) / 16)), dim3(256), 2 * (size_t)K,
                     qpg_stream(stream), rank, idx, pos_rank, freq_rank, Q, K, T);
  QPG_LAUNCH_CHECK("fuse_best_ranked_one_kernel");
  return QPG_OK;
}


static bool tabulated_walk_ok(bool serial_walk, int steps, int K, int Qc, GateGeom* geo) {
  const int codes_per_window = (steps * 4 < 30) ? steps * 4 : 30, last_idx = codes_per_window - 1;
  *geo = GateGeom{last_idx / 4, last_idx % 4};
  const size_t lds_g = (size_t)2 * steps * 2 * K * sizeof(uint16_t);
  return !serial_walk && geo->s_last == steps - 1 && 2 * K <= 65536 && Qc <= QPG_CHASE_QMAX && lds_g <= 64 * 1024 &&
         ((steps * 2 * K) % 8) == 0;
}

static int match_steps_impl(qpg_ctx* ctx, void* stream, const int16_t* aud_rank, const int32_t* aud_idx,
                            const int16_t* txt_rank, const int32_t* txt_idx, const int16_t* pos_rank,
                            const int16_t* freq_rank, const int32_t* code, int code_ld, const int32_t* aud_cidx,
                            const int32_t* aud_pslot, int Ga, const int32_t* txt_cidx, const int32_t* txt_pslot,
                            int Gt, const float* phase, int Tp, int mode, int M, int steps, int K, int seed_code,
                            const float* seed_phase, int32_t* gate_tables, int32_t* out_codes, float* out_phase,
                            int32_t* out_vote, int32_t* out_status, const int32_t* guard_flags, int n_chains,
                            const int32_t* seed_codes, int64_t status_stride, int n_takes = 0,
                            void* takes_ws = nullptr, size_t takes_ws_bytes = 0) {
  QPG_REQUIRE(ctx && pos_rank && freq_rank && code && phase && seed_phase && gate_tables && out_codes && out_phase &&
                  out_vote && out_status,
              "qpg_match_steps: null pointer");
  QPG_REQUIRE(n_chains >= 1 && (n_chains == 1 || (seed_codes && status_stride >= 2)),
              "qpg_match_steps_batch: n_chains >= 1, device seed codes and a status stride >= 2");
  const bool serial_walk = (mode & QPG_MODE_SERIAL_WALK) != 0;
  const bool prefused = (mode & QPG_MODE_PREFUSED) != 0;
  mode &= ~(QPG_MODE_SERIAL_WALK | QPG_MODE_PREFUSED);
  QPG_REQUIRE(!prefused || mode == 0, "qpg_match_steps: QPG_MODE_PREFUSED goes with the two-modality mode");
  QPG_REQUIRE(mode >= 0 && mode <= 2, "qpg_match_steps: bad mode %d", mode);
  QPG_REQUIRE(mode == QPG_MODE_TXT || (aud_rank && aud_idx && aud_cidx && aud_pslot && Ga > 0),
              "qpg_match_steps: audio tables missing");
  QPG_REQUIRE(mode == QPG_MODE_AUD || (txt_rank && txt_idx && txt_cidx && txt_pslot && Gt > 0),
              "qpg_match_steps: text tables missing");
  QPG_REQUIRE(M >= 0 && steps > 0 && steps * 4 <= 64 && K > 0 && K <= 64 * QPG_KMAX_PER_LANE && (K % 4) == 0 &&
                  seed_code >= 0 && seed_code < K && Ga <= 64 && Gt <= 64,
              "qpg_match_steps: bad size");
  const size_t lds = (size_t)2 * steps * K * sizeof(int32_t);
  QPG_REQUIRE(lds <= 96 * 1024, "qpg_match_steps: steps*K too large for the LDS gate tables");
  if (M == 0) {
    hipLaunchKernelGGL(status_only_kernel, dim3(1), dim3(1), 0, qpg_stream(stream), out_status, guard_flags);
    QPG_LAUNCH_CHECK("status_only_kernel");
    return QPG_OK;
  }
  const int Qc = M * steps;
  const int Q = Qc * n_chains;
  GateGeom geo;
  const bool tabulated = tabulated_walk_ok(serial_walk, steps, K, Qc, &geo);
  if (n_takes > 0 && !tabulated) {
    qpg_set_error("qpg_match_steps_takes: the tabulated walk does not apply (serial walk asked for, or steps = %d / K = %d "
                  "/ %d steps per clip outside its geometry)", steps, K, Qc);
    return QPG_EUNSUP;
  }
  QPG_REQUIRE(n_takes <= 0 || (takes_ws && takes_ws_bytes >= qpg_match_steps_takes_ws_bytes(n_takes, M, steps)),
              "qpg_match_steps_takes: workspace too small (qpg_match_steps_takes_ws_bytes)");
  int32_t* T0 = gate_tables;
  int32_t* T1 = gate_tables + (int64_t)Q * K;
  if (prefused) {
  } else if (mode == 0 && (K % 16) == 0 && K <= 4096) {
    hipLaunchKernelGGL(fuse_best_ranked_kernel, dim3((unsigned)(((int64_t)Q * K) / 16)), dim3(256), 4 * (size_t)K,
                       qpg_stream(stream), aud_rank, aud_idx, txt_rank, txt_idx, pos_rank, freq_rank, Q, K, T0, T1);
  } else {
    dim3 grid((unsigned)(((int64_t)Q * K + 3) / 4), 1);
    hipLaunchKernelGGL(fuse_best_kernel, grid, dim3(256), 0, qpg_stream(stream), aud_rank, aud_idx, txt_rank, txt_idx,
                       pos_rank, freq_rank, Q, K, mode, T0, T1);
  }
  QPG_LAUNCH_CHECK("fuse_best_kernel");
  TailArgs A;
  A.T0 = T0; A.T1 = T1; A.code = code; A.code_ld = code_ld;
  const bool txt0 = (mode == QPG_MODE_TXT), txt1 = (mode != QPG_MODE_AUD);
  A.cidx0 = txt0 ? txt_cidx : aud_cidx; A.pslot0 = txt0 ? txt_pslot : aud_pslot; A.G0 = txt0 ? Gt : Ga;
  A.cidx1 = txt1 ? txt_cidx : aud_cidx; A.pslot1 = txt1 ? txt_pslot : aud_pslot; A.G1 = txt1 ? Gt : Ga;
  A.phase = phase; A.Tp = Tp; A.M = M; A.steps = steps; A.step_codes = 4;
  A.codes_per_window = (steps * 4 < 30) ? steps * 4 : 30;
  A.K = K; A.seed_code = seed_code; A.seed_phase = seed_phase; A.seed_codes = seed_codes; A.n_chains = n_chains;
  A.status_stride = status_stride;
  A.out_codes = out_codes; A.out_phase = out_phase; A.out_vote = out_vote; A.out_status = out_status;
  A.guard_flags = guard_flags;
  const size_t lds_g = (size_t)2 * steps * 2 * K * sizeof(uint16_t);
  if (!tabulated) {
    QPG_REQUIRE(n_chains == 1, "qpg_match_steps_batch: the sequential walk takes one chain per call");
    hipLaunchKernelGGL(match_walk_kernel, dim3(1), dim3(64), lds, qpg_stream(stream), A);
    QPG_LAUNCH_CHECK("match_walk_kernel");
    return QPG_OK;
  }
  uint16_t* gtab = reinterpret_cast<uint16_t*>(gate_tables + (int64_t)2 * Q * K);
  const int64_t lanes = (int64_t)Q * 2 * K * 8;
  const int dedup_from = ctx->opt[QPG_OPT_GATE_DEDUP_FROM_CHAINS];
  if (dedup_from > 0 && n_chains >= dedup_from && K <= 512) {
    hipLaunchKernelGGL(gate_table_dedup_kernel, dim3((unsigned)Q), dim3(GD_THREADS), 0, qpg_stream(stream), A, geo, gtab);
    QPG_LAUNCH_CHECK("gate_table_dedup_kernel");
  } else {
    hipLaunchKernelGGL(gate_table_kernel, dim3((unsigned)((lanes + 255) / 256)), dim3(256), 0, qpg_stream(stream), A,
                       geo, gtab);
    QPG_LAUNCH_CHECK("gate_table_kernel");
  }
  if (n_takes > 0) {
    uint16_t* step0 = reinterpret_cast<uint16_t*>(takes_ws);
    uint16_t* trail = step0 + takes_trail_off(n_takes);
    const int stages = ctx->opt[QPG_OPT_TAKES_STAGES];
    if (stages & 1) {
      hipLaunchKernelGGL(takes_step0_kernel, dim3((unsigned)(((int64_t)n_takes * 8 + 255) / 256)), dim3(256), 0,
                         qpg_stream(stream), A, n_takes, step0);
      QPG_LAUNCH_CHECK("takes_step0_kernel");
    }
    if (stages & 2) {
      hipLaunchKernelGGL(gate_chase_takes_kernel,
                         dim3((unsigned)((n_takes + QPG_TAKES_PER_BLOCK - 1) / QPG_TAKES_PER_BLOCK)), dim3(1024), lds_g,
                         qpg_stream(stream), M, steps, K, n_takes, (const uint16_t*)gtab, (const uint16_t*)step0, trail);
      QPG_LAUNCH_CHECK("gate_chase_takes_kernel");
    }
    if (stages & 4) {
      hipLaunchKernelGGL(takes_epilogue_kernel, dim3((unsigned)n_takes), dim3(256), 0, qpg_stream(stream), A, n_takes,
                         (const uint16_t*)trail);
      QPG_LAUNCH_CHECK("takes_epilogue_kernel");
    }
    return QPG_OK;
  }
  hipLaunchKernelGGL(gate_chase_kernel, dim3(n_chains), dim3(1024), lds_g, qpg_stream(stream), A, (const uint16_t*)gtab);
  QPG_LAUNCH_CHECK("gate_chase_kernel");
  return QPG_OK;
}

extern "C" int qpg_match_steps(qpg_ctx* ctx, void* stream, const int16_t* aud_rank, const int32_t* aud_idx,
                               const int16_t* txt_rank, const int32_t* txt_idx, const int16_t* pos_rank,
                               const int16_t* freq_rank, const int32_t* code, int code_ld, const int32_t* aud_cidx,
                               const int32_t* aud_pslot, int Ga, const int32_t* txt_cidx, const int32_t* txt_pslot,
                               int Gt, const float* phase, int Tp, int mode, int M, int steps, int K, int seed_code,
                               const float* seed_phase, int32_t* gate_tables, int32_t* out_codes, float* out_phase,
                               int32_t* out_vote, int32_t* out_status, const int32_t* guard_flags) {
  return match_steps_impl(ctx, stream, aud_rank, aud_idx, txt_rank, txt_idx, pos_rank, freq_rank, code, code_ld, aud_cidx,
                          aud_pslot, Ga, txt_cidx, txt_pslot, Gt, phase, Tp, mode, M, steps, K, seed_code, seed_phase,
                          gate_tables, out_codes, out_phase, out_vote, out_status, guard_flags, 1, nullptr, 2);
}

extern "C" int qpg_match_steps_batch(qpg_ctx* ctx, void* stream, const int16_t* aud_rank, const int32_t* aud_idx,
                                     const int16_t* txt_rank, const int32_t* txt_idx, const int16_t* pos_rank,
                                     const int16_t* freq_rank, const int32_t* code, int code_ld, const int32_t* aud_cidx,
                                     const int32_t* aud_pslot, int Ga, const int32_t* txt_cidx, const int32_t* txt_pslot,
                                     int Gt, const float* phase, int Tp, int mode, int M, int steps, int K,
                                     int n_chains, const int32_t* seed_codes, const float* seed_phase,
                                     int32_t* gate_tables, int32_t* out_codes, float* out_phase, int32_t* out_vote,
                                     int32_t* out_status, int64_t status_stride, const int32_t* guard_flags) {
  QPG_REQUIRE(M > 0 && seed_codes, "qpg_match_steps_batch: M > 0 and device seed codes");
  return match_steps_impl(ctx, stream, aud_rank, aud_idx, txt_rank, txt_idx, pos_rank, freq_rank, code, code_ld, aud_cidx,
                          aud_pslot, Ga, txt_cidx, txt_pslot, Gt, phase, Tp, mode, M, steps, K, 0, seed_phase, gate_tables,
                          out_codes, out_phase, out_vote, out_status, guard_flags, n_chains, seed_codes, status_stride);
}

extern "C" size_t qpg_match_steps_takes_ws_bytes(int n_takes, int M, int steps) {
  if (n_takes < 1 || M < 1 || steps < 1) return 0;
  return sizeof(uint16_t) * (size_t)(takes_trail_off(n_takes) + (int64_t)M * steps * n_takes);
}

extern "C" int qpg_match_steps_takes(qpg_ctx* ctx, void* stream, const int16_t* aud_rank, const int32_t* aud_idx,
                                     const int16_t* txt_rank, const int32_t* txt_idx, const int16_t* pos_rank,
                                     const int16_t* freq_rank, const int32_t* code, int code_ld, const int32_t* aud_cidx,
                                     const int32_t* aud_pslot, int Ga, const int32_t* txt_cidx, const int32_t* txt_pslot,
                                     int Gt, const float* phase, int Tp, int mode, int M, int steps, int K,
                                     int n_takes, const int32_t* seed_codes, const float* seed_phase,
                                     int32_t* gate_tables, int32_t* out_codes, float* out_phase, int32_t* out_vote,
                                     int32_t* out_status, int64_t status_stride, const int32_t* guard_flags,
                                     void* workspace, size_t workspace_bytes) {
  QPG_REQUIRE(M > 0 && seed_codes && n_takes >= 1 && n_takes <= QPG_TAKES_MAX && status_stride >= 2,
              "qpg_match_steps_takes: M > 0, 1 <= n_takes <= %d, device seed codes and a status stride >= 2", QPG_TAKES_MAX);
  return match_steps_impl(ctx, stream, aud_rank, aud_idx, txt_rank, txt_idx, pos_rank, freq_rank, code, code_ld, aud_cidx,
                          aud_pslot, Ga, txt_cidx, txt_pslot, Gt, phase, Tp, mode, M, steps, K, 0, seed_phase, gate_tables,
                          out_codes, out_phase, out_vote, out_status, guard_flags, 1, seed_codes, status_stride, n_takes,
                          workspace, workspace_bytes);
}
```

Baseline: 6.074 million frames/s.

## Fuse best-ranked gate fusion into rank kernels and merge gate table with chase

Arms the context so the rank-producing select/sorted-finish kernels also compute the fused best-ranked gate table in their epilogue, which removes a separate fuse launch per side. It also merges the gate table dedup kernel and the chase kernel into a single launch, using a last-block ticket counter so the final block runs the chase. The aim is to cut launch count and latency in the small single-clip pipeline. In exchange, host-side arming state lives in the context and is not thread-safe, the fused kernels use more threads and LDS, and the chase now runs serially in one trailing block.

```diff
diff --git a/include/qpg.h b/include/qpg.h
--- a/include/qpg.h
+++ b/include/qpg.h
@@ -22,6 +22,8 @@
 int qpg_ctx_destroy(qpg_ctx* ctx);
 #define QPG_OPT_GATE_DEDUP_FROM_CHAINS 0
 #define QPG_OPT_TAKES_STAGES 1
+#define QPG_OPT_FUSE_IN_RANK_LAUNCH 2
+#define QPG_OPT_WALK_ONE_LAUNCH 3
 #define QPG_OPT_COUNT 4
 int qpg_ctx_set_option(qpg_ctx* ctx, int option, int value);
 int qpg_ctx_get_option(qpg_ctx* ctx, int option, int* value);
@@ -229,6 +231,11 @@
                           int64_t status_stride, const int32_t* guard_flags, void* workspace, size_t workspace_bytes);
 int qpg_fuse_best_ranked(qpg_ctx*, void* stream, const int16_t* rank, const int32_t* idx, const int16_t* pos_rank,
                          const int16_t* freq_rank, int Q, int K, int32_t* T);
+int qpg_fuse_arm(qpg_ctx*, void* stream, const int16_t* pos_rank, const int16_t* freq_rank, int Q, int K, int32_t* T0,
+                 int32_t* T1);
+int qpg_fuse_finish(qpg_ctx*, void* stream, int side, const int16_t* rank, const int32_t* idx, const int16_t* pos_rank,
+                    const int16_t* freq_rank, int Q, int K, int32_t* T);
+int qpg_fuse_state(qpg_ctx*, int side);
 
 typedef struct qpg_comm qpg_comm;
 int qpg_comm_unique_id(void* id, int64_t id_bytes);
diff --git a/qpgesture_amd/code_knn.py b/qpgesture_amd/code_knn.py
--- a/qpgesture_amd/code_knn.py
+++ b/qpgesture_amd/code_knn.py
@@ -775,6 +775,21 @@
         sharded = plan.sharded
         T = dict(aud_d=None, aud_idx=None, aud_rank=None, txt_d=None, txt_idx=None, txt_rank=None)
         gtab = torch.empty((3, max(M, 1) * steps, db.K), dtype=torch.int32, device=dev) if plan.split_fuse else None
+        if gtab is not None and Q > 0:
+            _lib.call("qpg_fuse_arm", dev, db.pos_rank, db.freq_rank, Q, db.K, gtab[0], gtab[1])
+            try:
+                return self._sweep_sides(T, plan, gtab, test_interp, test_context, q_win, q_t, q_row, M, steps, mode,
+                                         owner_blocks, after_sweep)
+            except BaseException:
+                _lib.call("qpg_fuse_arm", dev, None, None, 0, 0, None, None)
+                raise
+        return self._sweep_sides(T, plan, gtab, test_interp, test_context, q_win, q_t, q_row, M, steps, mode, owner_blocks,
+                                 after_sweep)
+
+    def _sweep_sides(self, T, plan, gtab, test_interp, test_context, q_win, q_t, q_row, M, steps, mode, owner_blocks,
+                     after_sweep):
+        db, dev = self.db, self.db.device
+        Q, sharded = M * steps, plan.sharded
         lay = self._layout(Q, owner_blocks, mode) if sharded else None
         side = self._fork_side() if plan.overlap else None
         packed = None
@@ -786,7 +801,7 @@
         def keep(p_, g, r):
             T[p_ + "_d"], T[p_ + "_idx"], T[p_ + "_rank"] = r[0], r[1], (None if sharded else r[2])
             if gtab is not None:
-                _lib.call("qpg_fuse_best_ranked", dev, r[2], r[1], db.pos_rank, db.freq_rank, Q, db.K, gtab[g])
+                _lib.call("qpg_fuse_finish", dev, g, r[2], r[1], db.pos_rank, db.freq_rank, Q, db.K, gtab[g])
 
         def text_pack():
             tc = test_context.contiguous()
diff --git a/qpgesture_amd/csrc/qpg_common.h b/qpgesture_amd/csrc/qpg_common.h
--- a/qpgesture_amd/csrc/qpg_common.h
+++ b/qpgesture_amd/csrc/qpg_common.h
@@ -6,13 +6,26 @@
 
 #include "../../include/qpg.h"
 
+#define QPG_WALK_TICKETS 1024
 struct qpg_ctx {
   int device;
   int n_cu;
   float* zeros;
   bool select_lds_raised;
   int opt[QPG_OPT_COUNT];
+  unsigned int* tickets;
+  const void* ticket_owner[QPG_WALK_TICKETS];
+  int n_tickets;
+  struct FuseArm {
+    const int16_t* pos_rank;
+    const int16_t* freq_rank;
+    int32_t* T;
+    int Q, K;
+    bool armed, done;
+  } fuse[2];
 };
+
+unsigned int* qpg_walk_ticket(qpg_ctx* ctx, const void* gate_tables);
 
 #ifdef QPG_DEBUG_HOOKS
 #define QPG_HOOK_VAR(type, name, value) static type name = value
diff --git a/qpgesture_amd/csrc/qpg_core.hip b/qpgesture_amd/csrc/qpg_core.hip
--- a/qpgesture_amd/csrc/qpg_core.hip
+++ b/qpgesture_amd/csrc/qpg_core.hip
@@ -1,4 +1,5 @@
 #include <stdarg.h>
+#include <mutex>
 
 #include "qpg_common.h"
 #include <stdlib.h>
@@ -52,11 +53,17 @@
   for (int i = 0; i < QPG_OPT_COUNT; ++i) c->opt[i] = 0;
   c->opt[QPG_OPT_GATE_DEDUP_FROM_CHAINS] = 1;
   c->opt[QPG_OPT_TAKES_STAGES] = 7;
+  c->opt[QPG_OPT_FUSE_IN_RANK_LAUNCH] = 1;
+  c->opt[QPG_OPT_WALK_ONE_LAUNCH] = 1;
+  c->tickets = nullptr;
+  c->n_tickets = 0;
+  c->fuse[0] = c->fuse[1] = qpg_ctx::FuseArm{nullptr, nullptr, nullptr, 0, 0, false, false};
   int prev = 0;
   (void)hipGetDevice(&prev);
-  const bool ok = hipSetDevice(device) == hipSuccess && hipMalloc(reinterpret_cast<void**>(&c->zeros), 4096) == hipSuccess &&
-                  hipMemset(c->zeros, 0, 4096) == hipSuccess;
+  const bool ok = hipSetDevice(device) == hipSuccess && hipMalloc(reinterpret_cast<void**>(&c->zeros), 4096 + 4 * QPG_WALK_TICKETS) == hipSuccess &&
+                  hipMemset(c->zeros, 0, 4096 + 4 * QPG_WALK_TICKETS) == hipSuccess;
   (void)hipSetDevice(prev);
+  if (ok) c->tickets = reinterpret_cast<unsigned int*>(c->zeros + 1024);
   if (!ok) {
     qpg_set_error("qpg_ctx_create: could not allocate the context's zero page on device %d", device);
     delete c;
@@ -72,6 +79,16 @@
   if (option == QPG_OPT_GATE_DEDUP_FROM_CHAINS) QPG_REQUIRE(value >= 0, "qpg_ctx_set_option: gate_dedup_from_chains >= 0");
   ctx->opt[option] = value;
   return QPG_OK;
+}
+
+static std::mutex g_ticket_mutex;
+unsigned int* qpg_walk_ticket(qpg_ctx* ctx, const void* gate_tables) {
+  std::lock_guard<std::mutex> lock(g_ticket_mutex);
+  for (int i = 0; i < ctx->n_tickets; ++i)
+    if (ctx->ticket_owner[i] == gate_tables) return ctx->tickets + i;
+  if (ctx->n_tickets == QPG_WALK_TICKETS) return nullptr;
+  ctx->ticket_owner[ctx->n_tickets] = gate_tables;
+  return ctx->tickets + ctx->n_tickets++;
 }
 
 extern "C" int qpg_ctx_get_option(qpg_ctx* ctx, int option, int* value) {
diff --git a/qpgesture_amd/csrc/qpg_fuse.h b/qpgesture_amd/csrc/qpg_fuse.h
--- /dev/null
+++ b/qpgesture_amd/csrc/qpg_fuse.h
@@ -0,0 +1,95 @@
+#pragma once
+#include "qpg_common.h"
+
+struct FuseTail {
+  const int16_t* pos_rank;
+  const int16_t* freq_rank;
+  int32_t* T;
+};
+
+static inline FuseTail qpg_fuse_take(qpg_ctx* ctx, int side, int Q, int K) {
+  qpg_ctx::FuseArm& a = ctx->fuse[side];
+  if (!a.armed || a.done || a.Q != Q || a.K != K) return FuseTail{nullptr, nullptr, nullptr};
+  a.done = true;
+  return FuseTail{a.pos_rank, a.freq_rank, a.T};
+}
+
+struct FuseMin {
+  double v;
+  int i;
+};
+__device__ __forceinline__ FuseMin fuse_min(FuseMin a, FuseMin b) {
+  return (b.v < a.v || (b.v == a.v && b.i < a.i)) ? b : a;
+}
+template <int PJ>
+__device__ __forceinline__ FuseMin fuse_xchg(FuseMin m) {
+  const unsigned long long b = (unsigned long long)__double_as_longlong(m.v);
+  const unsigned int lo = (unsigned int)lane_xor<PJ>((int)(unsigned int)b);
+  const unsigned int hi = (unsigned int)lane_xor<PJ>((int)(unsigned int)(b >> 32));
+  return FuseMin{__longlong_as_double((long long)(((unsigned long long)hi << 32) | lo)), lane_xor<PJ>(m.i)};
+}
+__device__ __forceinline__ FuseMin fuse_reduce16(FuseMin x) {
+  x = fuse_min(x, fuse_xchg<8>(x));
+  x = fuse_min(x, fuse_xchg<4>(x));
+  x = fuse_min(x, fuse_xchg<2>(x));
+  x = fuse_min(x, fuse_xchg<1>(x));
+  return x;
+}
+
+template <typename OrderT, typename IdxF>
+__device__ __forceinline__ void fuse_rank_epilogue(const OrderT* order, const int16_t* freq,
+                                                   const int16_t* __restrict__ pos_rank, int K, IdxF&& idx_of,
+                                                   int32_t* __restrict__ Trow) {
+  constexpr int TB = 8;
+  const int l16 = threadIdx.x & 15, g = threadIdx.x >> 4, G = blockDim.x >> 4;
+  int c0[4];
+  double f0[4];
+#pragma unroll
+  for (int u = 0; u < 4; ++u) {
+    const int r = 16 * u + l16;
+    c0[u] = r < K ? (int)order[r] : -1;
+    f0[u] = r < K ? (double)freq[c0[u]] : 0.0;
+  }
+  for (int pb = g; pb < K; pb += TB * G) {
+    int pv[TB][4];
+#pragma unroll
+    for (int t = 0; t < TB; ++t) {
+      const int p = pb + t * G;
+#pragma unroll
+      for (int u = 0; u < 4; ++u) pv[t][u] = (p < K && c0[u] >= 0) ? (int)pos_rank[(int64_t)p * K + c0[u]] : 0;
+    }
+#pragma unroll
+    for (int t = 0; t < TB; ++t)
+#pragma unroll
+      for (int u = 0; u < 4; ++u) asm volatile("" : "+v"(pv[t][u]));
+#pragma unroll
+    for (int t = 0; t < TB; ++t) {
+      const int p = pb + t * G;
+      if (p >= K) break;
+      FuseMin x{__builtin_inf(), 0x7fffffff};
+#pragma unroll
+      for (int u = 0; u < 4; ++u)
+        if (c0[u] >= 0) x = fuse_min(x, FuseMin{((double)pv[t][u] + f0[u] * 0.05) + (double)(16 * u + l16), c0[u]});
+      FuseMin m = fuse_reduce16(x);
+      const int16_t* pr = pos_rank + (int64_t)p * K;
+      for (int base = 64; base < K; base += 64) {
+        if ((double)base > m.v) break;
+        int c[4];
+        double pw[4], fw[4];
+#pragma unroll
+        for (int u = 0; u < 4; ++u) {
+          const int r = base + 16 * u + l16;
+          c[u] = r < K ? (int)order[r] : -1;
+          pw[u] = r < K ? (double)pr[c[u]] : 0.0;
+          fw[u] = r < K ? (double)freq[c[u]] : 0.0;
+        }
+        FuseMin y{__builtin_inf(), 0x7fffffff};
+#pragma unroll
+        for (int u = 0; u < 4; ++u)
+          if (c[u] >= 0) y = fuse_min(y, FuseMin{(pw[u] + fw[u] * 0.05) + (double)(base + 16 * u + l16), c[u]});
+        m = fuse_min(m, fuse_reduce16(y));
+      }
+      if (l16 == 0) Trow[p] = idx_of(m.i);
+    }
+  }
+}
diff --git a/qpgesture_amd/csrc/qpg_select.hip b/qpgesture_amd/csrc/qpg_select.hip
--- a/qpgesture_amd/csrc/qpg_select.hip
+++ b/qpgesture_amd/csrc/qpg_select.hip
@@ -1,4 +1,5 @@
 #include "qpg_common.h"
+#include "qpg_fuse.h"
 
 __device__ __forceinline__ unsigned long long order_key(double d) {
   unsigned long long b = (unsigned long long)__double_as_longlong(d);
@@ -654,7 +655,8 @@
     const DT* __restrict__ D, int64_t ldD, const int16_t* __restrict__ cand_code, int64_t C, int K, double absent,
     int32_t idx_base, double* __restrict__ out_dist, int32_t* __restrict__ out_idx, int16_t* __restrict__ out_rank,
     int q_block, int64_t block_stride, GuardArgs A, double eps1, const double* __restrict__ cn2,
-    const double* __restrict__ qn2, int use_qlds, int phase, unsigned char* __restrict__ ws, int pre, RankCut RC) {
+    const double* __restrict__ qn2, int use_qlds, int phase, unsigned char* __restrict__ ws, int pre, RankCut RC,
+    FuseTail FT) {
   extern __shared__ __attribute__((aligned(16))) unsigned char smem[];
   unsigned long long* best = reinterpret_cast<unsigned long long*>(smem);
   double* v = reinterpret_cast<double*>(smem + 8 * (size_t)K);
@@ -700,6 +702,14 @@
       s_code[r] = k;
     });
   };
+  auto fuse_tail = [&]() {
+    if (!FT.T) return;
+    int16_t* fl = reinterpret_cast<int16_t*>(l_d);
+    for (int k = tid; k < K; k += blockDim.x) fl[k] = FT.freq_rank[k];
+    __syncthreads();
+    fuse_rank_epilogue(s_code, fl, FT.pos_rank, K,
+                       [&](int c) { return besti[c] != 0xffffffffu ? (int32_t)besti[c] : -1; }, FT.T + (int64_t)q * K);
+  };
   int n = 0;
   bool order_parked = false;
   if (phase != 2) {
@@ -1210,6 +1220,7 @@
   }
   if (!repaired) rank_pass(true);
   SEL_STAMP(9);
+  auto settle_rank_ties = [&]() {
   if (A.eps <= 0.0) return;
   __syncthreads();
   for (int r = tid; r + 1 < K; r += blockDim.x) {
@@ -1252,6 +1263,9 @@
   SEL_STAMP(11);
   rank_pass(true);
   SEL_STAMP(12);
+  };
+  settle_rank_ties();
+  fuse_tail();
 }
 
 extern "C" int64_t qpg_percode_select_mixed_ws_bytes(int Q, int K) {
@@ -1306,9 +1320,12 @@
 #define SEL_MIX_LAUNCH(DT, SH, PHASE, PRE)                                                                                  \
   hipLaunchKernelGGL((percode_select_mixed_f64_kernel<DT>), dim3(Q), dim3(1024), SH, qpg_stream(stream),               \
                      static_cast<const DT*>(D), ldD, cand_code, C, K, absent, idx_base, out_dist, out_idx, out_rank,   \
-                     q_block, block_stride, A, eps1, cn2, qn2, use_qlds, PHASE, w, PRE, RCv)
+                     q_block, block_stride, A, eps1, cn2, qn2, use_qlds, PHASE, w, PRE, RCv, FTv)
   RankCut RCv = RCnone;
+  const FuseTail FTnone = {nullptr, nullptr, nullptr};
+  FuseTail FTv = FTnone;
   if (!ws) {
+    if (out_rank && q_block == 0) FTv = qpg_fuse_take(ctx, 0, Q, K);
     if (d_is_f32) SEL_MIX_LAUNCH(float, sh, 0, 0); else SEL_MIX_LAUNCH(double, sh, 0, 0);
     QPG_LAUNCH_CHECK("percode_select_mixed_f64_kernel");
     return QPG_OK;
@@ -1331,6 +1348,7 @@
   const int rb = Q >= 512 ? 8 : (Q >= 128 ? 16 : 64);
   hipLaunchKernelGGL((select_refine_kernel<4>), dim3(Q, rb), dim3(256), 0, qpg_stream(stream), A, K, cn2, qn2, w, use_qlds);
   QPG_LAUNCH_CHECK("select_refine_kernel");
+  if (out_rank && q_block == 0) FTv = qpg_fuse_take(ctx, 0, Q, K);
   if (d_is_f32) SEL_MIX_LAUNCH(float, sh2c, 2, 0); else SEL_MIX_LAUNCH(double, sh2, 2, 0);
   QPG_LAUNCH_CHECK("percode_select_mixed_f64_kernel (merge)");
 #undef SEL_MIX_LAUNCH
diff --git a/qpgesture_amd/csrc/qpg_sorted.hip b/qpgesture_amd/csrc/qpg_sorted.hip
--- a/qpgesture_amd/csrc/qpg_sorted.hip
+++ b/qpgesture_amd/csrc/qpg_sorted.hip
@@ -1,4 +1,5 @@
 #include "qpg_common.h"
+#include "qpg_fuse.h"
 
 __device__ __forceinline__ unsigned int okey32(float d) {
   const unsigned int b = __float_as_uint(d);
@@ -132,13 +133,17 @@
   }
 }
 
-__global__ __launch_bounds__(256) void sorted_finish_kernel(const float* __restrict__ dist, const int32_t* __restrict__ idx,
-                                                             int K, int16_t* __restrict__ out_rank,
-                                                             int32_t* __restrict__ out_nn) {
+template <bool FUSE>
+__device__ __forceinline__ void sorted_finish_block(const float* __restrict__ dist, const int32_t* __restrict__ idx, int K,
+                                                    int16_t* __restrict__ out_rank, int32_t* __restrict__ out_nn,
+                                                    FuseTail FT) {
   extern __shared__ __attribute__((aligned(16))) unsigned char smem[];
   unsigned long long* skey = reinterpret_cast<unsigned long long*>(smem);
   int* scode = reinterpret_cast<int*>(skey + rank_sort_pow2(K));
   float* v = reinterpret_cast<float*>(scode + rank_sort_pow2(K));
+  int32_t* sidx = reinterpret_cast<int32_t*>(v + K);
+  int16_t* order = reinterpret_cast<int16_t*>(sidx + K);
+  int16_t* fl = order + K;
   __shared__ unsigned long long nn_key;
   const int q = blockIdx.x, tid = threadIdx.x, lane = tid & 63;
   if (tid == 0) nn_key = ~0ull;
@@ -147,6 +152,10 @@
     const float dv = dist[(int64_t)q * K + k];
     const int iv = idx[(int64_t)q * K + k];
     v[k] = dv;
+    if (FUSE) {
+      sidx[k] = iv;
+      fl[k] = FT.freq_rank[k];
+    }
     if (iv >= 0) {
       const unsigned long long kv = ((unsigned long long)okey32(dv) << 32) | (unsigned int)iv;
       if (kv < mine) mine = kv;
@@ -163,7 +172,43 @@
     if (tid == 0) out_nn[q] = nn_key != ~0ull ? (int32_t)(nn_key & 0xffffffffu) : -1;
   }
   if (!out_rank) return;
-  block_sorted_ranks(v, K, skey, scode, [&](int k, int r) { out_rank[(int64_t)q * K + k] = (int16_t)r; });
+  block_sorted_ranks(v, K, skey, scode, [&](int k, int r) {
+    out_rank[(int64_t)q * K + k] = (int16_t)r;
+    if (FUSE) order[r] = (int16_t)k;
+  });
+  if (FUSE) {
+    __syncthreads();
+    fuse_rank_epilogue(order, fl, FT.pos_rank, K, [&](int c) { return sidx[c]; }, FT.T + (int64_t)q * K);
+  }
+}
+
+__global__ __launch_bounds__(256) void sorted_finish_kernel(const float* __restrict__ dist, const int32_t* __restrict__ idx,
+                                                             int K, int16_t* __restrict__ out_rank,
+                                                             int32_t* __restrict__ out_nn) {
+  sorted_finish_block<false>(dist, idx, K, out_rank, out_nn, FuseTail{nullptr, nullptr, nullptr});
+}
+
+__global__ __launch_bounds__(1024) void sorted_finish_fuse_kernel(const float* __restrict__ dist,
+                                                                   const int32_t* __restrict__ idx, int K,
+                                                                   int16_t* __restrict__ out_rank,
+                                                                   int32_t* __restrict__ out_nn, FuseTail FT) {
+  sorted_finish_block<true>(dist, idx, K, out_rank, out_nn, FT);
+}
+
+static int launch_sorted_finish(qpg_ctx* ctx, void* stream, const float* dist, const int32_t* idx, int Q, int K,
+                                int16_t* out_rank, int32_t* out_nn, bool may_fuse) {
+  const size_t sh = 12 * (size_t)rank_sort_pow2(K) + 4 * (size_t)K;
+  FuseTail FT = {nullptr, nullptr, nullptr};
+  if (out_rank && may_fuse && sh + 8 * (size_t)K <= 64 * 1024) FT = qpg_fuse_take(ctx, 1, Q, K);
+  if (FT.T) {
+    hipLaunchKernelGGL(sorted_finish_fuse_kernel, dim3(Q), dim3(1024), sh + 8 * (size_t)K, qpg_stream(stream), dist, idx, K,
+                       out_rank, out_nn, FT);
+    QPG_LAUNCH_CHECK("sorted_finish_fuse_kernel");
+  } else {
+    hipLaunchKernelGGL(sorted_finish_kernel, dim3(Q), dim3(256), sh, qpg_stream(stream), dist, idx, K, out_rank, out_nn);
+    QPG_LAUNCH_CHECK("sorted_finish_kernel");
+  }
+  return QPG_OK;
 }
 
 extern "C" int qpg_percode_select_sorted_f32(qpg_ctx* ctx, void* stream, const float* Dm, int64_t ldD, const float* tile_min,
@@ -193,9 +238,8 @@
                      idx_base, q_block, block_stride);
   QPG_LAUNCH_CHECK("percode_select_sorted_kernel");
   if (out_rank || out_nn) {
-    hipLaunchKernelGGL(sorted_finish_kernel, dim3(Q), dim3(256), 12 * (size_t)rank_sort_pow2(K) + 4 * (size_t)K, qpg_stream(stream),
-                       (const float*)out_dist, (const int32_t*)out_idx, K, out_rank, out_nn);
-    QPG_LAUNCH_CHECK("sorted_finish_kernel");
+    const int rc = launch_sorted_finish(ctx, stream, out_dist, out_idx, Q, K, out_rank, out_nn, q_block == 0);
+    if (rc != QPG_OK) return rc;
   }
   return QPG_OK;
 }
@@ -453,9 +497,8 @@
     QPG_LAUNCH_CHECK("percode_select_bycode_kernel");
   }
   if (out_rank || out_nn) {
-    hipLaunchKernelGGL(sorted_finish_kernel, dim3(Q), dim3(256), 12 * (size_t)rank_sort_pow2(K) + 4 * (size_t)K, qpg_stream(stream),
-                       (const float*)out_dist, (const int32_t*)out_idx, K, out_rank, out_nn);
-    QPG_LAUNCH_CHECK("sorted_finish_kernel");
+    const int rc = launch_sorted_finish(ctx, stream, out_dist, out_idx, Q, K, out_rank, out_nn, true);
+    if (rc != QPG_OK) return rc;
   }
   return QPG_OK;
 }
diff --git a/qpgesture_amd/csrc/qpg_tail.hip b/qpgesture_amd/csrc/qpg_tail.hip
--- a/qpgesture_amd/csrc/qpg_tail.hip
+++ b/qpgesture_amd/csrc/qpg_tail.hip
@@ -1,4 +1,5 @@
 #include "qpg_common.h"
+#include "qpg_fuse.h"
 #include <type_traits>
 
 __global__ __launch_bounds__(256) void l2_table_kernel(const float* __restrict__ sig, int K, int Dm,
@@ -519,13 +520,13 @@
 
 #define GD_SLOTS 2048
 #define GD_THREADS 1024
-__global__ __launch_bounds__(GD_THREADS) void gate_table_dedup_kernel(TailArgs A, GateGeom geo, uint16_t* __restrict__ Gt) {
+__device__ __forceinline__ void gate_row_dedup(const TailArgs& A, const GateGeom& geo, uint16_t* Gt, int q) {
   __shared__ int key[GD_SLOTS];
   __shared__ unsigned short val[GD_SLOTS];
   __shared__ unsigned short ulist[GD_SLOTS];
   __shared__ int n_u;
   const int K = A.K, Qc = A.M * A.steps, tid = threadIdx.x, lane = tid & 63;
-  const int q = blockIdx.x, chain = q / Qc, s = q % A.steps;
+  const int chain = q / Qc, s = q % A.steps;
   uint16_t* out = Gt + (int64_t)q * 2 * K;
   if (q == chain * Qc) {
     if (tid < 8) {
@@ -576,14 +577,17 @@
     if (slot[u] >= 0) out[u * GD_THREADS + tid] = val[slot[u]];
 }
 
+__global__ __launch_bounds__(GD_THREADS) void gate_table_dedup_kernel(TailArgs A, GateGeom geo, uint16_t* __restrict__ Gt) {
+  gate_row_dedup(A, geo, Gt, blockIdx.x);
+}
+
 #define QPG_CHASE_QMAX 2048
-__global__ __launch_bounds__(1024) void gate_chase_kernel(TailArgs A, const uint16_t* __restrict__ Gt) {
+__device__ __forceinline__ void gate_chase_block(TailArgs A, const uint16_t* Gt, int chain) {
   extern __shared__ __attribute__((aligned(16))) uint16_t gl[];
   __shared__ uint16_t sig[QPG_CHASE_QMAX];
   __shared__ int bad_s;
   const int K = A.K, Q = A.M * A.steps, tid = threadIdx.x, nt = blockDim.x;
   const int per_w = A.steps * 2 * K;
-  const int chain = blockIdx.x;
   const int64_t q0 = (int64_t)chain * Q;
   Gt += q0 * 2 * K;
   A.T0 += q0 * K;
@@ -642,6 +646,32 @@
   }
 }
 
+__global__ __launch_bounds__(1024) void gate_chase_kernel(TailArgs A, const uint16_t* __restrict__ Gt) {
+  gate_chase_block(A, Gt, blockIdx.x);
+}
+
+__global__ __launch_bounds__(GD_THREADS) void gate_chase_with_table_kernel(TailArgs A, GateGeom geo, uint16_t* Gt, unsigned int* ticket) {
+  __shared__ int is_last;
+  gate_row_dedup(A, geo, Gt, blockIdx.x);
+  asm volatile("s_waitcnt vmcnt(0)" ::: "memory");
+  __syncthreads();
+  if (threadIdx.x == 0) {
+    __builtin_amdgcn_fence(__ATOMIC_RELEASE, "agent");
+    asm volatile("s_waitcnt vmcnt(0)" ::: "memory");
+    const unsigned int t = __hip_atomic_fetch_add(ticket, 1u, __ATOMIC_ACQ_REL, __HIP_MEMORY_SCOPE_AGENT);
+    const int last = t == gridDim.x - 1;
+    if (last) {
+      __hip_atomic_store(ticket, 0u, __ATOMIC_RELAXED, __HIP_MEMORY_SCOPE_AGENT);
+      __builtin_amdgcn_fence(__ATOMIC_ACQUIRE, "agent");
+      asm volatile("s_waitcnt vmcnt(0)" ::: "memory");
+    }
+    is_last = last;
+  }
+  __syncthreads();
+  if (!is_last) return;
+  gate_chase_block(A, Gt, 0);
+}
+
 #define QPG_TAKES_PER_BLOCK 64
 __host__ __device__ __forceinline__ int64_t takes_trail_off(int n_takes) { return ((int64_t)n_takes + 7) & ~(int64_t)7; }
 
@@ -742,6 +772,42 @@
                      qpg_stream(stream), rank, idx, pos_rank, freq_rank, Q, K, T);
   QPG_LAUNCH_CHECK("fuse_best_ranked_one_kernel");
   return QPG_OK;
+}
+
+extern "C" int qpg_fuse_arm(qpg_ctx* ctx, void* stream, const int16_t* pos_rank, const int16_t* freq_rank, int Q, int K,
+                            int32_t* T0, int32_t* T1) {
+  (void)stream;
+  QPG_REQUIRE(ctx, "qpg_fuse_arm: null context");
+  for (int side = 0; side < 2; ++side) ctx->fuse[side] = qpg_ctx::FuseArm{nullptr, nullptr, nullptr, 0, 0, false, false};
+  if (!pos_rank && !freq_rank && !T0 && !T1) return QPG_OK;
+  QPG_REQUIRE(pos_rank && freq_rank && T0 && T1, "qpg_fuse_arm: null pointer (all four null: disarm)");
+  QPG_REQUIRE(Q > 0 && K > 0 && (K % 16) == 0 && K <= 4096 && ((int64_t)Q * K) / 16 < 0x7fffffffll,
+              "qpg_fuse_arm: K %% 16 == 0, K <= 4096");
+  QPG_REQUIRE((reinterpret_cast<uintptr_t>(T0) % 4) == 0 && (reinterpret_cast<uintptr_t>(T1) % 4) == 0 &&
+                  (reinterpret_cast<uintptr_t>(pos_rank) % 2) == 0 && (reinterpret_cast<uintptr_t>(freq_rank) % 2) == 0,
+              "qpg_fuse_arm: misaligned table");
+  if (!ctx->opt[QPG_OPT_FUSE_IN_RANK_LAUNCH]) return QPG_OK;
+  ctx->fuse[0] = qpg_ctx::FuseArm{pos_rank, freq_rank, T0, Q, K, true, false};
+  ctx->fuse[1] = qpg_ctx::FuseArm{pos_rank, freq_rank, T1, Q, K, true, false};
+  return QPG_OK;
+}
+
+extern "C" int qpg_fuse_state(qpg_ctx* ctx, int side) {
+  if (!ctx || side < 0 || side > 1) return QPG_EINVAL;
+  return !ctx->fuse[side].armed ? 0 : (ctx->fuse[side].done ? 2 : 1);
+}
+
+extern "C" int qpg_fuse_finish(qpg_ctx* ctx, void* stream, int side, const int16_t* rank, const int32_t* idx,
+                               const int16_t* pos_rank, const int16_t* freq_rank, int Q, int K, int32_t* T) {
+  QPG_REQUIRE(ctx && (side == 0 || side == 1), "qpg_fuse_finish: null context or side not 0 / 1");
+  const qpg_ctx::FuseArm a = ctx->fuse[side];
+  ctx->fuse[side] = qpg_ctx::FuseArm{nullptr, nullptr, nullptr, 0, 0, false, false};
+  if (a.armed && a.done) {
+    QPG_REQUIRE(a.T == T && a.Q == Q && a.K == K && a.pos_rank == pos_rank && a.freq_rank == freq_rank,
+                "qpg_fuse_finish: side %d's rank launch filled another table than the one asked for", side);
+    return QPG_OK;
+  }
+  return qpg_fuse_best_ranked(ctx, stream, rank, idx, pos_rank, freq_rank, Q, K, T);
 }
 
 
@@ -830,6 +896,15 @@
   uint16_t* gtab = reinterpret_cast<uint16_t*>(gate_tables + (int64_t)2 * Q * K);
   const int64_t lanes = (int64_t)Q * 2 * K * 8;
   const int dedup_from = ctx->opt[QPG_OPT_GATE_DEDUP_FROM_CHAINS];
+  if (ctx->opt[QPG_OPT_WALK_ONE_LAUNCH] && dedup_from == 1 && n_chains == 1 && n_takes == 0 && K <= 512 &&
+      lds_g <= 40 * 1024) {
+    unsigned int* ticket = qpg_walk_ticket(ctx, gate_tables);
+    if (ticket) {
+      hipLaunchKernelGGL(gate_chase_with_table_kernel, dim3((unsigned)Q), dim3(GD_THREADS), lds_g, qpg_stream(stream), A, geo, gtab, ticket);
+      QPG_LAUNCH_CHECK("gate_chase_with_table_kernel");
+      return QPG_OK;
+    }
+  }
   if (dedup_from > 0 && n_chains >= dedup_from && K <= 512) {
     hipLaunchKernelGGL(gate_table_dedup_kernel, dim3((unsigned)Q), dim3(GD_THREADS), 0, qpg_stream(stream), A, geo, gtab);
     QPG_LAUNCH_CHECK("gate_table_dedup_kernel");
```

Measured after the change: 5.923 million frames/s. 0.975x the previous value.
